# ESMS-Group-Public/FoKL-GPy

Hardware: AMD Instinct MI355X
Metric: candidate-terms/sec (basis build + Gibbs + BIC) (higher is better)
Workload: dtype f64

## Files before the change

### fokl_gpy_amd/_capi.py

```python
import ctypes
import os

import numpy as np

_HERE = os.path.dirname(os.path.abspath(__file__))
LIB_PATH = os.environ.get('FOKL_HIP_LIBRARY', os.path.join(_HERE, 'libfokl_hip.so'))

UNIQUE_ID_BYTES = 128
K_BASIS, K_GRAM, K_RESID, K_PREDICT, K_RESID_MF, K_GRAM_MFMA, K_GRAM_REDUCE = 0, 1, 2, 3, 4, 5, 6
K_INTEGRATE, K_BAND = 7, 8
K_OPTIMIZE = 9
K_OPTIMIZE_SYSTEM = 10
K_POPULATION = 11
K_RESAMPLE = 12
INTEGRATE_MAX_STATES = 4
RESID_TERMS_MAX_FACTORS = 32
RESID_TERMS_MAX_ORDER = 8
RESID_TERMS_LAYOUTS = ((8, 1), (16, 1), (8, 2), (4, 4), (2, 8), (8, 4), (16, 2), (4, 8))
SLOT_ONES, SLOT_Y, SLOT_FIRST_FREE = 0, 1, 2
PREDICT_NONE, PREDICT_VALU_LDS, PREDICT_VALU_GLOBAL, PREDICT_MFMA = 0, 1, 2, 3
POPULATION_COEFFICIENTS = ('none', 'registers', 'table')
POPULATION_MAX_CUTS = 32
RESAMPLE_MAX_COLUMNS = 768
RESAMPLE_ATTEMPT_CAP = 64
RESAMPLE_SEGMENTS = 3
RES_BETA, RES_SIG_NORMAL, RES_SIG_UNIFORM, RES_TAU_NORMAL, RES_TAU_UNIFORM, RES_START = 3, 4, 5, 6, 7, 8
GRAM_KERNELS = ('none', 'valu', 'tiles', 'dma', 'panel', 'tiles4')
RESID_KERNELS = ('none', 'columns', 'matrix_free')
BASIS_KERNELS = ('none', 'reg_table', 'lds_table')

c_int, c_i32, c_i64, c_dbl, c_vp = ctypes.c_int, ctypes.c_int32, ctypes.c_int64, ctypes.c_double, ctypes.c_void_p

SIGNATURES = {
    'fokl_version': (c_int, []),
    'fokl_device_count': (c_int, [c_vp]),
    'fokl_ctx_create': (c_int, [c_int, c_vp]),
    'fokl_ctx_destroy': (None, [c_vp]),
    'fokl_last_error': (ctypes.c_char_p, [c_vp]),
    'fokl_sync': (c_int, [c_vp]),
    'fokl_upload': (c_int, [c_vp, c_vp, c_vp, c_i64, c_int, c_int, c_vp, c_int, c_int]),
    'fokl_stage_inputs': (c_int, [c_vp, c_vp, c_i64, c_int, c_vp, c_vp]),
    'fokl_upload_staged': (c_int, [c_vp, c_vp, c_i64, c_int, c_int, c_vp, c_int, c_int, c_vp, c_vp]),
    'fokl_download_inputs': (c_int, [c_vp, c_vp]),
    'fokl_column_min_max': (c_int, [c_vp, c_i64, c_int, c_vp, c_vp, c_int]),
    'fokl_normalize_columns': (c_int, [c_vp, c_i64, c_int, c_vp, c_vp, c_int]),
    'fokl_reserve_slots': (c_int, [c_vp, c_int]),
    'fokl_slot_capacity': (c_int, [c_vp]),
    'fokl_rows': (c_i64, [c_vp]),
    'fokl_build_terms': (c_int, [c_vp, c_vp, c_int, c_vp]),
    'fokl_build_terms_deriv': (c_int, [c_vp, c_vp, c_int, c_vp, c_int, c_int, c_dbl]),
    'fokl_gram': (c_int, [c_vp, c_vp, c_int, c_vp, c_int, c_vp, c_int, c_int]),
    'fokl_gram_launch': (c_int, [c_vp, c_vp, c_int, c_vp, c_int, c_int]),
    'fokl_gram_fetch': (c_int, [c_vp, c_vp, c_i64]),
    'fokl_gram_ready': (c_int, [c_vp]),
    'fokl_gram_plan': (c_int, [c_vp, c_int, c_vp, c_int, c_int, c_vp, c_vp, c_vp, c_vp, c_vp, c_int]),
    'fokl_bic_resid': (c_int, [c_vp, c_vp, c_int, c_vp, c_vp, c_int]),
    'fokl_bic_resid_launch': (c_int, [c_vp, c_vp, c_int, c_vp]),
    'fokl_bic_resid_fetch': (c_int, [c_vp, c_vp, c_int]),
    'fokl_bic_resid_terms_launch': (c_int, [c_vp, c_vp, c_int, c_vp]),
    'fokl_predict': (c_int, [c_vp, c_vp, c_int, c_vp, c_int, c_int, c_vp, c_vp]),
    'fokl_predict_report': (c_int, [c_vp, c_vp]),
    'fokl_fit_report': (c_int, [c_vp, c_int, c_vp, c_int]),
    'fokl_population_stats': (c_int, [c_vp, c_vp, c_int, c_vp, c_int, c_vp, c_vp, c_int, c_int, c_vp, c_vp]),
    'fokl_population_report': (c_int, [c_vp, c_vp]),
    'fokl_resample_chains': (c_int, [c_vp, c_int, c_vp, c_vp, c_vp, c_dbl, c_dbl, c_dbl, c_dbl, c_dbl, c_int, c_vp, c_vp, c_int,
                                     c_int, c_int, ctypes.c_uint32, c_int, c_int, c_vp, c_vp, c_vp, c_vp, c_vp, c_vp]),
    'fokl_resample_report': (c_int, [c_vp, c_vp]),
    'fokl_read_slot': (c_int, [c_vp, c_int, c_i64, c_i64, c_vp]),
    'fokl_write_slot': (c_int, [c_vp, c_int, c_i64, c_i64, c_vp]),
    'fokl_timing_enable': (c_int, [c_vp, c_int]),
    'fokl_timing_reset': (c_int, [c_vp]),
    'fokl_timing_get': (c_int, [c_vp, c_int, c_vp, c_vp, c_vp, c_vp, c_vp]),
    'fokl_probe': (c_int, [c_vp, c_int, c_vp]),
    'fokl_gibbs_chain': (c_int, [c_vp, c_vp, c_int, c_dbl, c_dbl, c_dbl, c_dbl, c_dbl, c_dbl, c_dbl, c_int,
                                 c_vp, c_vp, c_vp, c_vp, c_vp, c_vp, c_vp]),
    'fokl_noise_tape': (c_int, [c_int, c_int, c_dbl, c_dbl, c_vp, c_vp, c_vp, c_vp, c_vp, c_vp, c_vp, c_vp, c_vp,
                                c_vp]),
    'fokl_gibbs_chain_from_tape': (c_int, [c_vp, c_vp, c_int, c_dbl, c_dbl, c_dbl, c_dbl, c_dbl, c_int, c_vp, c_vp, c_vp,
                                           c_vp, c_vp, c_vp, c_vp, c_vp, c_vp, c_vp]),
    'fokl_pool_create': (c_int, [c_int, c_int, c_int, c_int, c_int, c_vp, c_vp, c_vp, c_vp, c_vp, c_vp, c_int, c_vp]),
    'fokl_pool_stream': (c_vp, [c_vp]),
    'fokl_pool_use_dsyevd': (c_int, [c_vp, c_vp, c_int]),
    'fokl_pool_use_dgemm': (c_int, [c_vp, c_vp]),
    'fokl_device_dgemm': (None, [c_vp] * 13),
    'fokl_device_dgemm_configure': (c_int, [c_int, c_vp, c_int, c_vp]),
    'fokl_device_dgemm_stats': (c_int, [c_vp, c_vp, c_vp]),
    'fokl_pool_spectral_affinity': (c_int, [c_vp, c_vp, c_int]),
    'fokl_pool_release_hold': (c_int, [c_vp, ctypes.c_uint64]),
    'fokl_pool_destroy': (None, [c_vp]),
    'fokl_pool_submit_noise': (c_int, [c_vp, c_int, c_int, c_dbl, c_dbl, c_vp, c_vp, c_vp, c_vp, c_vp, c_vp, c_vp, c_int,
                                       c_vp, c_int, c_int, c_vp, c_vp]),
    'fokl_tape_ready': (c_int, [c_vp, c_int, c_vp, c_int]),
    'fokl_pool_resolve': (c_int, [c_vp, c_int]),
    'fokl_pool_submit_chain': (c_int, [c_vp, c_vp, c_vp, c_int, c_dbl, c_dbl, c_dbl, c_dbl, c_dbl, c_int, c_vp, c_vp,
                                       c_vp, c_vp, c_vp, c_vp, c_vp, c_int, c_int, c_vp, c_vp, c_vp, c_vp, c_vp]),
    'fokl_pool_submit_spectral': (c_int, [c_vp, c_vp, c_int, c_vp, c_int, c_int, c_vp, c_vp, c_vp, c_vp, c_vp,
                                          c_vp]),
    'fokl_pool_submit_spectral_update': (c_int, [c_vp, c_vp, c_int, c_vp, c_int, c_int, c_vp, c_vp, c_int, c_vp, c_vp, c_vp,
                                                 c_vp, c_vp, c_vp, c_vp, c_vp]),
    'fokl_pool_poll': (c_int, [c_vp]),
    'fokl_pool_wait': (c_int, [c_vp]),
    'fokl_pool_busy_seconds': (c_int, [c_vp, c_vp, c_vp, c_vp, c_vp]),
    'fokl_pool_noise_waits': (c_int, [c_vp, c_vp, c_vp]),
    'fokl_pool_chain_segments': (c_int, [c_vp, c_vp, c_vp]),
    'fokl_thread_cpu_seconds': (c_int, [c_vp, c_int]),
    'fokl_pool_stream_stats': (c_int, [c_vp, c_vp, c_vp, c_vp, c_vp, c_vp]),
    'fokl_stream_create': (c_int, [c_vp, c_i32, c_i32, c_dbl, c_int, c_vp, c_int, c_vp]),
    'fokl_stream_prestates_published': (c_i64, [c_vp]),
    'fokl_stream_given_gauss': (c_dbl, [c_vp]),
    'fokl_stream_destroy': (None, [c_vp]),
    'fokl_stream_walk': (c_int, [c_vp, c_int, c_int, c_dbl, c_dbl, c_vp, c_vp, c_vp, c_vp]),
    'fokl_stream_tell': (c_int, [c_vp, c_vp]),
    'fokl_stream_seek': (c_int, [c_vp, c_vp]),
    'fokl_stream_hold': (c_int, [c_vp, c_vp]),
    'fokl_stream_release': (c_int, [c_vp, ctypes.c_uint64]),
    'fokl_stream_advance_floor': (c_int, [c_vp]),
    'fokl_stream_state': (c_int, [c_vp, c_vp, c_vp, c_vp, c_vp]),
    'fokl_stream_expand': (c_int, [c_vp, c_int, c_dbl, c_dbl, c_vp, c_int, c_int, c_vp, c_vp, c_vp, c_vp, c_vp]),
    'fokl_stream_stats': (c_int, [c_vp, c_vp, c_vp, c_vp, c_vp, c_vp]),
    'fokl_stream_set_helpers': (c_int, [c_vp, c_int, c_vp]),
    'fokl_stream_place_bulk': (c_int, [c_vp, c_vp, c_int]),
    'fokl_stream_fast_ln_error': (c_dbl, [c_i64]),
    'fokl_search_create': (c_int, [c_vp, c_vp, c_vp, c_vp]),
    'fokl_search_bind_spectral': (c_int, [c_vp, c_vp, c_int, c_dbl, c_int]),
    'fokl_search_hold_spectral': (c_int, [c_vp, c_int]),
    'fokl_search_set_update': (c_int, [c_vp, c_int, c_int, c_int]),
    'fokl_search_set_decide': (c_int, [c_vp, c_int, c_dbl]),
    'fokl_search_set_deterministic': (c_int, [c_vp, c_int]),
    'fokl_search_destroy': (None, [c_vp]),
    'fokl_search_error': (ctypes.c_char_p, [c_vp]),
    'fokl_search_mispredicted': (c_int, [c_vp]),
    'fokl_search_set_substage': (c_int, [c_vp, c_vp, c_int]),
    'fokl_search_speculate': (c_int, [c_vp, c_vp, c_vp, c_int]),
    'fokl_search_drop_speculation': (c_int, [c_vp]),
    'fokl_search_spectral': (c_int, [c_vp, c_vp, c_int, c_vp, c_int, c_vp]),
    'fokl_search_spectral_from': (c_int, [c_vp, c_vp, c_int, c_vp, c_int, c_vp, c_int, c_vp]),
    'fokl_spectrum_done': (c_int, [c_vp]),
    'fokl_spectrum_wait': (c_int, [c_vp, c_vp, c_vp, c_vp]),
    'fokl_spectrum_release': (None, [c_vp, c_vp]),
    'fokl_spectrum_retain': (c_int, [c_vp, c_vp]),
    'fokl_search_model_begin': (c_int, [c_vp, c_vp, c_int, c_vp, c_int, c_vp, c_vp, c_vp, c_int, c_vp, c_vp]),
    'fokl_search_model_commit': (c_int, [c_vp, c_vp, c_vp, c_dbl, c_int, c_vp]),
    'fokl_run_create': (c_int, [c_vp, c_vp, c_vp]),
    'fokl_run_set_update': (c_int, [c_vp, c_int, c_int, c_int]),
    'fokl_run_search': (c_int, [c_vp, c_vp]),
    'fokl_run_result': (c_int, [c_vp, c_vp, c_vp, c_vp, c_vp, c_vp]),
    'fokl_run_arrays': (c_int, [c_vp, c_vp, c_vp, c_vp, c_vp, c_vp, c_vp]),
    'fokl_run_error': (ctypes.c_char_p, [c_vp]),
    'fokl_run_destroy': (None, [c_vp]),
    'fokl_search_score': (c_int, [c_vp, c_vp, c_dbl, c_dbl, c_int, c_int, c_vp]),
    'fokl_outcome_info': (c_int, [c_vp, c_vp, c_vp]),
    'fokl_outcome_spectrum': (c_int, [c_vp, c_vp, c_vp]),
    'fokl_outcome_chain_ready': (c_int, [c_vp]),
    'fokl_outcome_draws': (c_int, [c_vp, c_vp, c_vp]),
    'fokl_outcome_intercept_scale': (c_int, [c_vp, c_vp, c_vp]),
    'fokl_outcome_new_term_stats': (c_int, [c_vp, c_vp, c_vp, c_int, c_int, c_int, c_vp, c_vp]),
    'fokl_outcome_release': (None, [c_vp, c_vp]),
    'fokl_outcome_drop': (None, [c_vp, c_vp]),
    'fokl_search_verify': (c_int, [c_vp, c_int]),
    'fokl_search_register_forecast': (c_int, [c_vp, c_vp, c_int, c_vp, c_dbl]),
    'fokl_search_clear_forecasts': (None, [c_vp]),
    'fokl_search_likely_first_tests': (c_int, [c_vp, c_vp, c_int, c_dbl, c_vp, c_vp, c_vp]),
    'fokl_search_stats': (c_int, [c_vp, c_vp, c_int]),
    'fokl_search_trace': (c_i64, [c_vp, c_vp, c_i64]),
    'fokl_search_kill_tests': (c_int, [c_vp, c_vp, c_vp]),
    'fokl_finish_tape_blocks': (c_int, [c_int, c_int, c_vp, c_vp, c_vp, c_vp, c_int, c_int, c_int, c_vp]),
    'fokl_gibbs_chain_from_finished_tape': (c_int, [c_vp, c_vp, c_int, c_dbl, c_dbl, c_dbl, c_dbl, c_dbl, c_int, c_vp,
                                                    c_vp, c_vp, c_vp, c_int, c_vp, c_vp, c_vp, c_vp]),
    'fokl_gibbs_chain_segments_host': (c_int, [c_vp, c_vp, c_int, c_dbl, c_dbl, c_dbl, c_dbl, c_dbl, c_int, c_vp, c_vp,
                                               c_vp, c_vp, c_int, c_vp, c_vp, c_vp, c_vp, c_int, c_int, c_vp]),
    'fokl_rng_normals': (c_int, [c_vp, c_vp, c_vp, c_vp, c_i64, c_vp]),
    'fokl_rng_gammas': (c_int, [c_vp, c_vp, c_vp, c_vp, c_dbl, c_dbl, c_i64, c_vp]),
    'fokl_gp_integrate': (c_int, [c_int, c_int, c_i64, c_vp, c_vp, c_vp, c_vp, c_vp, c_vp, c_vp, c_vp, c_vp, c_int, c_int,
                                  c_dbl, c_vp, c_vp]),
    'fokl_gp_integrate_ensemble': (c_int, [c_vp, c_int, c_int, c_int, c_i64, c_vp, c_vp, c_vp, c_vp, c_vp, c_vp, c_vp, c_vp,
                                           c_vp, c_vp, c_int, c_int, c_dbl, c_vp, c_int, c_int, c_vp, c_vp, c_vp]),
    'fokl_model_optimize': (c_int, [c_vp, c_int, c_int, c_vp, c_int, c_vp, c_vp, c_int, c_int, c_vp, c_vp, c_int, c_vp, c_dbl,
                                    c_int, c_dbl, c_vp, c_vp, c_vp, c_vp]),
    'fokl_system_optimize': (c_int, [c_vp, c_int, c_int, c_vp, c_vp, c_vp, c_vp, c_vp, c_vp, c_int, c_vp, c_vp, c_int, c_int,
                                     c_vp, c_vp, c_int, c_vp, c_int, c_int, c_dbl, c_dbl, c_dbl, c_int, c_vp, c_vp, c_vp,
                                     c_int, c_dbl, c_dbl, c_vp, c_vp, c_vp, c_vp, c_vp, c_vp, c_vp]),
    'fokl_embedded_hmc': (c_int, [c_vp, c_int, c_int, c_vp, c_int, c_vp, c_int, c_vp, c_int, c_vp, c_int, c_int, c_int, c_int,
                                  ctypes.c_uint32, c_vp, c_dbl, c_int, c_vp, c_vp, c_vp, c_vp, c_vp, c_vp, c_vp, c_vp, c_vp]),
    'fokl_embedded_rng': (c_int, [ctypes.c_uint32, ctypes.c_uint32, ctypes.c_uint32, c_int, c_int, c_vp]),
    'fokl_dchain_create': (c_int, [c_int, c_int, c_vp]),
    'fokl_dchain_destroy': (None, [c_vp]),
    'fokl_dchain_submit': (c_int, [c_vp, c_int, c_int, c_vp, c_vp, c_dbl, c_dbl, c_dbl, c_dbl, c_dbl, c_vp, c_vp, c_vp,
                                   c_vp, c_vp, c_vp, c_int, c_int, c_int, c_vp, c_vp]),
    'fokl_dchain_prestate_ring': (c_int, [c_vp, c_vp, c_vp]),
    'fokl_dchain_bind_stream': (c_int, [c_vp, c_vp]),
    'fokl_dchain_submit_rows': (c_int, [c_vp, c_int, c_int, c_vp, c_vp, c_dbl, c_dbl, c_dbl, c_dbl, c_dbl, c_dbl, c_dbl, c_vp,
                                        c_vp, c_vp, c_vp, c_vp, c_int, c_vp, c_vp]),
    'fokl_dchain_stream_stats': (c_int, [c_vp, c_vp, c_vp]),
# ... 228 lines not shown
            off.append(off[-1] + pad(count))
        rows = off[4] + pad((ints[1] + d + 1) // 2) + 8
        off.append(rows)
        return tuple(off), ints, rows + 4 * d + 8

    @classmethod
    def doubles_needed(cls, p1, draws):
        return cls._layout(int(p1), int(draws))[2]

    def __init__(self, p1, draws, raw=None):
        self.p1, self.draws = p1, d = int(p1), int(draws)
        off, ints, total = self._layout(p1, d)
        self._off, self._ints = off, ints
        if raw is None:
            raw = np.empty(total, dtype=np.float64)
        elif raw.shape[0] < total:
            raise ValueError("buffer too small for this tape")
        shift = ((-raw.__array_interface__['data'][0]) % 64) // 8
        self._buf = raw[shift:]
        self._addr = self._buf.__array_interface__['data'][0]
        self._buf[off[4]:off[4] + ints[1] // 2] = 0.0
        self.finishing_requested = False
        self.materialised_by_pool = False

    def _int_area(self):
        return self._buf[self._off[4]:].view(np.int32)

    normals = property(lambda self: self._buf[:self.draws * self.p1].reshape(self.draws, self.p1))
    pair_r2 = property(lambda self: self._buf[self._off[1]:self._off[1] + self.draws * (self.p1 // 2 + 1)]
                       .reshape(self.draws, self.p1 // 2 + 1))
    gam_sig = property(lambda self: self._buf[self._off[2]:self._off[2] + self.draws])
    gam_tau = property(lambda self: self._buf[self._off[3]:self._off[3] + self.draws])
    progress = property(lambda self: self._int_area()[:1])
    block_done = property(lambda self: self._int_area()[self._ints[0]:self._ints[0] + -(-self.draws // self.BLOCK)])
    lead = property(lambda self: self._int_area()[self._ints[1]:self._ints[1] + self.draws])

    def pointers(self):
        a, off = self._addr, self._off
        return (a, a + 8 * off[1], a + 8 * off[4] + 4 * self._ints[1], a + 8 * off[2], a + 8 * off[3])

    def progress_pointer(self):
        return self._addr + 8 * self._off[4]

    def rows_pointer(self):
        return self._addr + 8 * self._off[5]

    rows = property(lambda self: self._buf[self._off[5]:self._off[5] + 4 * self.draws].view(np.uint64)
                    .reshape(self.draws, 4))

    def block_done_pointer(self):
        return self._addr + 8 * self._off[4] + 4 * self._ints[0]


def record_noise_tape(tape, astar, atau_star, stream):
    try:
        _check(load().fokl_noise_tape(tape.p1, tape.draws, float(astar), float(atau_star), *stream.args(),
                                      *tape.pointers(), tape.progress_pointer()))
    except BaseException:
        tape.progress[0] = -1
        raise
    return tape


def noise_tape(p1, draws, astar, atau_star, stream):
    return record_noise_tape(NoiseTape(p1, draws), astar, atau_star, stream)


class _StreamCursor(ctypes.Structure):
    _fields_ = [('position', ctypes.c_uint64), ('gauss_source', ctypes.c_uint64), ('has_gauss', ctypes.c_int32)]


class StreamEngine:

    def __init__(self, stream, bulk_threads=2, prestates=None):
        self._lib = load()
        self._h = None
        self.stream = stream
        h = c_vp(0)
        _check(self._lib.fokl_stream_create(_ptr(stream.key), stream.pos, stream.has_gauss, stream.cache,
                                            int(bulk_threads), prestates[0] if prestates else None,
                                            prestates[1] if prestates else 0, ctypes.byref(h)))
        self._h = h

    def close(self, write_back=True):
        if self._h:
            if write_back:
                _check(self._lib.fokl_stream_state(self._h, *self.stream.args()))
            self._lib.fokl_stream_destroy(self._h)
            self._h = None

    def __del__(self):
        self.close(write_back=False)

    def walk(self, tape, astar, atau_star):
        hold = ctypes.c_uint64(0)
        _check(self._lib.fokl_stream_hold(self._h, ctypes.byref(hold)))
        a = tape._addr
        rc = self._lib.fokl_stream_walk(self._h, tape.p1, tape.draws, float(astar), float(atau_star), tape.rows_pointer(),
                                        a + 8 * tape._off[2], a + 8 * tape._off[3], tape.progress_pointer())
        if rc:
            self._lib.fokl_stream_release(self._h, hold)
        _check(rc)
        _check(self._lib.fokl_stream_advance_floor(self._h))
        return hold.value

    def expand(self, tape, astar, atau_star, first=0, last=None):
        ptr = tape.pointers()
        _check(self._lib.fokl_stream_expand(self._h, tape.p1, float(astar), float(atau_star), tape.rows_pointer(),
                                            int(first), tape.draws if last is None else int(last), ptr[0], ptr[1], ptr[2],
                                            ptr[3], ptr[4]))
        return tape

    def release(self, hold):
        _check(self._lib.fokl_stream_release(self._h, ctypes.c_uint64(hold)))

    def tell(self):
        cur = _StreamCursor()
        _check(self._lib.fokl_stream_tell(self._h, ctypes.byref(cur)))
        return cur

    def seek(self, cursor):
        _check(self._lib.fokl_stream_seek(self._h, ctypes.byref(cursor)))

    def numpy_state(self):
        st = LegacyStream(self.stream.as_numpy_state())
        _check(self._lib.fokl_stream_state(self._h, *st.args()))
        return st.as_numpy_state()

    def stats(self):
        b, w, seg, ga, ge = c_dbl(0), c_dbl(0), c_i64(0), c_i64(0), c_i64(0)
        _check(self._lib.fokl_stream_stats(self._h, *[ctypes.byref(x) for x in (b, w, seg, ga, ge)]))
        return dict(bulk_s=b.value, walker_wait_s=w.value, segments=seg.value, gamma_attempts=ga.value,
                    gamma_attempts_exact=ge.value)


def tape_ready(tape):
    return load().fokl_tape_ready(tape.progress_pointer(), tape.draws,
                                  tape.block_done_pointer() if tape.materialised_by_pool else None, tape.BLOCK)


def gibbs_chain_from_tape(lamb, qty, b, btau, dtd, sigsqd0, tausqd0, tape, want_sig_tau=False, follow=False):
    lamb = np.ascontiguousarray(lamb, dtype=np.float64)
    qty = np.ascontiguousarray(qty, dtype=np.float64)
    p1 = lamb.shape[0]
    if p1 != tape.p1:
        raise ValueError("tape was recorded for a different model size")
    w = np.empty((tape.draws, p1), dtype=np.float64)
    sigs = np.empty(tape.draws) if want_sig_tau else None
    taus = np.empty(tape.draws) if want_sig_tau else None
    flag = ctypes.c_int32(0)
    _check(load().fokl_gibbs_chain_from_tape(_ptr(lamb), _ptr(qty), p1, float(b), float(btau), float(dtd),
                                             float(sigsqd0), float(tausqd0), tape.draws, *tape.pointers(), _ptr(w),
                                             _ptr(sigs), _ptr(taus), ctypes.byref(flag),
                                             tape.progress_pointer() if follow else None))
    if want_sig_tau:
        return w, bool(flag.value), sigs, taus
    return w, bool(flag.value)


def finish_tape_blocks(tape, part=0, parts=1, follow=False):
    ptr = tape.pointers()
    _check(load().fokl_finish_tape_blocks(tape.p1, tape.draws, ptr[0], ptr[1], ptr[2],
                                          tape.progress_pointer() if follow else None, int(part), int(parts),
                                          tape.BLOCK, tape.block_done_pointer()))


def gibbs_chain_from_finished_tape(lamb, qty, b, btau, dtd, sigsqd0, tausqd0, tape, follow=False):
    lamb = np.ascontiguousarray(lamb, dtype=np.float64)
    qty = np.ascontiguousarray(qty, dtype=np.float64)
    p1 = lamb.shape[0]
    if p1 != tape.p1:
        raise ValueError("tape was recorded for a different model size")
    w = np.empty((tape.draws, p1), dtype=np.float64)
    flag = ctypes.c_int32(0)
    ptr = tape.pointers()
    _check(load().fokl_gibbs_chain_from_finished_tape(_ptr(lamb), _ptr(qty), p1, float(b), float(btau), float(dtd),
                                                      float(sigsqd0), float(tausqd0), tape.draws, ptr[0], ptr[3],
                                                      ptr[4], tape.block_done_pointer() if follow else None,
                                                      tape.BLOCK, _ptr(w), None, None, ctypes.byref(flag)))
    return w, bool(flag.value)


CHAIN_SEGMENTS, CHAIN_WARM = 8, 64


def gibbs_chain_segments_host(lamb, qty, b, btau, dtd, sigsqd0, tausqd0, tape, follow=False, segments=CHAIN_SEGMENTS,
                              warm=CHAIN_WARM, states=False):
    lamb = np.ascontiguousarray(lamb, dtype=np.float64)
    qty = np.ascontiguousarray(qty, dtype=np.float64)
    p1 = lamb.shape[0]
    if p1 != tape.p1:
        raise ValueError("tape was recorded for a different model size")
    w = np.empty((tape.draws, p1), dtype=np.float64)
    sigs = np.empty(tape.draws, dtype=np.float64) if states else None
    taus = np.empty(tape.draws, dtype=np.float64) if states else None
    flag, bad_cut = ctypes.c_int32(0), ctypes.c_int32(0)
    ptr = tape.pointers()
    _check(load().fokl_gibbs_chain_segments_host(_ptr(lamb), _ptr(qty), p1, float(b), float(btau), float(dtd),
                                                 float(sigsqd0), float(tausqd0), tape.draws, ptr[0], ptr[3], ptr[4],
                                                 tape.block_done_pointer() if follow else None, tape.BLOCK, _ptr(w),
                                                 _ptr(sigs) if states else None, _ptr(taus) if states else None,
                                                 ctypes.byref(flag), int(segments), int(warm), ctypes.byref(bad_cut)))
    if states:
        return w, bool(flag.value), bool(bad_cut.value), sigs, taus
    return w, bool(flag.value), bool(bad_cut.value)



def _scipy_dsyevd_address():
    try:
        from scipy.linalg import cython_lapack
        capsule = cython_lapack.__pyx_capi__['dsyevd']
        api = ctypes.pythonapi
        api.PyCapsule_GetName.restype = ctypes.c_char_p
        api.PyCapsule_GetName.argtypes = [ctypes.py_object]
        api.PyCapsule_GetPointer.restype = ctypes.c_void_p
        api.PyCapsule_GetPointer.argtypes = [ctypes.py_object, ctypes.c_char_p]
        name = api.PyCapsule_GetName(capsule)
        if name is None or name.count(b'int *') != 6 or b'long' in name:
            return None
        return api.PyCapsule_GetPointer(capsule, name)
    except (ImportError, KeyError):
        return None


def _scipy_dgemm_address():
    try:
        from scipy.linalg import cython_blas
        capsule = cython_blas.__pyx_capi__['dgemm']
        api = ctypes.pythonapi
        api.PyCapsule_GetName.restype = ctypes.c_char_p
        api.PyCapsule_GetName.argtypes = [ctypes.py_object]
        api.PyCapsule_GetPointer.restype = ctypes.c_void_p
        api.PyCapsule_GetPointer.argtypes = [ctypes.py_object, ctypes.c_char_p]
        name = api.PyCapsule_GetName(capsule)
        if name is None or name.count(b'int *') != 6 or name.count(b'char *') != 2 or b'long' in name:
            return None
        return api.PyCapsule_GetPointer(capsule, name)
    except (ImportError, KeyError):
        return None


def _scipy_dsyevr_address():
    from scipy.linalg import cython_lapack
    capsule = cython_lapack.__pyx_capi__['dsyevr']
    api = ctypes.pythonapi
    api.PyCapsule_GetName.restype = ctypes.c_char_p
    api.PyCapsule_GetName.argtypes = [ctypes.py_object]
    api.PyCapsule_GetPointer.restype = ctypes.c_void_p
    api.PyCapsule_GetPointer.argtypes = [ctypes.py_object, ctypes.c_char_p]
    name = api.PyCapsule_GetName(capsule)
    if name is None or name.count(b'int *') != 11 or b'long' in name:
        raise FoklNativeError(-2, f"unexpected signature of scipy's dsyevr: {name!r}")
    return api.PyCapsule_GetPointer(capsule, name)


class PoolJob:
    __slots__ = ('_h', 'keep', 'result', 'recycle', 'held', 'unresolved', 'ignore_failure', 'co_reader')

    def __init__(self, handle, keep, result=None, tentative=False):
        self._h, self.keep, self.result = handle, keep, result
        self.recycle = None
        self.held = None
        self.unresolved = bool(tentative)
        self.ignore_failure = False
        self.co_reader = None

    def done(self):
        if self._h is not None and load().fokl_pool_poll(self._h):
            self.wait()
        return self._h is None

    def resolve(self, commit):
        if self.unresolved:
            self.unresolved = False
            _check(load().fokl_pool_resolve(self._h, int(bool(commit))))

    def wait(self):
        if self._h is not None:
            h, self._h = self._h, None
            rc = load().fokl_pool_wait(h)
            if not self.ignore_failure:
                _check(rc)
        return self.result


class SpectralResult:
    __slots__ = ('lamb', 'Qt', 'qty', 'betahat', 'moments', '_buf', '_addr')

    @staticmethod
    def doubles(p1):
        return p1 * (p1 + 3) + 2

    def __init__(self, p1, buf=None):
        buf = self._buf = np.empty(p1 * (p1 + 3) + 2, dtype=np.float64) if buf is None else buf
        self._addr = buf.__array_interface__['data'][0]
        self.lamb, self.qty, self.betahat = buf[:p1], buf[p1:2 * p1], buf[2 * p1:3 * p1]
        self.Qt = buf[3 * p1:3 * p1 + p1 * p1].reshape(p1, p1)
        self.moments = buf[3 * p1 + p1 * p1:]

    def pointers(self, p1):
        a = self._addr
        return (a, a + 24 * p1, a + 8 * p1, a + 16 * p1, a + 8 * p1 * (p1 + 3))


class HostPool:

    def __init__(self, stream, chain_threads=2, finish_threads=2, spectral_threads=3, noise_cpu=-1, bulk_threads=2,
                 prestates=None, device_dgemm=None):
        self._lib = load()
        self.stream = stream
        self._h = None
        h = c_vp(0)
        fn = _scipy_dsyevr_address() if spectral_threads > 0 else None
        self.finish_threads = int(finish_threads)
        _check(self._lib.fokl_pool_create(int(chain_threads), self.finish_threads, int(spectral_threads),
                                          max(1, int(bulk_threads)), int(noise_cpu), c_vp(fn),
                                          *stream.args(), prestates[0] if prestates else None,
                                          prestates[1] if prestates else 0, ctypes.byref(h)))
        self._h = h
        self.dsyevd_from = 0
        dc_from = int(os.environ.get('FOKL_EIGH_DC_FROM', '80'))
        if spectral_threads > 0 and dc_from > 0 and os.environ.get('FOKL_EIGH_SIGNS', 'canonical') != 'lapack':
            fd = _scipy_dsyevd_address()
            if fd:
                _check(self._lib.fokl_pool_use_dsyevd(self._h, c_vp(fd), dc_from))
                self.dsyevd_from = dc_from
        self.has_dgemm = False
        if spectral_threads > 0:
            fg = _scipy_dgemm_address()
            self.device_dgemm_from = 0
            if fg and device_dgemm is not None:
                entry = c_vp(0)
                if self._lib.fokl_device_dgemm_configure(int(device_dgemm[0]), c_vp(fg), int(device_dgemm[1]),
                                                         ctypes.byref(entry)) == 0 and entry.value:
                    fg, self.device_dgemm_from = entry.value, int(device_dgemm[1])
            if fg:
                _check(self._lib.fokl_pool_use_dgemm(self._h, c_vp(fg)))
                self.has_dgemm = True

    def spectral_affinity(self, cpus):
        cpus = np.ascontiguousarray(sorted(cpus), dtype=np.int32)
        _check(self._lib.fokl_pool_spectral_affinity(self._h, _ptr(cpus), cpus.shape[0]))

    def stream_handle(self):
        return self._lib.fokl_pool_stream(self._h)

    def set_walk_helpers(self, count, cpus=None):
        arr = None
        if cpus is not None:
            arr = np.ascontiguousarray(list(cpus)[:count] + [-1] * max(0, count - len(cpus)), dtype=np.int32)
        _check(self._lib.fokl_stream_set_helpers(c_vp(self.stream_handle()), int(count), _ptr(arr) if arr is not None else None))

    def place_bulk_threads(self, cpus):
        arr = np.ascontiguousarray(list(cpus), dtype=np.int32)
        _check(self._lib.fokl_stream_place_bulk(c_vp(self.stream_handle()), _ptr(arr), arr.shape[0]))

    def close(self):
        if self._h:
            self._lib.fokl_pool_destroy(self._h)
            self._h = None

    __del__ = close

    def submit_noise(self, tape, astar, atau_star, tentative=False, finish=False):
        h = c_vp(0)
        finish = bool(finish) and self.finish_threads > 0
        _check(self._lib.fokl_pool_submit_noise(self._h, tape.p1, tape.draws, float(astar), float(atau_star),
                                                tape.rows_pointer(), *tape.pointers(), tape.progress_pointer(),
                                                int(bool(tentative)), tape.block_done_pointer(), tape.BLOCK, int(finish),
                                                None, ctypes.byref(h)))
        tape.finishing_requested = finish
        tape.materialised_by_pool = True
        return PoolJob(h, (tape,), tape, tentative)

    def submit_chain(self, lamb, qty, b, btau, dtd, sigsqd0, tausqd0, tape, w_raw=None):
        p1 = lamb.shape[0]
        if p1 != tape.p1:
            raise ValueError("tape was recorded for a different model size")
        if w_raw is None:
            w = np.empty((tape.draws, p1), dtype=np.float64)
        else:
            w = w_raw[:tape.draws * p1].reshape(tape.draws, p1)
        flag = np.zeros(1, dtype=np.int32)
        h = c_vp(0)
        _check(self._lib.fokl_pool_submit_chain(self._h, _ptr(lamb), _ptr(qty), p1, float(b), float(btau), float(dtd),
                                                float(sigsqd0), float(tausqd0), tape.draws, *tape.pointers(),
                                                tape.progress_pointer(), tape.block_done_pointer(),
                                                tape.BLOCK, int(tape.finishing_requested), _ptr(w), _ptr(flag),
                                                None, None, ctypes.byref(h)))
        return PoolJob(h, (lamb, qty, tape, w, flag), (w, flag))

    def submit_spectral(self, gram, idx, ycol):
        p1 = idx.shape[0]
        res = SpectralResult(p1)
        h = c_vp(0)
        _check(self._lib.fokl_pool_submit_spectral(self._h, _ptr(gram), gram.shape[1], _ptr(idx), p1, int(ycol),
                                                   *res.pointers(p1), ctypes.byref(h)))
        return PoolJob(h, (gram, idx, res), res)

    def submit_spectral_update(self, gram, idx, ycol, parent, parent_pos):
        p1 = idx.shape[0]
        res = SpectralResult(p1)
        updated = np.full(1, -1, dtype=np.int32)
        h = c_vp(0)
        _check(self._lib.fokl_pool_submit_spectral_update(self._h, _ptr(gram), gram.shape[1], _ptr(idx), p1, int(ycol),
                                                          _ptr(parent.lamb), _ptr(parent.Qt), int(parent_pos), None,
                                                          *res.pointers(p1), _ptr(updated), ctypes.byref(h)))
        return PoolJob(h, (gram, idx, res, parent, updated), res), updated

    def busy_seconds(self):
        v = [c_dbl(0) for _ in range(4)]
        _check(self._lib.fokl_pool_busy_seconds(self._h, *[ctypes.byref(x) for x in v]))
        w = [c_dbl(0), c_dbl(0)]
        _check(self._lib.fokl_pool_noise_waits(self._h, ctypes.byref(w[0]), ctypes.byref(w[1])))
        b, ww, seg, ga, ge = c_dbl(0), c_dbl(0), c_i64(0), c_i64(0), c_i64(0)
        _check(self._lib.fokl_pool_stream_stats(self._h, *[ctypes.byref(x) for x in (b, ww, seg, ga, ge)]))
        cs = [c_i64(0), c_i64(0)]
        _check(self._lib.fokl_pool_chain_segments(self._h, ctypes.byref(cs[0]), ctypes.byref(cs[1])))
        return dict(noise=v[0].value, chain=v[1].value, finish=v[2].value, spectral=v[3].value,
                    host_chains_segmented=cs[0].value, host_chain_recuts=cs[1].value,
                    noise_queue_wait=w[0].value, noise_verdict_wait=w[1].value, bulk=b.value, walker_wait=ww.value,
                    stream_segments=seg.value, gamma_attempts=ga.value, gamma_attempts_exact=ge.value)



class _SearchParams(ctypes.Structure):
    _fields_ = [('n', c_i64), ('a', c_dbl), ('b', c_dbl), ('atau', c_dbl), ('btau', c_dbl), ('threshav', c_dbl),
                ('threshstda', c_dbl), ('threshstdb', c_dbl), ('guess_margin', c_dbl), ('draws', c_i32), ('half0', c_i32),
                ('aic', c_i32), ('lookahead', c_i32), ('foresight', c_i32), ('speculation_max', c_i32),
                ('tentative_tapes', c_i32), ('test_rewinds', c_i32), ('device_chain_columns', c_i32),
                ('finish_threads', c_i32), ('flip_guess', c_i32), ('device_rows', c_i32)]


class _OutcomeView(ctypes.Structure):
    _fields_ = [('spectrum', c_vp), ('idx', c_vp), ('ev', c_dbl), ('siglik', c_dbl), ('intercept_scale', c_dbl),
                ('p1', c_i32), ('on_device', c_i32)]


_FORESEE_CB = ctypes.CFUNCTYPE(None, c_vp, ctypes.POINTER(c_i32), c_int)
_IDLE_CB = ctypes.CFUNCTYPE(c_int, c_vp)
_RESIDUAL_CB = ctypes.CFUNCTYPE(c_int, c_vp, ctypes.POINTER(c_i32), c_int, ctypes.POINTER(c_dbl), ctypes.POINTER(c_dbl),
                                ctypes.POINTER(c_dbl))


class _KillTestsArgs(ctypes.Structure):
# ... 301 lines not shown
        self._engine, self._ticket, self.p1, self.draws, self.keep = engine, ticket, p1, draws, keep
        self.recycle = None
        self._stats = None
        self.ignore_failure = False
        self._area = self._flag = None
        self._mark = float(ticket) if ticket is not None else 0.0
        self._misses = 0
        if stats_address:
            self._area = np.ctypeslib.as_array((ctypes.c_double * (7 + p1)).from_address(stats_address))
            self._flag = ctypes.c_double.from_address(stats_address + 8 * (4 + p1))

    def resolve(self, commit):
        pass

    def _ran(self):
        return self._flag is not None and self._flag.value == self._mark

    def done(self):
        if self._ticket is None or self._stats is not None or self._ran():
            return True
        if self._flag is not None:
            self._misses += 1
            if self._misses % 64:
                return False
        return bool(self._engine._lib.fokl_dchain_poll(self._engine._h, self._ticket))

    def wait(self):
        if self._stats is None:
            if self._ticket is None:
                raise RuntimeError("device chain: released before anybody read its statistics")
            if self._ran():
                self._stats = np.array(self._area[:4 + self.p1])
            else:
                buf = np.empty(4 + self.p1, dtype=np.float64)
                _check(self._engine._lib.fokl_dchain_wait(self._engine._h, self._ticket, _ptr(buf)))
                self._stats = buf
        return self._stats[4:], np.array([int(self._stats[0])], dtype=np.int32)

    @property
    def kernel_seconds(self):
        if self._area is not None and self._ran():
            return float(self._area[5 + self.p1])
        return 0.0

    @property
    def rows_averaged(self):
        self.wait()
        return int(self._stats[3])

    @property
    def bad_cut(self):
        self.wait()
        if self._area is None:
            raise RuntimeError("device chain: released, its statistics area belongs to another chain")
        return bool(self._area[6 + self.p1] != 0.0)

    @property
    def last_state(self):
        self.wait()
        return float(self._stats[1]), float(self._stats[2])

    def fetch_w(self, out=None):
        w = np.empty((self.draws, self.p1), dtype=np.float64) if out is None else out
        _check(self._engine._lib.fokl_dchain_fetch_w(self._engine._h, self._ticket, _ptr(w)))
        return w

    def try_release(self):
        if self._ticket is None or not self._engine._h:
            return True
        if self._flag is not None and not self._ran() and self._stats is None:
            return False
        if self._engine._lib.fokl_dchain_try_release(self._engine._h, self._ticket):
            self._ticket, self.keep, self._area, self._flag = None, None, None, None
            return True
        return False

    def release(self):
        if self._ticket is not None and self._engine._h:
            self._engine._lib.fokl_dchain_release(self._engine._h, self._ticket)
        self._ticket = None
        self.keep = self._area = self._flag = None


class DeviceChainEngine:
    max_columns = 768

    def __init__(self, device=0, slots=96):
        self._lib = load()
        self._h = None
        h = c_vp(0)
        _check(self._lib.fokl_dchain_create(int(device), int(slots), ctypes.byref(h)))
        self._h = h
        self.device = int(device)

    def close(self):
        if self._h:
            self._lib.fokl_dchain_destroy(self._h)
            self._h = None

    __del__ = close

    def submit(self, lamb, qty, b, btau, dtd, sigsqd0, tausqd0, tape, stat_first=0, follow=True):
        lamb = np.ascontiguousarray(lamb, dtype=np.float64)
        qty = np.ascontiguousarray(qty, dtype=np.float64)
        p1 = lamb.shape[0]
        if p1 != tape.p1:
            raise ValueError("tape was recorded for a different model size")
        ptr = tape.pointers()
        finished = bool(tape.finishing_requested)
        ticket, area = c_i64(0), c_vp(0)
        _check(self._lib.fokl_dchain_submit(self._h, p1, tape.draws, _ptr(lamb), _ptr(qty), float(b), float(btau),
                                            float(dtd), float(sigsqd0), float(tausqd0), ptr[0], ptr[2], ptr[3], ptr[4],
                                            tape.progress_pointer() if follow else None,
                                            tape.block_done_pointer() if finished or tape.materialised_by_pool else None,
                                            tape.BLOCK, int(finished),
                                            int(stat_first), ctypes.byref(ticket), ctypes.byref(area)))
        return DeviceChainJob(self, ticket.value, p1, tape.draws, (tape,), area.value)

    def prestate_ring(self):
        ring, entries = c_vp(0), c_int(0)
        _check(self._lib.fokl_dchain_prestate_ring(self._h, ctypes.byref(ring), ctypes.byref(entries)))
        return ring.value, entries.value

    def bind(self, stream_handle):
        _check(self._lib.fokl_dchain_bind_stream(self._h, stream_handle))

    def submit_rows(self, lamb, qty, b, btau, dtd, sigsqd0, tausqd0, astar, atau_star, tape, span, stat_first=0):
        lamb = np.ascontiguousarray(lamb, dtype=np.float64)
        qty = np.ascontiguousarray(qty, dtype=np.float64)
        p1 = lamb.shape[0]
        ptr = tape.pointers()
        ticket, area = c_i64(0), c_vp(0)
        _check(self._lib.fokl_dchain_submit_rows(self._h, p1, tape.draws, _ptr(lamb), _ptr(qty), float(b), float(btau),
                                                 float(dtd), float(sigsqd0), float(tausqd0), float(astar), float(atau_star),
                                                 tape.rows_pointer(), ptr[3], ptr[4], tape.progress_pointer(), _ptr(span),
                                                 int(stat_first), ctypes.byref(ticket), ctypes.byref(area)))
        return DeviceChainJob(self, ticket.value, p1, tape.draws, (tape, span), area.value)

    def stream_stats(self):
        seg, rows = c_i64(0), c_i64(0)
        _check(self._lib.fokl_dchain_stream_stats(self._h, ctypes.byref(seg), ctypes.byref(rows)))
        return dict(segments_made=seg.value, rows_jobs=rows.value)

    def flush(self):
        _check(self._lib.fokl_dchain_flush(self._h))

    def stats(self):
        busy, issued, launches, staged = c_dbl(0), c_i64(0), c_i64(0), c_i64(0)
        _check(self._lib.fokl_dchain_stats(self._h, ctypes.byref(busy), ctypes.byref(issued), ctypes.byref(launches),
                                           ctypes.byref(staged)))
        recuts = c_i64(0)
        _check(self._lib.fokl_dchain_recuts(self._h, ctypes.byref(recuts)))
        return dict(dispatch_s=busy.value, issued=issued.value, launches=launches.value, staged=staged.value,
                    recuts=recuts.value)


class DeviceSpectralJob:

    def __init__(self, engine, ticket, result, p1):
        self.engine, self.ticket, self.p1 = engine, int(ticket), int(p1)
        n = self.p1
        area = (ctypes.c_double * (n * n + 3 * n + 7)).from_address(result)
        self._area = np.frombuffer(area, dtype=np.float64)
        self._released = False

    def done(self):
        rc = self.engine._lib.fokl_dspectral_poll(self.engine._h, self.ticket)
        if rc < 0:
            _check(-rc)
        return rc == 1

    def wait(self):
        _check(self.engine._lib.fokl_dspectral_wait(self.engine._h, self.ticket))
        n, a = self.p1, self._area
        return a[:n], a[3 * n:3 * n + n * n].reshape(n, n), a[n:2 * n], a[2 * n:3 * n], a[3 * n + n * n:3 * n + n * n + 2]

    def info(self):
        a = self._area[3 * self.p1 + self.p1 * self.p1 + 2:]
        return dict(sweeps=int(a[0]), rotations=int(a[1]), seconds=float(a[2]), not_converged=bool(a[3]))
# ... 147 lines not shown
                 bic_resid_fetch=bic_resid_fetch)
    keep = [pending, raised]
    for name, fn in table.items():
        cb = _OPS_TYPES[name](guard(fn))
        keep.append(cb)
        setattr(ops, name, ctypes.cast(cb, c_vp).value)
    return ops, tuple(keep)


class NativeRun:

    def __init__(self, backend, kernel_id, **params):
        self._lib = load()
        self._h = None
        self._ops, self._keep = backend_ops(backend, kernel_id)
        if isinstance(self._keep[0], dict):
            self._keep[0]['m'] = int(params['m'])
        self._prm = _RunParams(**{k: int(v) for k, v in params.items()})
        self.m = int(params['m'])
        h = c_vp(0)
        _check(self._lib.fokl_run_create(ctypes.byref(self._ops), ctypes.byref(self._prm), ctypes.byref(h)))
        self._h = h
        self._reraise()

    def _reraise(self):
        raised = self._keep[1] if isinstance(self._keep[0], dict) else None
        if raised:
            exc = raised[0]
            del raised[:]
            raise exc

    def set_update(self, from_columns, depth, lookahead):
        _check(self._lib.fokl_run_set_update(self._h, int(from_columns), int(depth), int(lookahead)))

    def search(self, native_search):
        rc = self._lib.fokl_run_search(self._h, native_search._h)
        self._reraise()
        if rc != 0:
            native_search._checked(rc)
        return self

    def result(self):
        rows, n_evs, subs = c_i32(0), c_i32(0), c_i32(0)
        best, last = c_vp(0), c_vp(0)
        _check(self._lib.fokl_run_result(self._h, ctypes.byref(rows), ctypes.byref(n_evs), ctypes.byref(subs),
                                         ctypes.byref(best), ctypes.byref(last)))
        mtx = np.zeros((max(rows.value, 0), self.m), dtype=np.int32)
        evs = np.zeros(n_evs.value)
        sizes = np.zeros(max(subs.value, 1), dtype=np.int32)
        stats = np.zeros(16)
        total = self._lib.fokl_run_arrays(self._h, _ptr(mtx) if mtx.size else None, _ptr(evs) if evs.size else None,
                                          _ptr(sizes), None, None, _ptr(stats))
        mean_abs, rel_std = np.zeros(max(total, 1)), np.zeros(max(total, 1))
        self._lib.fokl_run_arrays(self._h, None, None, None, _ptr(mean_abs), _ptr(rel_std), None)
        per, at = [], 0
        for size in sizes[:subs.value]:
            per.append(dict(mean_abs=mean_abs[at:at + size].copy(), rel_std=rel_std[at:at + size].copy()))
            at += int(size)
        return (mtx.astype(np.float64), evs, per, best.value, last.value, dict(zip(RUN_STATS, stats[:len(RUN_STATS)])))

    def close(self):
        if self._h is not None and self._h:
            self._lib.fokl_run_destroy(self._h)
            self._h = None

    def __del__(self):
        try:
            self.close()
        except Exception:
            pass


class DeviceContext:

    def __init__(self, device=0):
        self._lib = load()
        h = c_vp(0)
        _check(self._lib.fokl_ctx_create(int(device), ctypes.byref(h)))
        self._h = h
        self.device = device

    def close(self):
        if getattr(self, '_h', None) is not None and self._h:
            self._lib.fokl_ctx_destroy(self._h)
            self._h = None

    def __del__(self):
        try:
            self.close()
        except Exception:
            pass

    def _ck(self, rc):
        _check(rc, self._h)

    def sync(self):
        self._ck(self._lib.fokl_sync(self._h))

    _lazy_owner = None

    def _settle_lazy_inputs(self, keep=None):
        owner, self._lazy_owner = self._lazy_owner, None
        model = owner() if owner is not None else None
        if model is not None and model is not keep:
            model._materialise_inputs()

    def upload(self, x, y, kernel_id, phis_packed, n_basis, width):
        self._settle_lazy_inputs()
        x = np.ascontiguousarray(x, dtype=np.float64)
        y = np.ascontiguousarray(np.reshape(y, -1), dtype=np.float64)
        if x.ndim != 2 or x.shape[0] != y.shape[0]:
            raise ValueError("inputs must be [n, m] and data [n]")
        phis_packed = np.ascontiguousarray(phis_packed, dtype=np.float64)
        self._ck(self._lib.fokl_upload(self._h, _ptr(x), _ptr(y), x.shape[0], x.shape[1], int(kernel_id),
                                       _ptr(phis_packed), int(n_basis), int(width)))
        self.n, self.m = x.shape

    def stage_inputs(self, x, owner=None):
        if x.dtype != np.float64 or x.ndim != 2 or not x.flags.c_contiguous:
            raise ValueError("stage_inputs: float64 C-contiguous [n, m] expected")
        self._settle_lazy_inputs(keep=owner)
        lows, highs = np.empty(x.shape[1]), np.empty(x.shape[1])
        self._ck(self._lib.fokl_stage_inputs(self._h, _ptr(x), x.shape[0], x.shape[1], _ptr(lows), _ptr(highs)))
        self._staged_shape = x.shape
        return lows, highs

    def upload_staged(self, y, kernel_id, phis_packed, n_basis, width, lows, spans, owner=None):
        n, m = self._staged_shape
        y = np.ascontiguousarray(np.reshape(y, -1), dtype=np.float64)
        if y.shape[0] != n:
            raise ValueError("inputs must be [n, m] and data [n]")
        phis_packed = np.ascontiguousarray(phis_packed, dtype=np.float64)
        lows, spans = np.ascontiguousarray(lows, dtype=np.float64), np.ascontiguousarray(spans, dtype=np.float64)
        self._ck(self._lib.fokl_upload_staged(self._h, _ptr(y), n, m, int(kernel_id), _ptr(phis_packed), int(n_basis),
                                              int(width), _ptr(lows), _ptr(spans)))
        self.n, self.m = n, m
        if owner is not None:
            import weakref
            self._lazy_owner = weakref.ref(owner)

    def download_inputs(self):
        out = np.empty((getattr(self, 'n', 0) or 1, getattr(self, 'm', 0) or 1), dtype=np.float64)
        self._ck(self._lib.fokl_download_inputs(self._h, _ptr(out)))
        return out

    def reserve_slots(self, n_slots):
        self._ck(self._lib.fokl_reserve_slots(self._h, int(n_slots)))

    @property
    def slot_capacity(self):
        return self._lib.fokl_slot_capacity(self._h)

    def build_terms(self, terms, slots):
        terms = np.ascontiguousarray(np.atleast_2d(terms), dtype=np.int32)
        slots = np.ascontiguousarray(slots, dtype=np.int32)
        if terms.shape[0] != slots.shape[0]:
            raise ValueError("one slot per term")
        self._ck(self._lib.fokl_build_terms(self._h, _ptr(terms), terms.shape[0], _ptr(slots)))

    def build_terms_deriv(self, terms, slots, wrt_input, order, divisor):
        terms = np.ascontiguousarray(np.atleast_2d(terms), dtype=np.int32)
        slots = np.ascontiguousarray(slots, dtype=np.int32)
        if terms.shape[0] != slots.shape[0]:
            raise ValueError("one slot per term")
        self._ck(self._lib.fokl_build_terms_deriv(self._h, _ptr(terms), terms.shape[0], _ptr(slots), int(wrt_input),
                                                  int(order), float(divisor)))
# ... 317 lines not shown
```

### fokl_gpy_amd/csrc/fokl_hostpool.cpp

```cpp
#include <algorithm>
#include <array>
#include <atomic>
#include <chrono>
#include <cmath>
#include <condition_variable>
#include <cstdint>
#include <cstdio>
#include <cstdlib>
#include <cstring>
#include <deque>
#include <mutex>
#include <string>
#include <thread>
#include <vector>

#include <immintrin.h>
#include <pthread.h>
#include <sched.h>
#include <sys/prctl.h>

#include "../../include/fokl_hip_internal.h"
#include "fokl_spin.h"

extern void fokl_set_global_error(const std::string &msg);

extern "C" __attribute__((visibility("hidden"))) void fokl_finish_tape_rows(int p1, double *normals, const double *pair_r2,
                                                                            const int32_t *lead, int k0, int k1);
extern "C" __attribute__((visibility("hidden"))) int64_t fokl_chain_follow_waited_ns();
extern "C" __attribute__((visibility("hidden"))) int fokl_gibbs_chain_from_raw_blocks(
    const double *lamb, const double *qty, int p1, double b, double btau, double dtd, double sigsqd0, double tausqd0,
    int draws, const double *normals, const double *pair_r2, const int32_t *lead, const double *gam_sig,
    const double *gam_tau, const int32_t *block_done, int block, double *w_out, int32_t *bstar_negative);

static std::atomic<int64_t> g_thread_cpu_ns[8];

extern "C" __attribute__((visibility("hidden"))) void fokl_note_thread_cpu(int kind)
{
    timespec ts;
    if (kind >= 0 && kind < 8 && clock_gettime(CLOCK_THREAD_CPUTIME_ID, &ts) == 0)
        g_thread_cpu_ns[kind].fetch_add((int64_t)ts.tv_sec * 1000000000LL + ts.tv_nsec, std::memory_order_relaxed);
}

extern "C" __attribute__((visibility("hidden"))) int64_t fokl_dchain_dispatcher_cpu_ns();

extern "C" int fokl_thread_cpu_seconds(double *seconds, int count)
{
    if (!seconds || count < 6) {
        fokl_set_global_error("fokl_thread_cpu_seconds: room for six values is needed");
        return FOKL_ERR_ARG;
    }
    for (int k = 0; k < 5; ++k) seconds[k] = 1e-9 * (double)g_thread_cpu_ns[k].load(std::memory_order_relaxed);
    seconds[5] = 1e-9 * (double)fokl_dchain_dispatcher_cpu_ns();
    return 6;
}

namespace {

struct ThreadCpuNote {
    int kind;
    ~ThreadCpuNote() { fokl_note_thread_cpu(kind); }
};

using dsyevr_fn = void (*)(char *jobz, char *range, char *uplo, int *n, double *a, int *lda, double *vl, double *vu,
                           int *il, int *iu, double *abstol, int *m, double *w, double *z, int *ldz, int *isuppz,
                           double *work, int *lwork, int *iwork, int *liwork, int *info);

using dsyevd_fn = void (*)(char *jobz, char *uplo, int *n, double *a, int *lda, double *w, double *work, int *lwork,
                          int *iwork, int *liwork, int *info);

using dgemm_fn = void (*)(char *transa, char *transb, int *m, int *n, int *k, double *alpha, double *a, int *lda, double *b,
                          int *ldb, double *beta, double *c, int *ldc);

enum class Kind { noise, chain, finish, spectral };

struct Queue {
    std::mutex m;
    std::condition_variable cv;
    std::deque<fokl_host_job *> q;
    bool stop = false;
};

}

struct fokl_host_job {
    void (*then)(void *) = nullptr;
    void *then_arg = nullptr;
    Kind kind;
    fokl_host_pool *pool = nullptr;
    std::atomic<int> done{0};
    int status = FOKL_OK;
    std::string error;
    bool tentative = false;
    std::atomic<int> verdict{0};
    int64_t t_submit = 0, t_start = 0, t_recorded = 0;
    std::atomic<int> pending{1};
    std::atomic<int> started{0};
    fokl_host_job *parent = nullptr;
    int p1 = 0, draws = 0;
    double astar = 0, atau_star = 0;
    fokl_tape_row *rows = nullptr;
    uint64_t hold = 0;
    bool held = false;
    uint64_t *span_out = nullptr;
    bool rows_only = false;
    bool finish_normals = false;
    double *normals = nullptr, *pair_r2 = nullptr, *gam_sig = nullptr, *gam_tau = nullptr;
    int32_t *lead = nullptr, *progress = nullptr;
    const double *lamb = nullptr, *qty = nullptr;
    double b = 0, btau = 0, dtd = 0, sigsqd0 = 0, tausqd0 = 0;
    double *w_out = nullptr;
    int32_t *bstar_negative = nullptr;
    const int32_t *raw_block_done = nullptr;
    int32_t *block_done = nullptr;
    int block = 0, part = 0, parts = 0;
    bool self_owned = false;
    const double *gram = nullptr;
    int ld = 0, ycol = 0;
    std::vector<int32_t> idx;
    double *lamb_out = nullptr, *qt_out = nullptr, *qty_out = nullptr, *betahat_out = nullptr, *moments_out = nullptr;
    const double *parent_lamb = nullptr, *parent_qt = nullptr;
    int parent_pos = -1;
    bool parent_failed = false;
    int32_t *updated_out = nullptr;
    std::vector<fokl_host_job *> dependents;
    bool has_run = false;
    int run_status = FOKL_OK;
};

struct fokl_host_pool {
    Queue noise_q, chain_q, spectral_q;
    std::deque<Queue> finish_q;
    std::vector<std::thread> threads;
    std::vector<size_t> spectral_thread_ids;
    dsyevr_fn dsyevr = nullptr;
    dsyevd_fn dsyevd = nullptr;
    int dsyevd_from = 0;
    dgemm_fn dgemm = nullptr;
    std::mutex dep_m;
    fokl_stream *stream = nullptr;
    uint32_t *mt_key = nullptr;
    int32_t *mt_pos = nullptr, *has_gauss = nullptr;
    double *gauss_cache = nullptr;
    std::atomic<int64_t> noise_busy_ns{0}, chain_busy_ns{0}, finish_busy_ns{0}, spectral_busy_ns{0};
    std::atomic<int64_t> chains_segmented{0}, chain_recuts{0};
    bool chain_profile = std::getenv("FOKL_CHAIN_PROFILE") != nullptr;
    std::atomic<int64_t> noise_queue_wait_ns{0}, noise_verdict_wait_ns{0};
    std::mutex done_m;
    std::condition_variable done_cv;
    std::mutex start_m;
    std::condition_variable start_cv;
    std::string trace_path;
    std::vector<std::array<int64_t, 7>> trace;
    int test_delay_us = 0;
    bool lapack_signs = false;
    double singular = 1e-9;
};

namespace {

inline int64_t now_ns()
{
    return std::chrono::duration_cast<std::chrono::nanoseconds>(std::chrono::steady_clock::now().time_since_epoch())
        .count();
}

void finish(fokl_host_job *job, int status, const char *what)
{
    fokl_host_pool *pool = job->pool;
    job->status = status;
    if (status != FOKL_OK) job->error = what;
    {
        std::lock_guard<std::mutex> lock(pool->done_m);
        job->done.store(1, std::memory_order_release);
    }
    pool->done_cv.notify_all();
}

void spectral_tail(fokl_host_pool *pool, fokl_host_job *job, const double *xty);

int spectral(fokl_host_pool *pool, fokl_host_job *job, std::string &err)
{
    const int n = (int)job->idx.size();
    const int32_t *idx = job->idx.data();
    const double *g = job->gram;
    const size_t ld = (size_t)job->ld;
    static thread_local std::vector<double> a, xty, work;
    static thread_local std::vector<int> iwork, isuppz;
    if (a.size() < (size_t)n * n) a.resize((size_t)n * n);
    if (xty.size() < (size_t)n) xty.resize((size_t)n);
    for (int i = 0; i < n; ++i) {
        const double *row = g + (size_t)idx[i] * ld;
        for (int j = 0; j < n; ++j) a[(size_t)j * n + i] = row[idx[j]];
        xty[i] = row[job->ycol];
    }
    char jobz = 'V', range = 'A', uplo = 'L';
    int nn = n, lda = n, ldz = n, il = 1, iu = n, m = 0, info = 0, lwork = -1, liwork = -1, iwork_query = 0;
    double vl = 0.0, vu = 1.0, abstol = 0.0, work_query = 0.0;
    double *z = job->qt_out;
    bool by_dsyevd = false;
    if (pool->dsyevd && pool->dsyevd_from > 0 && n >= pool->dsyevd_from && !pool->lapack_signs) {
        std::memcpy(z, a.data(), sizeof(double) * (size_t)n * n);
        pool->dsyevd(&jobz, &uplo, &nn, z, &lda, job->lamb_out, &work_query, &lwork, &iwork_query, &liwork, &info);
        if (info != 0) {
            err = "dsyevd workspace query failed";
            return FOKL_ERR_NUMERIC;
        }
        lwork = (int)work_query;
        liwork = iwork_query;
        if (work.size() < (size_t)std::max(1, lwork)) work.resize((size_t)std::max(1, lwork));
        if (iwork.size() < (size_t)std::max(1, liwork)) iwork.resize((size_t)std::max(1, liwork));
        pool->dsyevd(&jobz, &uplo, &nn, z, &lda, job->lamb_out, work.data(), &lwork, iwork.data(), &liwork, &info);
        if (info != 0) {
            err = "dsyevd did not converge (info = " + std::to_string(info) + ")";
            return FOKL_ERR_NUMERIC;
        }
        by_dsyevd = true;
    }
    if (by_dsyevd && !(job->lamb_out[0] > pool->singular * job->lamb_out[n - 1])) {
        by_dsyevd = false;
        lwork = liwork = -1;
    }
    if (!by_dsyevd) {
        if (isuppz.size() < (size_t)2 * std::max(1, n)) isuppz.resize((size_t)2 * std::max(1, n));
        pool->dsyevr(&jobz, &range, &uplo, &nn, a.data(), &lda, &vl, &vu, &il, &iu, &abstol, &m, job->lamb_out, z, &ldz,
                     isuppz.data(), &work_query, &lwork, &iwork_query, &liwork, &info);
        if (info != 0) {
            err = "dsyevr workspace query failed";
            return FOKL_ERR_NUMERIC;
        }
        lwork = (int)work_query;
        liwork = iwork_query;
        if (work.size() < (size_t)std::max(1, lwork)) work.resize((size_t)std::max(1, lwork));
        if (iwork.size() < (size_t)std::max(1, liwork)) iwork.resize((size_t)std::max(1, liwork));
        pool->dsyevr(&jobz, &range, &uplo, &nn, a.data(), &lda, &vl, &vu, &il, &iu, &abstol, &m, job->lamb_out, z, &ldz,
                     isuppz.data(), work.data(), &lwork, iwork.data(), &liwork, &info);
        if (info != 0 || m != n) {
            err = "dsyevr did not converge (info = " + std::to_string(info) + ")";
            return FOKL_ERR_NUMERIC;
        }
    }
    spectral_tail(pool, job, xty.data());
    return FOKL_OK;
}

void spectral_tail(fokl_host_pool *pool, fokl_host_job *job, const double *xty)
{
    const int n = (int)job->idx.size();
    const int32_t *idx = job->idx.data();
    const double *g = job->gram;
    const size_t ld = (size_t)job->ld;
    double *z = job->qt_out;
    for (int j = 0; j < n && !pool->lapack_signs; ++j) {
        double *v = z + (size_t)j * n;
        int piv = 0;
        double best = std::fabs(v[0]);
        for (int i = 1; i < n; ++i)
// ... 290 lines not shown
    if (deps.size() > 1) {
        {
            std::lock_guard<std::mutex> lk(pool->spectral_q.m);
            for (auto it = deps.rbegin(); it + 1 != deps.rend(); ++it) pool->spectral_q.q.push_front(*it);
        }
        if (deps.size() > 2)
            pool->spectral_q.cv.notify_all();
        else
            pool->spectral_q.cv.notify_one();
    }
    return deps.front();
}

fokl_host_job *run(fokl_host_pool *pool, fokl_host_job *job)
{
    const auto t0 = std::chrono::steady_clock::now();
    fokl_host_job *next = nullptr;
    int rc = FOKL_OK;
    std::string err;
    std::atomic<int64_t> *busy = nullptr;
    switch (job->kind) {
    case Kind::noise:
        break;
    case Kind::finish:
        rc = expand_tape_blocks(pool, job);
        busy = &pool->finish_busy_ns;
        break;
    case Kind::chain:
        if (pool->chain_profile) job->t_start = now_ns();
        if (job->block_done) {
            int32_t recut = 0;
            rc = fokl_gibbs_chain_segments_host(job->lamb, job->qty, job->p1, job->b, job->btau, job->dtd, job->sigsqd0,
                                                job->tausqd0, job->draws, job->normals, job->gam_sig, job->gam_tau,
                                                job->block_done, job->block, job->w_out, nullptr, nullptr,
                                                job->bstar_negative, FOKL_CHAIN_SEGMENTS, FOKL_CHAIN_WARM, &recut);
            const char *recursion = std::getenv("FOKL_HCHAIN_RECURSION");
            if (job->draws >= 4 * FOKL_CHAIN_WARM && !(recursion && std::strcmp(recursion, "serial") == 0))
                pool->chains_segmented.fetch_add(1, std::memory_order_relaxed);
            if (recut) pool->chain_recuts.fetch_add(1, std::memory_order_relaxed);
            const auto t_chain = std::chrono::steady_clock::now();
            if (rc != FOKL_OK) err = "chain: invalid arguments or the tape producer failed";
            if (rc == FOKL_OK && job->then) job->then(job->then_arg);
            if (pool->chain_profile) {
                const auto us = [](std::chrono::steady_clock::duration d) {
                    return 1e-3 * (double)std::chrono::duration_cast<std::chrono::nanoseconds>(d).count();
                };
                const double waited = 1e-3 * (double)fokl_chain_follow_waited_ns();
                std::fprintf(stderr, "fokl_chain: p1 %d draws %d queued %.1f us, waited for the tape %.1f us, recursion %.1f us, "
                                     "statistics %.1f us, recut %d\n", job->p1, job->draws, 1e-3 * (double)(job->t_start - job->t_submit),
                             waited, us(t_chain - t0) - waited, us(std::chrono::steady_clock::now() - t_chain), (int)recut);
            }
            busy = &pool->chain_busy_ns;
            break;
        }
        rc = fokl_gibbs_chain_from_raw_blocks(job->lamb, job->qty, job->p1, job->b, job->btau, job->dtd, job->sigsqd0,
                                              job->tausqd0, job->draws, job->normals, job->pair_r2, job->lead,
                                              job->gam_sig, job->gam_tau, job->raw_block_done, job->block, job->w_out,
                                              job->bstar_negative);
        if (rc != FOKL_OK) err = "chain: invalid arguments or the tape producer failed";
        if (rc == FOKL_OK && job->then) job->then(job->then_arg);
        busy = &pool->chain_busy_ns;
        break;
    case Kind::spectral:
        rc = job->parent_lamb ? spectral_update(pool, job, err) : spectral(pool, job, err);
        next = release_dependents(pool, job, rc);
        busy = &pool->spectral_busy_ns;
        break;
    }
    if (busy) {
        const auto dt = std::chrono::steady_clock::now() - t0;
        busy->fetch_add(std::chrono::duration_cast<std::chrono::nanoseconds>(dt).count(), std::memory_order_relaxed);
    }
    if (job->self_owned) {
        if (job->parent) settle(job->parent);
        delete job;
        return next;
    }
    finish(job, rc, err.c_str());
    return next;
}

void worker(fokl_host_pool *pool, Queue *queue)
{
    ThreadCpuNote note{queue == &pool->chain_q ? 1 : queue == &pool->spectral_q ? 3 : 2};
    prctl(PR_SET_TIMERSLACK, 2000UL, 0, 0, 0);
    for (;;) {
        fokl_host_job *job;
        {
            std::unique_lock<std::mutex> lock(queue->m);
            queue->cv.wait(lock, [&] { return queue->stop || !queue->q.empty(); });
            if (queue->q.empty()) return;
            job = queue->q.front();
            queue->q.pop_front();
        }
        while (job) job = run(pool, job);
    }
}

struct Speculation {
    fokl_host_job *job;
    fokl_stream_cursor at_start;
};

constexpr size_t kMaxSpeculation = 64;

void trace_noise(fokl_host_pool *pool, fokl_host_job *job, int64_t verdict_seen)
{
    if (!pool->trace_path.empty())
        pool->trace.push_back({job->t_submit, job->t_start, job->t_recorded, verdict_seen, job->p1,
                               job->tentative ? 1 : 0, job->verdict.load(std::memory_order_acquire)});
}

void settle(fokl_host_job *job)
{
    if (job->pending.fetch_sub(1, std::memory_order_acq_rel) != 1) return;
    fokl_host_pool *pool = job->pool;
    if (job->held && !job->span_out) {
        job->held = false;
        fokl_stream_release(pool->stream, job->hold);
    }
    {
        std::lock_guard<std::mutex> lock(pool->done_m);
        job->done.store(1, std::memory_order_release);
    }
    pool->done_cv.notify_all();
}

void mark_started(fokl_host_pool *pool, fokl_host_job *job)
{
    if (job->pending.load(std::memory_order_relaxed) > 1) {
        {
            std::lock_guard<std::mutex> lock(pool->start_m);
            job->started.store(1, std::memory_order_release);
        }
        pool->start_cv.notify_all();
    } else {
        job->started.store(1, std::memory_order_release);
    }
}

void record_tape(fokl_host_pool *pool, fokl_host_job *job)
{
    mark_started(pool, job);
    const auto t0 = std::chrono::steady_clock::now();
    job->t_start = std::chrono::duration_cast<std::chrono::nanoseconds>(t0.time_since_epoch()).count();
    int rc = fokl_stream_hold(pool->stream, &job->hold);
    job->held = rc == FOKL_OK;
    if (job->span_out) job->span_out[0] = job->hold;
    if (rc == FOKL_OK && job->rows_only) {
        int32_t local = 0;
        rc = fokl_stream_walk(pool->stream, job->p1, job->draws, job->astar, job->atau_star, job->rows, job->gam_sig,
                              job->gam_tau, &local);
        if (rc == FOKL_OK) {
            fokl_stream_cursor at;
            fokl_stream_tell(pool->stream, &at);
            if (job->span_out) job->span_out[1] = at.position;
        }
        __atomic_store_n(job->progress, rc == FOKL_OK ? job->draws : -1, __ATOMIC_RELEASE);
    } else if (rc == FOKL_OK && !pool->finish_q.empty()) {
        rc = fokl_stream_walk(pool->stream, job->p1, job->draws, job->astar, job->atau_star, job->rows, job->gam_sig,
                              job->gam_tau, job->progress);
    } else if (rc == FOKL_OK) {
        const int block = job->block > 0 ? job->block : FOKL_TAPE_BLOCK;
        for (int k0 = 0; k0 < job->draws && rc == FOKL_OK; k0 += block) {
            const int k1 = std::min(job->draws, k0 + block);
            rc = fokl_stream_walk(pool->stream, job->p1, k1 - k0, job->astar, job->atau_star, job->rows + k0,
                                  job->gam_sig + k0, job->gam_tau + k0, nullptr);
            if (rc == FOKL_OK)
                rc = fokl_stream_expand(pool->stream, job->p1, job->astar, job->atau_star, job->rows, k0, k1, job->normals,
                                        job->pair_r2, job->lead, job->gam_sig, job->gam_tau);
            if (rc != FOKL_OK) break;
            if (job->block_done) __atomic_store_n(job->block_done + k0 / block, 1, __ATOMIC_RELEASE);
            __atomic_store_n(job->progress, k1, __ATOMIC_RELEASE);
        }
        if (rc != FOKL_OK) {
            if (job->block_done)
                for (int blk = 0; blk < (job->draws + block - 1) / block; ++blk) {
                    int32_t open = 0;
                    __atomic_compare_exchange_n(job->block_done + blk, &open, -1, false, __ATOMIC_ACQ_REL,
                                                __ATOMIC_ACQUIRE);
                }
            __atomic_store_n(job->progress, -1, __ATOMIC_RELEASE);
        }
    }
    if (rc != FOKL_OK) {
        job->status = rc;
        job->error = "noise tape: invalid arguments, gamma shape or the stream's producers failed";
    }
    fokl_stream_advance_floor(pool->stream);
    const auto t1 = std::chrono::steady_clock::now();
    job->t_recorded = std::chrono::duration_cast<std::chrono::nanoseconds>(t1.time_since_epoch()).count();
    pool->noise_busy_ns.fetch_add(std::chrono::duration_cast<std::chrono::nanoseconds>(t1 - t0).count(),
                                  std::memory_order_relaxed);
}

void noise_worker(fokl_host_pool *pool)
{
    ThreadCpuNote note{0};
    prctl(PR_SET_TIMERSLACK, 2000UL, 0, 0, 0);
    Queue *queue = &pool->noise_q;
    std::deque<Speculation> open;
    auto aborted = [&](fokl_host_job *job) {
        __atomic_store_n(job->progress, -1, __ATOMIC_RELEASE);
        if (job->block_done && job->pending.load(std::memory_order_acquire) <= 1) {
            const int block = job->block > 0 ? job->block : FOKL_TAPE_BLOCK;
            for (int blk = 0; blk < (job->draws + block - 1) / block; ++blk) {
                int32_t open = 0;
                __atomic_compare_exchange_n(job->block_done + blk, &open, -1, false, __ATOMIC_ACQ_REL, __ATOMIC_ACQUIRE);
            }
        }
        mark_started(pool, job);
        trace_noise(pool, job, now_ns());
        settle(job);
    };
    auto first_aborted = [&]() -> size_t {
        size_t i = 0;
        while (i < open.size() && open[i].job->verdict.load(std::memory_order_acquire) >= 0) ++i;
        return i;
    };
    auto settle_verdicts = [&] {
        while (!open.empty() && open.front().job->verdict.load(std::memory_order_acquire) > 0) {
            fokl_host_job *job = open.front().job;
            open.pop_front();
            trace_noise(pool, job, now_ns());
            settle(job);
        }
        const size_t cut = first_aborted();
        if (cut < open.size()) {
            fokl_stream_seek(pool->stream, &open[cut].at_start);
            for (size_t k = cut; k < open.size(); ++k) aborted(open[k].job);
            open.erase(open.begin() + (std::ptrdiff_t)cut, open.end());
        }
    };
    for (;;) {
        settle_verdicts();
        if (pool->test_delay_us > 0)
            std::this_thread::sleep_for(std::chrono::microseconds(pool->test_delay_us));
        fokl_host_job *job = nullptr;
        bool stopping = false, must_settle = false;
        {
            std::unique_lock<std::mutex> lock(queue->m);
            if (open.empty()) {
                const auto w0 = std::chrono::steady_clock::now();
                queue->cv.wait(lock, [&] { return queue->stop || !queue->q.empty(); });
                pool->noise_queue_wait_ns.fetch_add(
                    std::chrono::duration_cast<std::chrono::nanoseconds>(std::chrono::steady_clock::now() - w0).count(),
                    std::memory_order_relaxed);
                if (queue->q.empty()) return;
            }
            stopping = queue->stop;
            if (!queue->q.empty()) {
                fokl_host_job *next = queue->q.front();
                if (!open.empty() && first_aborted() < open.size())
                    must_settle = true;
                else if (open.empty() || (next->tentative && open.size() < kMaxSpeculation)) {
                    job = next;
                    queue->q.pop_front();
                }
            }
        }
        if (must_settle) continue;
        if (!job) {
            (void)stopping;
            const auto w0 = std::chrono::steady_clock::now();
            auto settled = [&] {
                return open.front().job->verdict.load(std::memory_order_acquire) > 0 || first_aborted() < open.size();
            };
            auto more = [&] {
                if (open.size() >= kMaxSpeculation) return false;
                std::lock_guard<std::mutex> lock(queue->m);
                return !queue->q.empty() && queue->q.front()->tentative;
            };
            for (int spins = 0; !settled(); ++spins) {
                if (spins < fokl_spin_budget(4000)) {
                    _mm_pause();
                    if ((spins & 63) == 63 && more()) break;
                } else {
                    std::unique_lock<std::mutex> lock(queue->m);
                    if (settled()) break;
                    if (open.size() < kMaxSpeculation && !queue->q.empty() && queue->q.front()->tentative) break;
                    queue->cv.wait_until(lock, std::chrono::system_clock::now() + std::chrono::microseconds(200));
                    if (open.size() < kMaxSpeculation && !queue->q.empty() && queue->q.front()->tentative) break;
                }
            }
            pool->noise_verdict_wait_ns.fetch_add(
                std::chrono::duration_cast<std::chrono::nanoseconds>(std::chrono::steady_clock::now() - w0).count(),
                std::memory_order_relaxed);
            continue;
        }
        if (job->tentative) {
            if (job->verdict.load(std::memory_order_acquire) < 0) {
                aborted(job);
                continue;
            }
            open.push_back({job, {}});
            fokl_stream_tell(pool->stream, &open.back().at_start);
            record_tape(pool, job);
        } else {
            record_tape(pool, job);
            trace_noise(pool, job, job->t_recorded);
            settle(job);
        }
    }
}

void submit(Queue &queue, fokl_host_job *job)
{
    {
        std::lock_guard<std::mutex> lock(queue.m);
        queue.q.push_back(job);
    }
    queue.cv.notify_one();
}

void stop(Queue &queue)
{
    {
        std::lock_guard<std::mutex> lock(queue.m);
        queue.stop = true;
    }
    queue.cv.notify_all();
}

}

extern "C" int fokl_pool_create(int chain_threads, int finish_threads, int spectral_threads, int bulk_threads,
                                int noise_cpu, void *dsyevr, uint32_t *mt_key, int32_t *mt_pos, int32_t *has_gauss,
                                double *gauss_cache, uint32_t *prestate_ring, int prestate_entries, fokl_host_pool **out)
{
    if (!out || chain_threads < 1 || bulk_threads < 1 || bulk_threads > 16 || spectral_threads < 0 || chain_threads > 64 || spectral_threads > 64 ||
        finish_threads < 0 || finish_threads > 64 || !mt_key ||
        !mt_pos || !has_gauss || !gauss_cache || (spectral_threads > 0 && !dsyevr)) {
        fokl_set_global_error("fokl_pool_create: bad thread counts, null RNG state or missing dsyevr");
        return FOKL_ERR_ARG;
    }
    if (*mt_pos < 0 || *mt_pos > 624) {
        fokl_set_global_error("fokl_pool_create: invalid MT19937 position");
        return FOKL_ERR_ARG;
    }
    auto *pool = new fokl_host_pool();
    if (fokl_stream_create(mt_key, *mt_pos, *has_gauss, *gauss_cache, bulk_threads, prestate_ring, prestate_entries,
                           &pool->stream) != FOKL_OK) {
        delete pool;
        return FOKL_ERR_STATE;
    }
    pool->dsyevr = reinterpret_cast<dsyevr_fn>(dsyevr);
    pool->mt_key = mt_key;
    pool->mt_pos = mt_pos;
    pool->has_gauss = has_gauss;
    pool->gauss_cache = gauss_cache;
    if (const char *path = std::getenv("FOKL_POOL_TRACE")) pool->trace_path = path;
    if (const char *us = std::getenv("FOKL_POOL_TEST_DELAY_US")) pool->test_delay_us = std::max(0, std::atoi(us));
    if (const char *signs = std::getenv("FOKL_EIGH_SIGNS")) pool->lapack_signs = std::strcmp(signs, "lapack") == 0;
    if (const char *sing = std::getenv("FOKL_EIGH_SINGULAR")) pool->singular = std::max(0.0, std::atof(sing));
    try {
        pool->threads.emplace_back(noise_worker, pool);
        if (noise_cpu >= 0 && noise_cpu < CPU_SETSIZE) {
            cpu_set_t set;
            CPU_ZERO(&set);
            CPU_SET(noise_cpu, &set);
            pthread_setaffinity_np(pool->threads.back().native_handle(), sizeof(set), &set);
        }
        for (int i = 0; i < chain_threads; ++i) pool->threads.emplace_back(worker, pool, &pool->chain_q);
        pool->finish_q.resize((size_t)finish_threads);
        for (auto &q : pool->finish_q) pool->threads.emplace_back(worker, pool, &q);
        for (int i = 0; i < spectral_threads; ++i) {
            pool->spectral_thread_ids.push_back(pool->threads.size());
            pool->threads.emplace_back(worker, pool, &pool->spectral_q);
        }
    } catch (const std::exception &e) {
        stop(pool->noise_q);
        stop(pool->chain_q);
        stop(pool->spectral_q);
        for (auto &q : pool->finish_q) stop(q);
        for (auto &t : pool->threads) t.join();
        fokl_stream_destroy(pool->stream);
        delete pool;
        fokl_set_global_error(std::string("fokl_pool_create: ") + e.what());
        return FOKL_ERR_STATE;
    }
    *out = pool;
    return FOKL_OK;
}

extern "C" void fokl_pool_destroy(fokl_host_pool *pool)
{
    if (!pool) return;
    stop(pool->noise_q);
    stop(pool->chain_q);
    stop(pool->spectral_q);
    for (auto &q : pool->finish_q) stop(q);
    for (auto &t : pool->threads) t.join();
    fokl_stream_state(pool->stream, pool->mt_key, pool->mt_pos, pool->has_gauss, pool->gauss_cache);
    fokl_stream_destroy(pool->stream);
    if (!pool->trace_path.empty()) {
        if (FILE *f = std::fopen(pool->trace_path.c_str(), "a")) {
            for (const auto &r : pool->trace)
                std::fprintf(f, "noise %lld %lld %lld %lld %lld %lld %lld\n", (long long)r[0], (long long)r[1],
                             (long long)r[2], (long long)r[3], (long long)r[4], (long long)r[5], (long long)r[6]);
            std::fclose(f);
        }
    }
    delete pool;
}

static void submit_finish_jobs(fokl_host_pool *pool, fokl_host_job *parent, bool finish_normals)
{
    const int parts = (int)pool->finish_q.size();
    for (int part = 0; part < parts; ++part) {
        auto *fin = new fokl_host_job();
        fin->pool = pool;
        fin->kind = Kind::finish;
        fin->self_owned = true;
        fin->parent = parent;
        fin->p1 = parent->p1;
        fin->draws = parent->draws;
        fin->astar = parent->astar;
        fin->atau_star = parent->atau_star;
        fin->rows = parent->rows;
        fin->normals = parent->normals;
        fin->pair_r2 = parent->pair_r2;
        fin->lead = parent->lead;
        fin->gam_sig = parent->gam_sig;
        fin->gam_tau = parent->gam_tau;
        fin->progress = parent->progress;
        fin->block_done = parent->block_done;
        fin->block = parent->block;
        fin->finish_normals = finish_normals;
        fin->part = part;
        fin->parts = parts;
        submit(pool->finish_q[(size_t)part], fin);
    }
}

extern "C" int fokl_pool_submit_noise(fokl_host_pool *pool, int p1, int draws, double astar, double atau_star,
                                      fokl_tape_row *rows, double *normals, double *pair_r2, int32_t *lead,
                                      double *gam_sig, double *gam_tau, int32_t *progress, int tentative,
                                      int32_t *block_done, int block, int finish, uint64_t *span_out,
                                      fokl_host_job **out)
{
    const bool rows_only = finish == 2;
    if (!pool || !out || p1 <= 0 || draws < 0 || !rows || !gam_sig || !gam_tau || !progress ||
        (!rows_only && (!normals || !pair_r2 || !lead || !block_done || block < 1)) || (rows_only && !span_out)) {
        fokl_set_global_error("fokl_pool_submit_noise: null pointer, empty model or bad block size");
        return FOKL_ERR_ARG;
    }
    auto *job = new fokl_host_job();
    job->pool = pool;
    job->kind = Kind::noise;
    job->p1 = p1;
    job->draws = draws;
    job->astar = astar;
    job->atau_star = atau_star;
    job->rows = rows;
    job->normals = normals;
    job->pair_r2 = pair_r2;
    job->lead = lead;
    job->gam_sig = gam_sig;
    job->gam_tau = gam_tau;
    job->progress = progress;
    job->block_done = block_done;
    job->block = block;
    job->tentative = tentative != 0;
    job->span_out = span_out;
    job->rows_only = rows_only;
    if (!pool->trace_path.empty()) job->t_submit = now_ns();
    *out = job;
    if (!rows_only && !pool->finish_q.empty()) {
        job->pending.store(1 + (int)pool->finish_q.size(), std::memory_order_relaxed);
        submit_finish_jobs(pool, job, finish == 1);
    }
    submit(pool->noise_q, job);
    return FOKL_OK;
}

extern "C" int fokl_pool_submit_chain(fokl_host_pool *pool, const double *lamb, const double *qty, int p1, double b,
                                      double btau, double dtd, double sigsqd0, double tausqd0, int draws,
                                      const double *normals, const double *pair_r2, const int32_t *lead,
                                      const double *gam_sig, const double *gam_tau, const int32_t *progress,
                                      int32_t *block_done, int block, int finishing_requested, double *w_out,
                                      int32_t *bstar_negative, void (*then)(void *), void *then_arg, fokl_host_job **out)
{
    if (!pool || !out || !lamb || !qty || p1 <= 0 || draws < 0 || !normals || !pair_r2 || !lead || !gam_sig ||
        !gam_tau || !progress || !w_out || !bstar_negative || !block_done || block < 1) {
        fokl_set_global_error("fokl_pool_submit_chain: null pointer or empty model");
        return FOKL_ERR_ARG;
    }
    auto *job = new fokl_host_job();
    job->pool = pool;
    job->kind = Kind::chain;
    job->lamb = lamb;
    job->qty = qty;
    job->p1 = p1;
    job->b = b;
    job->btau = btau;
    job->dtd = dtd;
    job->sigsqd0 = sigsqd0;
    job->tausqd0 = tausqd0;
    job->draws = draws;
    job->normals = const_cast<double *>(normals);
    job->pair_r2 = const_cast<double *>(pair_r2);
    job->lead = const_cast<int32_t *>(lead);
    job->gam_sig = const_cast<double *>(gam_sig);
    job->gam_tau = const_cast<double *>(gam_tau);
    job->progress = const_cast<int32_t *>(progress);
    job->w_out = w_out;
    job->bstar_negative = bstar_negative;
    job->block = block;
    job->then = then;
    job->then_arg = then_arg;
    if (finishing_requested)
        job->block_done = block_done;
    else
        job->raw_block_done = block_done;
    *out = job;
    if (pool->chain_profile) job->t_submit = now_ns();
    submit(pool->chain_q, job);
    return FOKL_OK;
}

static int new_spectral_job(const char *who, fokl_host_pool *pool, const double *gram, int ld, const int32_t *idx, int p1,
                            int ycol, double *lamb_out, double *qt_out, double *qty_out, double *betahat_out,
                            double *moments_out, fokl_host_job **job_out)
{
    const std::string name(who);
    if (!pool || !job_out || !gram || !idx || p1 <= 0 || ld <= 0 || ycol < 0 || ycol >= ld || !lamb_out || !qt_out ||
        !qty_out || !betahat_out) {
        fokl_set_global_error(name + ": null pointer, empty model or y column out of range");
        return FOKL_ERR_ARG;
    }
    if (!pool->dsyevr) {
        fokl_set_global_error(name + ": the pool was created without spectral threads");
        return FOKL_ERR_STATE;
    }
    for (int i = 0; i < p1; ++i)
        if (idx[i] < 0 || idx[i] >= ld) {
            fokl_set_global_error(name + ": column index out of range");
            return FOKL_ERR_ARG;
        }
    auto *job = new fokl_host_job();
    job->pool = pool;
    job->kind = Kind::spectral;
    job->gram = gram;
    job->ld = ld;
    job->ycol = ycol;
    job->idx.assign(idx, idx + p1);
    job->lamb_out = lamb_out;
    job->qt_out = qt_out;
    job->qty_out = qty_out;
    job->betahat_out = betahat_out;
    job->moments_out = moments_out;
    *job_out = job;
    return FOKL_OK;
}

extern "C" int fokl_pool_submit_spectral(fokl_host_pool *pool, const double *gram, int ld, const int32_t *idx, int p1,
                                         int ycol, double *lamb_out, double *qt_out, double *qty_out,
                                         double *betahat_out, double *moments_out, fokl_host_job **out)
{
    const int rc = new_spectral_job("fokl_pool_submit_spectral", pool, gram, ld, idx, p1, ycol, lamb_out, qt_out, qty_out,
                                    betahat_out, moments_out, out);
    if (rc == FOKL_OK) submit(pool->spectral_q, *out);
    return rc;
}

extern "C" int fokl_pool_submit_spectral_update(fokl_host_pool *pool, const double *gram, int ld, const int32_t *idx, int p1,
                                                int ycol, const double *parent_lamb, const double *parent_qt,
                                                int parent_pos, fokl_host_job *parent_job, double *lamb_out,
                                                double *qt_out, double *qty_out, double *betahat_out, double *moments_out,
                                                int32_t *updated, fokl_host_job **out)
{
    if (!parent_lamb || !parent_qt || parent_pos < 0 || parent_pos > p1 ||
        (parent_job && (parent_job->kind != Kind::spectral || parent_job->pool != pool))) {
        fokl_set_global_error("fokl_pool_submit_spectral_update: no parent, position out of range or a job of another kind");
        return FOKL_ERR_ARG;
    }
    const int rc = new_spectral_job("fokl_pool_submit_spectral_update", pool, gram, ld, idx, p1, ycol, lamb_out, qt_out,
                                    qty_out, betahat_out, moments_out, out);
    if (rc != FOKL_OK) return rc;
    fokl_host_job *job = *out;
    job->parent_lamb = parent_lamb;
    job->parent_qt = parent_qt;
    job->parent_pos = parent_pos;
    job->updated_out = updated;
    if (parent_job) {
        std::lock_guard<std::mutex> lk(pool->dep_m);
        if (!parent_job->has_run) {
            parent_job->dependents.push_back(job);
            return FOKL_OK;
        }
        job->parent_failed = parent_job->run_status != FOKL_OK;
    }
    submit(pool->spectral_q, job);
    return FOKL_OK;
}

extern "C" int fokl_pool_use_dgemm(fokl_host_pool *pool, void *fn)
{
    if (!pool) {
        fokl_set_global_error("fokl_pool_use_dgemm: null pool");
        return FOKL_ERR_ARG;
    }
    pool->dgemm = reinterpret_cast<dgemm_fn>(fn);
    return FOKL_OK;
}

extern "C" int fokl_tape_ready(const int32_t *progress, int draws, const int32_t *block_done, int block)
{
    if (progress) {
        const int32_t p = __atomic_load_n(progress, __ATOMIC_ACQUIRE);
        if (p < 0) return -1;
        if (p < draws) return 0;
    }
    if (block_done && block > 0) {
        const int nblocks = (draws + block - 1) / block;
        for (int blk = nblocks - 1; blk >= 0; --blk) {
            const int32_t f = __atomic_load_n(block_done + blk, __ATOMIC_ACQUIRE);
            if (f < 0) return -1;
            if (f == 0) return 0;
        }
    }
    return 1;
}

extern "C" int fokl_pool_resolve(fokl_host_job *job, int commit)
{
    if (!job || job->kind != Kind::noise || !job->tentative) {
        fokl_set_global_error("fokl_pool_resolve: not a tentative noise job");
        return FOKL_ERR_ARG;
    }
    int expected = 0;
    if (!job->verdict.compare_exchange_strong(expected, commit ? 1 : -1)) {
        fokl_set_global_error("fokl_pool_resolve: the job has been resolved already");
        return FOKL_ERR_STATE;
    }
// ... 115 lines not shown
```

### fokl_gpy_amd/csrc/fokl_stream.cpp

```cpp
#include <algorithm>
#include <atomic>
#include <chrono>
#include <cmath>
#include <condition_variable>
#include <cstdint>
#include <cstdio>
#include <cstdlib>
#include <cstring>
#include <memory>
#include <mutex>
#include <set>
#include <string>
#include <thread>
#include <vector>

#include <immintrin.h>
#include <sched.h>
#include <deque>

#include "../../include/fokl_hip_internal.h"
#include "fokl_spin.h"

extern void fokl_set_global_error(const std::string &msg);
extern "C" __attribute__((visibility("hidden"))) void fokl_note_thread_cpu(int kind);

namespace {

constexpr int MT_N = 624, MT_SHIFT = 227;
constexpr int kSegBlocks = FOKL_SEGMENT_BLOCKS;
constexpr int kSegWords = kSegBlocks * MT_N;
constexpr int kSegDoubles = kSegWords / 2;
static_assert(kSegDoubles == FOKL_SEGMENT_DOUBLES, "include/fokl_hip_internal.h and this file disagree on the segment size");
constexpr int kSegSlots = kSegDoubles / 2;
constexpr int kSegMaskWords = kSegSlots / 64;
constexpr int kSegTail = 32;
constexpr int kTable = 8192;
constexpr int kAhead = 24;
constexpr int kAheadMax = 192;
constexpr uint64_t kLeadBit = FOKL_ROW_LEAD;
constexpr uint64_t kCachedHalf = FOKL_SOURCE_X1_HALF;
constexpr uint64_t kGivenGauss = FOKL_SOURCE_GIVEN;
constexpr uint64_t kFinalValue = FOKL_GAMMA_FINAL_VALUE;

static_assert(kSegSlots % 64 == 0, "mask words must not straddle segments");

#define FOKL_WIDE_TARGET __attribute__((target("avx512f,avx512dq,avx512vl,avx512bw,bmi,bmi2,popcnt,lzcnt")))

inline bool cpu_is_wide()
{
    static const bool wide = [] {
        const char *isa = std::getenv("FOKL_SAMPLER_ISA");
        if (isa && std::strcmp(isa, "base") == 0) return false;
        return __builtin_cpu_supports("avx512f") && __builtin_cpu_supports("avx512dq") &&
               __builtin_cpu_supports("avx512vl") && __builtin_cpu_supports("avx512bw") &&
               __builtin_cpu_supports("bmi2") && __builtin_cpu_supports("popcnt");
    }();
    return wide;
}

struct alignas(64) Segment {
    uint32_t buf[MT_N + kSegWords + kSegTail];
    alignas(64) uint64_t mask[2][kSegMaskWords];
    alignas(64) uint64_t g0[2][kSegMaskWords + 1];
    alignas(64) uint64_t g1[3][2][kSegMaskWords + 1];
    uint16_t cum[2][kSegMaskWords + 2];
    int32_t safe[2];
    int64_t index;
    std::atomic<int> ready;

    uint32_t *words() { return buf + MT_N; }
    const uint32_t *words() const { return buf + MT_N; }
};


inline uint32_t twist(uint32_t a, uint32_t b)
{
    const uint32_t y = (a & 0x80000000u) | (b & 0x7fffffffu);
    return (y >> 1) ^ ((0u - (y & 1u)) & 0x9908b0dfu);
}

void recurrence_portable(uint32_t *buf, int from, int to)
{
    for (int g = from; g < to; ++g) buf[g] = buf[g - MT_SHIFT] ^ twist(buf[g - MT_N], buf[g - MT_N + 1]);
}

FOKL_WIDE_TARGET void recurrence_wide(uint32_t *buf, int from, int to)
{
    const __m512i upper = _mm512_set1_epi32((int)0x80000000u), mag = _mm512_set1_epi32((int)0x9908b0dfu);
    const __m512i one = _mm512_set1_epi32(1);
    int g = from;
    if ((from & 15) == 0 && (reinterpret_cast<uintptr_t>(buf) & 63) == 0) {
        __m512i a = _mm512_load_si512(buf + g - MT_N);
        __m512i c_lo = _mm512_load_si512(buf + g - 240);
        for (; g + 16 <= to; g += 16) {
            const __m512i a_next = _mm512_load_si512(buf + g - MT_N + 16);
            const __m512i c_hi = _mm512_load_si512(buf + g - 224);
            const __m512i b = _mm512_alignr_epi32(a_next, a, 1);
            const __m512i c = _mm512_alignr_epi32(c_hi, c_lo, 13);
            const __m512i y = _mm512_ternarylogic_epi32(upper, a, b, 0xca);
            const __mmask16 odd = _mm512_test_epi32_mask(y, one);
            __m512i r = _mm512_xor_si512(c, _mm512_srli_epi32(y, 1));
            r = _mm512_mask_xor_epi32(r, odd, r, mag);
            _mm512_store_si512(buf + g, r);
            a = a_next;
            c_lo = c_hi;
        }
    }
// ... 157 lines not shown
            const __m512i c3 = _mm512_and_si512(s1, s2);
            alignas(64) uint64_t value[4][8], own[8];
            _mm512_store_si512(own, m);
            _mm512_store_si512(value[0], A1);
            _mm512_store_si512(value[1], _mm512_or_si512(_mm512_xor_si512(s1, s2), E5));
            _mm512_store_si512(value[2], _mm512_or_si512(_mm512_ternarylogic_epi64(c1, c2, c3, 0x96), E5));
            _mm512_store_si512(value[3], _mm512_or_si512(_mm512_ternarylogic_epi64(c1, c2, c3, 0xe8), E5));
            for (int k = 0; k < 8; ++k) {
                seg->cum[a][w0 + k] = (uint16_t)c;
                const int at = (int)(c >> 6), sh = (int)(c & 63);
                for (int pl = 0; pl < 4; ++pl) {
                    const uint64_t bits = _pext_u64(value[pl][k], own[k]);
                    planes[pl][at] |= bits << sh;
                    if (sh) planes[pl][at + 1] |= bits >> (64 - sh);
                }
                c += (uint32_t)__builtin_popcountll(own[k]);
            }
        }
        seg->cum[a][kSegMaskWords] = seg->cum[a][kSegMaskWords + 1] = (uint16_t)c;
        seg->safe[a] = (int32_t)seg->cum[a][kSegMaskWords - 1] +
                       __builtin_popcountll(M[kSegMaskWords - 1] & ((1ull << 40) - 1));
    }
}

std::mutex g_spare_m;
std::vector<Segment *> g_spares;
constexpr size_t kSpareMax = 1024;

Segment *take_segment()
{
    {
        std::lock_guard<std::mutex> lock(g_spare_m);
        if (!g_spares.empty()) {
            Segment *s = g_spares.back();
            g_spares.pop_back();
            return s;
        }
    }
    void *mem = nullptr;
    if (posix_memalign(&mem, 64, sizeof(Segment)) != 0) return nullptr;
    return new (mem) Segment;
}

void give_segment(Segment *s)
{
    if (!s) return;
    {
        std::lock_guard<std::mutex> lock(g_spare_m);
        if (g_spares.size() < kSpareMax) {
            g_spares.push_back(s);
            return;
        }
    }
    s->~Segment();
    std::free(s);
}

}

namespace {
struct WalkCrew;
}

struct fokl_stream {
    WalkCrew *crew = nullptr;
    uint32_t key0[MT_N];
    int pos0 = 0;
    int o = 0;
    std::mutex token_m;
    std::mutex room_m;
    std::condition_variable room_cv;
    std::atomic<int> sleepers{0};
    uint32_t carry[MT_N];
    int64_t next_raw = 0;
    int64_t oldest_alive = 0;
    std::atomic<int64_t> limit{kAhead};
    std::atomic<int> ahead{kAhead};
    std::atomic<int64_t> low_water{0};
    uint32_t *pre_ring = nullptr;
    int pre_entries = 0;
    std::atomic<int64_t> pre_published{0};
    bool stop = false;
    std::atomic<bool> stop_flag{false};
    std::vector<std::thread> threads;
    std::atomic<Segment *> table[kTable];
    std::atomic<int64_t> bulk_busy_ns{0}, segments_made{0};
    std::atomic<int64_t> token_ns{0}, token_recurrence_ns{0}, token_wait_ns{0};
    std::mutex hold_m;
    std::multiset<uint64_t> holds;
    uint64_t walker_floor = 0;
    uint64_t D = 0;
    int has_gauss = 0;
    uint64_t gauss_src = 0;
    double gauss0 = 0.0;
    std::atomic<int64_t> walker_wait_ns{0};
    std::atomic<int64_t> exact_draws{0}, gamma_draws{0};
    std::atomic<int64_t> rollbacks{0};
    std::atomic<int64_t> position_iterations{0};
    bool wide = false;
    std::string error;
};

namespace {

inline int64_t now_ns()
{
    return std::chrono::duration_cast<std::chrono::nanoseconds>(std::chrono::steady_clock::now().time_since_epoch())
        .count();
}

void update_low_water(fokl_stream *e)
{
    uint64_t d = e->walker_floor;
    if (!e->holds.empty()) d = std::min(d, *e->holds.begin());
    e->low_water.store((int64_t)(d / kSegDoubles), std::memory_order_release);
}

void generate_raw(fokl_stream *e, uint32_t *buf, int64_t index)
{
    int from = MT_N;
    if (index == 0) {
        std::memset(buf, 0, MT_N * sizeof(uint32_t));
        std::memcpy(buf + MT_N, e->key0, MT_N * sizeof(uint32_t));
        from = 2 * MT_N;
    } else {
        std::memcpy(buf, e->carry, MT_N * sizeof(uint32_t));
    }
    const int to = MT_N + kSegWords + kSegTail;
    if (e->wide)
        recurrence_wide(buf, from, to);
    else
        recurrence_portable(buf, from, to);
    std::memcpy(e->carry, buf + kSegWords, MT_N * sizeof(uint32_t));
    if (e->pre_ring) {
        constexpr int kRuns = kSegBlocks / FOKL_PRESTATE_BLOCKS;
        for (int run = 0; run < kRuns; ++run) {
            const int64_t entry_index = index * kRuns + run;
            uint32_t *entry = e->pre_ring + (size_t)(entry_index % e->pre_entries) * FOKL_PRESTATE_WORDS;
            const bool given = index == 0 && run == 0;
            std::memcpy(entry, given ? e->key0 : buf + (size_t)MT_N * FOKL_PRESTATE_BLOCKS * run, MT_N * sizeof(uint32_t));
            entry[MT_N] = (uint32_t)((uint64_t)entry_index & 0xffffffffu);
            entry[MT_N + 1] = (uint32_t)((uint64_t)entry_index >> 32);
            entry[MT_N + 2] = given ? 1u : 0u;
            entry[MT_N + 3] = (uint32_t)e->o;
        }
        e->pre_published.store(index + 1, std::memory_order_release);
    }
}

static const bool g_bulk_profile = std::getenv("FOKL_WALK_PROFILE") != nullptr;

void bulk_worker(fokl_stream *e)
{
    struct Note {
        ~Note() { fokl_note_thread_cpu(4); }
    } note;

    void *scratch_mem = nullptr;
    if (posix_memalign(&scratch_mem, 64, sizeof(uint32_t) * (size_t)(MT_N + kSegWords + kSegTail + 64)) != 0) {
        std::lock_guard<std::mutex> lock(e->token_m);
        e->error = "fokl_stream: out of memory";
        e->stop = true;
        e->stop_flag.store(true, std::memory_order_release);
        e->room_cv.notify_all();
        return;
    }
    struct Free {
        void *p;
        ~Free() { std::free(p); }
    } scratch_owner{scratch_mem};
    uint32_t *scratch = static_cast<uint32_t *>(scratch_mem);
    for (;;) {
        Segment *seg = take_segment();
        if (!seg) {
            std::lock_guard<std::mutex> lock(e->token_m);
            e->error = "fokl_stream: out of memory";
            e->stop = true;
            e->stop_flag.store(true, std::memory_order_release);
            e->room_cv.notify_all();
            return;
        }
        int64_t index = 0;
        std::vector<Segment *> retired;
        {
            const int64_t t_want = g_bulk_profile ? now_ns() : 0;
            std::unique_lock<std::mutex> lock(e->token_m);
            int64_t t_got = g_bulk_profile ? now_ns() : 0;
            if (g_bulk_profile) e->token_wait_ns.fetch_add(t_got - t_want, std::memory_order_relaxed);
            for (;;) {
                if (e->stop) {
                    give_segment(seg);
                    return;
                }
                const int64_t low = e->low_water.load(std::memory_order_acquire);
                if (e->next_raw < e->limit.load(std::memory_order_acquire) && e->next_raw - low < kTable - 2) break;
                const int64_t next = e->next_raw;
                lock.unlock();
                auto room_now = [&] {
                    return e->stop_flag.load(std::memory_order_seq_cst) ||
                           (next < e->limit.load(std::memory_order_seq_cst) &&
                            next - e->low_water.load(std::memory_order_seq_cst) < kTable - 2);
                };
                bool ready = false;
                for (int spins = 0, lim = fokl_spin_budget(400); spins < lim && !ready; ++spins) {
                    ready = room_now();
                    if (!ready) _mm_pause();
                }
                if (!ready) {
                    std::unique_lock<std::mutex> room(e->room_m);
                    e->sleepers.fetch_add(1, std::memory_order_seq_cst);
                    e->room_cv.wait(room, room_now);
                    e->sleepers.fetch_sub(1, std::memory_order_seq_cst);
                }
                lock.lock();
                if (g_bulk_profile) t_got = now_ns();
            }
            const int64_t low = e->low_water.load(std::memory_order_acquire);
            while (e->oldest_alive < low && e->oldest_alive < e->next_raw) {
                retired.push_back(e->table[e->oldest_alive % kTable].exchange(nullptr, std::memory_order_acq_rel));
                ++e->oldest_alive;
            }
            index = e->next_raw;
            seg->index = index;
            seg->ready.store(0, std::memory_order_relaxed);
            const int64_t t0 = now_ns();
            generate_raw(e, scratch, index);
            e->bulk_busy_ns.fetch_add(now_ns() - t0, std::memory_order_relaxed);
            ++e->next_raw;
            if (g_bulk_profile) {
                e->token_recurrence_ns.fetch_add(now_ns() - t0, std::memory_order_relaxed);
                e->token_ns.fetch_add(now_ns() - t_got, std::memory_order_relaxed);
            }
        }
        for (Segment *s : retired) give_segment(s);
        const int64_t t0 = now_ns();
        std::memcpy(seg->buf, scratch, MT_N * sizeof(uint32_t));
        if (e->wide)
            finish_segment_wide(seg, e->o, scratch + MT_N);
        else
            finish_segment_portable(seg, e->o, scratch + MT_N);
        seg->ready.store(1, std::memory_order_release);
        e->table[index % kTable].store(seg, std::memory_order_release);
        e->segments_made.fetch_add(1, std::memory_order_relaxed);
        e->bulk_busy_ns.fetch_add(now_ns() - t0, std::memory_order_relaxed);
    }
}

static const bool g_ahead_adapts = !(std::getenv("FOKL_STREAM_AHEAD") && std::strcmp(std::getenv("FOKL_STREAM_AHEAD"), "fixed") == 0);

Segment *segment_of(fokl_stream *e, uint64_t D, bool walker)
{
    const int64_t index = (int64_t)(D / kSegDoubles);
    Segment *seg = e->table[index % kTable].load(std::memory_order_acquire);
    if (seg && seg->index == index) return seg;
    const int ahead = e->ahead.load(std::memory_order_relaxed);
    if (walker && index + ahead > e->limit.load(std::memory_order_relaxed)) {
        e->limit.store(index + ahead, std::memory_order_seq_cst);
        if (e->sleepers.load(std::memory_order_seq_cst) > 0) {
            { std::lock_guard<std::mutex> lock(e->room_m); }
            e->room_cv.notify_all();
        }
    }
    const int64_t t0 = now_ns();
    for (int spins = 0;; ++spins) {
        seg = e->table[index % kTable].load(std::memory_order_acquire);
        if (seg && seg->index == index) break;
        if (spins < fokl_spin_budget(4000))
            _mm_pause();
        else
            std::this_thread::sleep_for(std::chrono::microseconds(5));
        if ((spins & 1023) == 1023 && e->stop_flag.load(std::memory_order_acquire)) return nullptr;
    }
    if (walker) {
        const int64_t waited = e->walker_wait_ns.fetch_add(now_ns() - t0, std::memory_order_relaxed) + (now_ns() - t0);
        const int64_t want = kAhead + 8 * (waited / 500000);
        if (want > ahead && ahead < kAheadMax && g_ahead_adapts) e->ahead.store((int)std::min<int64_t>(want, kAheadMax), std::memory_order_relaxed);
    }
    return seg;
}

struct Reader {
    fokl_stream *e;
    bool walker;
    int o;
    Segment *seg = nullptr;
    uint64_t lo = 1, hi = 0;
    bool failed = false;

    Reader(fokl_stream *engine, bool is_walker) : e(engine), walker(is_walker), o(engine->o) {}

    __attribute__((always_inline)) inline bool locate(uint64_t D)
    {
        if (D - lo < (uint64_t)kSegDoubles && seg) return true;
        return relocate(D);
    }

    __attribute__((noinline)) bool relocate(uint64_t D)
    {
        Segment *s = segment_of(e, D, walker);
        if (!s) {
            failed = true;
            return false;
        }
        seg = s;
        lo = (D / kSegDoubles) * kSegDoubles;
        hi = lo + kSegDoubles;
        if (walker) {
            const int64_t want = (int64_t)(D / kSegDoubles) + 1 + e->ahead.load(std::memory_order_relaxed);
            if (want > e->limit.load(std::memory_order_relaxed)) {
                e->limit.store(want, std::memory_order_seq_cst);
                if (e->sleepers.load(std::memory_order_seq_cst) > 0) {
                    { std::lock_guard<std::mutex> lock(e->room_m); }
                    e->room_cv.notify_all();
                }
            }
        }
        return true;
    }

    __attribute__((always_inline)) inline void prefetch_words(uint64_t D) const
    {
        if (D - lo >= (uint64_t)kSegDoubles) return;
        const char *p = reinterpret_cast<const char *>(seg->words() + o + 2 * (D - lo));
        __builtin_prefetch(p);
        __builtin_prefetch(p + 24);
    }

// ... 608 lines not shown
    const uint64_t slot = 64ull * wc + (uint64_t)_tzcnt_u64(_pdep_u64(1ull << (idx - cum[wc]), seg->mask[a][wc]));
    const uint64_t A = lo + 2 * slot + (uint64_t)a;
    if (hs) {
        const uint64_t *X = seg->mask[a ^ 1];
        uint64_t t = slot + 1 + (uint64_t)a;
        uint64_t mm = X[t >> 6] >> (t & 63);
        if (!mm) {
            t = (t | 63) + 1;
            mm = X[t >> 6];
        }
        t += (uint64_t)_tzcnt_u64(mm);
        const uint64_t Q = lo + 2 * t + (uint64_t)(a ^ 1);
        src[0] = A | kCachedHalf;
        up[0] = A + 2;
        src[1] = Q;
        up[1] = Q + 2;
        after = {Q + 3, Q, 1};
    } else {
        src[0] = A;
        up[0] = A + 2;
        src[1] = A | kCachedHalf;
        up[1] = A + 3;
        after = {A + 4, A, 0};
    }
}

static const bool g_prefetch_second = !(std::getenv("FOKL_WALK_PREFETCH") && std::strcmp(std::getenv("FOKL_WALK_PREFETCH"), "first") == 0);

FOKL_WIDE_TARGET static inline void block_positions(const BlockIn &in, BlockOut &out, int o)
{
    uint32_t wc = in.wc0;
    uint64_t D = in.D0, gsrc = in.gsrc0;
    const bool stream_rows = g_row_stream && (reinterpret_cast<uintptr_t>(in.rows) & 31) == 0;
    for (int i = 0; i < in.count; ++i) {
        const int lead = in.h[i];
        iteration_sites(in.seg, in.lo, in.a, wc, in.e[i], in.hs[i], out.source + 2 * i, out.upos + 2 * i, out.after[i]);
        const __m256i rowv = _mm256_set_epi64x((long long)out.source[2 * i + 1], (long long)out.source[2 * i],
                                               (long long)(lead ? gsrc : 0), (long long)(D | (lead ? kLeadBit : 0)));
        if (stream_rows)
            _mm256_stream_si256(reinterpret_cast<__m256i *>(in.rows + i), rowv);
        else
            _mm256_storeu_si256(reinterpret_cast<__m256i *>(in.rows + i), rowv);
        D = out.after[i].D;
        gsrc = out.after[i].gauss_src;
        const char *site = reinterpret_cast<const char *>(in.seg->words() + o + 2 * ((out.source[2 * i] & ~kCachedHalf) - in.lo));
        __builtin_prefetch(site);
        __builtin_prefetch(site + 24);
        if (g_prefetch_second) {
            const char *site2 = reinterpret_cast<const char *>(in.seg->words() + o + 2 * ((out.source[2 * i + 1] & ~kCachedHalf) - in.lo));
            __builtin_prefetch(site2 + 24);
        }
    }
}

constexpr int kCrewRing = 16;
static const int g_crew_depth = [] {
    const char *v = std::getenv("FOKL_CREW_DEPTH");
    const int n = v ? std::atoi(v) : 8;
    return n >= 2 && n <= kCrewRing ? n : 8;
}();
constexpr int kCrewMax = 4;

struct alignas(64) CrewSlot {
    BlockIn in;
    int redo = -1;
    IterationStart redo_from{};
    int64_t exact = 0;
    alignas(64) std::atomic<uint64_t> ready{0};
    alignas(64) std::atomic<uint64_t> done{0};
};

struct WalkCrew {
    fokl_stream *e = nullptr;
    int helpers = 0;
    CrewSlot slots[kCrewRing];
    uint64_t issued = 0;
    alignas(64) std::atomic<uint64_t> claimed{0};
    std::unique_ptr<BlockOut> walker_out;
    alignas(64) std::atomic<bool> stop{false};
    std::atomic<int> sleepers{0};
    std::mutex m;
    std::condition_variable cv;
    std::vector<std::thread> threads;
    std::vector<int> cpus;
};

FOKL_WIDE_TARGET static void crew_process(WalkCrew *crew, uint64_t n, BlockOut &out, Walk &checker)
{
    CrewSlot &slot = crew->slots[n % kCrewRing];
    const BlockIn &in = slot.in;
    const int o = crew->e->o;
    checker.r.failed = false;
    const int64_t t0 = g_walk_profile ? now_ns() : 0;
    block_positions(in, out, o);
    const int64_t t1 = g_walk_profile ? now_ns() : 0;
    const __m512d bvec = _mm512_setr_pd(in.b_sig, in.b_tau, in.b_sig, in.b_tau, in.b_sig, in.b_tau, in.b_sig, in.b_tau);
    const __m512d cvec = _mm512_setr_pd(in.c_sig, in.c_tau, in.c_sig, in.c_tau, in.c_sig, in.c_tau, in.c_sig, in.c_tau);
    int64_t exact = 0;
    const int redo = check_tests(checker, o, out.source, out.upos, in.count, bvec, cvec, in.b_sig, in.c_sig, in.b_tau, in.c_tau,
                                 exact);
    if (g_walk_profile) {
        g_walk_ns[1].fetch_add(t1 - t0, std::memory_order_relaxed);
        g_walk_ns[2].fetch_add(now_ns() - t1, std::memory_order_relaxed);
    }
    slot.redo = redo;
    slot.exact = exact;
    if (redo > 0)
        slot.redo_from = out.after[redo - 1];
    else if (redo == 0)
        slot.redo_from = {in.D0, in.gsrc0, (int)in.h[0]};
    _mm_sfence();
    slot.done.store(n, std::memory_order_release);
}

static inline uint64_t crew_claim(WalkCrew *crew)
{
    uint64_t n = crew->claimed.load(std::memory_order_acquire);
    while (crew->slots[(n + 1) % kCrewRing].ready.load(std::memory_order_acquire) == n + 1)
        if (crew->claimed.compare_exchange_weak(n, n + 1, std::memory_order_acq_rel)) return n + 1;
    return 0;
}

FOKL_WIDE_TARGET void crew_helper(WalkCrew *crew, int which)
{
    struct Note {
        ~Note() { fokl_note_thread_cpu(0); }
    } note;
    if (which < (int)crew->cpus.size() && crew->cpus[(size_t)which] >= 0) {
        cpu_set_t set;
        CPU_ZERO(&set);
        CPU_SET(crew->cpus[(size_t)which], &set);
        (void)sched_setaffinity(0, sizeof(set), &set);
    }
    Walk checker(crew->e, Walk::ReaderOnly{});
    std::unique_ptr<BlockOut> out(new BlockOut());
    for (;;) {
        uint64_t n = 0;
        for (int spins = 0; (n = crew_claim(crew)) == 0; ++spins) {
            if (crew->stop.load(std::memory_order_acquire)) return;
            if (spins < fokl_spin_budget(20000)) {
                _mm_pause();
            } else {
                std::unique_lock<std::mutex> lock(crew->m);
                crew->sleepers.fetch_add(1, std::memory_order_seq_cst);
                crew->cv.wait(lock, [&] {
                    if (crew->stop.load(std::memory_order_seq_cst)) return true;
                    const uint64_t c = crew->claimed.load(std::memory_order_seq_cst);
                    return crew->slots[(c + 1) % kCrewRing].ready.load(std::memory_order_seq_cst) == c + 1;
                });
                crew->sleepers.fetch_sub(1, std::memory_order_seq_cst);
                spins = 0;
            }
        }
        crew_process(crew, n, *out, checker);
    }
}

void crew_stop(fokl_stream *e)
{
    WalkCrew *crew = e->crew;
    if (!crew) return;
    {
        std::lock_guard<std::mutex> lock(crew->m);
        crew->stop.store(true, std::memory_order_seq_cst);
    }
    crew->cv.notify_all();
    for (auto &t : crew->threads) t.join();
    delete crew;
    e->crew = nullptr;
}

FOKL_WIDE_TARGET static inline void prefetch_crossing(fokl_stream *e, Walk &w, int p1)
{
    if (!w.r.seg || w.D - w.r.lo >= (uint64_t)kSegDoubles) return;
    const Segment *seg = w.r.seg;
    const uint64_t q = (w.D - w.r.lo) >> 1;
    const size_t word = (size_t)(q >> 6);
    __builtin_prefetch(&seg->mask[0][word]);
    __builtin_prefetch(&seg->mask[1][word]);
    if (word + 8 < (size_t)kSegMaskWords) {
        __builtin_prefetch(&seg->mask[0][word + 8]);
        __builtin_prefetch(&seg->mask[1][word + 8]);
    }
    const uint64_t site = (w.D - w.r.lo) + (uint64_t)(1.27 * (p1 + 1));
    const char *words = reinterpret_cast<const char *>(seg->words() + e->o);
    const Segment *next = e->table[(seg->index + 1) % kTable].load(std::memory_order_acquire);
    if (next && next->index != seg->index + 1) next = nullptr;
    for (int line = -2; line <= 3; ++line) {
        const int64_t d = (int64_t)site + 8 * line;
        if (d < 0) continue;
        if (d < kSegDoubles)
            __builtin_prefetch(words + 8 * d);
        else if (next)
            __builtin_prefetch(reinterpret_cast<const char *>(next->words() + e->o) + 8 * (d - kSegDoubles));
    }
    if (next && site + 512 >= (uint64_t)kSegDoubles) {
        for (int a = 0; a < 2; ++a) {
            __builtin_prefetch(&next->mask[a][0]);
            __builtin_prefetch(&next->cum[a][0]);
            __builtin_prefetch(&next->g0[a][0]);
            __builtin_prefetch(&next->g1[0][a][0]);
            __builtin_prefetch(&next->g1[1][a][0]);
            __builtin_prefetch(&next->g1[2][a][0]);
        }
        __builtin_prefetch(&next->safe[0]);
    }
}

static const bool g_crew_inline = !(std::getenv("FOKL_CREW_INLINE") && std::strcmp(std::getenv("FOKL_CREW_INLINE"), "0") == 0);

FOKL_WIDE_TARGET int walk_tape_crew(fokl_stream *e, int p1, int draws, double astar, double atau_star, fokl_tape_row *rows,
                                    int32_t *progress)
{
    WalkCrew *crew = e->crew;
    const int64_t t_enter = g_walk_profile ? now_ns() : 0;
    int64_t idle_ns = 0;
    Walk w(e);
    const double b_sig = astar - 1.0 / 3.0, c_sig = 1.0 / std::sqrt(9 * b_sig);
    const double b_tau = atau_star - 1.0 / 3.0, c_tau = 1.0 / std::sqrt(9 * b_tau);
    int64_t exact = 0, rolled_back = 0, by_position = 0;
    int k = 0, k_issued = 0, published = 0;
    auto publish = [&](int upto) {
        const int whole = upto == draws ? draws : upto - upto % FOKL_TAPE_BLOCK;
        if (progress && whole > published) __atomic_store_n(progress, whole, __ATOMIC_RELEASE);
        published = std::max(published, whole);
    };
    uint64_t first_open = crew->issued + 1;
    std::deque<uint64_t> inline_after;
    Walk lender(e, Walk::ReaderOnly{});
    auto wait_done = [&](uint64_t n) -> CrewSlot & {
        CrewSlot &slot = crew->slots[n % kCrewRing];
        int64_t idle_from = 0;
        for (int spins = 0; slot.done.load(std::memory_order_acquire) != n; ++spins) {
            if (const uint64_t mine = crew_claim(crew)) {
                if (idle_from) idle_ns += now_ns() - idle_from;
                idle_from = 0;
                crew_process(crew, mine, *crew->walker_out, lender);
                spins = 0;
            } else if (spins < 50000) {
                if (g_walk_profile && !idle_from) idle_from = now_ns();
                _mm_pause();
            } else {
                std::this_thread::yield();
            }
        }
        if (idle_from) idle_ns += now_ns() - idle_from;
        return slot;
    };
    auto judge_oldest = [&]() -> bool {
// ... 231 lines not shown
}

inline uint64_t walker_reach(const fokl_stream *e)
{
    return e->has_gauss && e->gauss_src != kGivenGauss ? std::min(e->D, e->gauss_src) : e->D;
}

}

extern "C" int fokl_stream_create(const uint32_t *mt_key, int32_t mt_pos, int32_t has_gauss, double gauss_cache,
                                  int bulk_threads, uint32_t *prestate_ring, int prestate_entries, fokl_stream **out)
{
    if (!out || !mt_key || mt_pos < 0 || mt_pos > MT_N || bulk_threads < 1 || bulk_threads > 16 ||
        (prestate_ring && prestate_entries < 4 * kAheadMax * (kSegBlocks / FOKL_PRESTATE_BLOCKS))) {
        fokl_set_global_error("fokl_stream_create: null pointer, invalid MT19937 position or thread count");
        return FOKL_ERR_ARG;
    }
    auto *e = new fokl_stream();
    std::memcpy(e->key0, mt_key, sizeof(e->key0));
    e->pos0 = mt_pos;
    e->o = mt_pos & 1;
    e->D = (uint64_t)(mt_pos >> 1);
    e->walker_floor = e->D;
    e->has_gauss = has_gauss ? 1 : 0;
    e->gauss_src = kGivenGauss;
    e->gauss0 = gauss_cache;
    e->pre_ring = prestate_ring;
    e->pre_entries = prestate_ring ? prestate_entries : 0;
    e->wide = cpu_is_wide();
    for (auto &t : e->table) t.store(nullptr, std::memory_order_relaxed);
    try {
        for (int i = 0; i < bulk_threads; ++i) e->threads.emplace_back(bulk_worker, e);
    } catch (const std::exception &ex) {
        {
            std::lock_guard<std::mutex> lock(e->token_m);
            e->stop = true;
        }
        {
            std::lock_guard<std::mutex> room(e->room_m);
            e->stop_flag.store(true, std::memory_order_release);
        }
        e->room_cv.notify_all();
        for (auto &t : e->threads) t.join();
        delete e;
        fokl_set_global_error(std::string("fokl_stream_create: ") + ex.what());
        return FOKL_ERR_STATE;
    }
    *out = e;
    return FOKL_OK;
}

extern "C" void fokl_stream_destroy(fokl_stream *e)
{
    if (!e) return;
    if (g_walk_profile && g_walk_iterations.load() > 0) {
        const double n = (double)g_walk_iterations.exchange(0);
        std::fprintf(stderr, "fokl_stream: rank walk, %.0f iterations: chase %.2f positions %.2f tests %.2f ns per iteration; "
                             "position walk %.0f iterations, %.1f ns each\n", n, g_walk_ns[0].exchange(0) / n,
                     g_walk_ns[1].exchange(0) / n, g_walk_ns[2].exchange(0) / n, (double)g_walk_by_position.load(),
                     g_walk_ns[3].exchange(0) / std::max(1.0, (double)g_walk_by_position.load()));
        g_walk_by_position.store(0);
        if (g_crew_tapes.load() > 0)
            std::fprintf(stderr, "fokl_stream: walk crew: %lld tapes, the walking thread inside them %.3f ms, of which waiting for a "
                                 "verdict with no block to take %.3f ms\n", (long long)g_crew_tapes.exchange(0),
                         g_crew_wall_ns.exchange(0) / 1e6, g_crew_idle_ns.exchange(0) / 1e6);
    }
    if (g_walk_profile && e->segments_made.load() > 0) {
        const double n = (double)e->segments_made.load();
        std::fprintf(stderr, "fokl_stream: %.0f segments; per segment: token held %.2f us (recurrence + pre-states %.2f), waited for "
                             "the token %.2f us, all of the bulk phase %.2f us; walker waited %.2f ms, ahead %d\n", n,
                     e->token_ns.load() / 1e3 / n, e->token_recurrence_ns.load() / 1e3 / n, e->token_wait_ns.load() / 1e3 / n,
                     e->bulk_busy_ns.load() / 1e3 / n, e->walker_wait_ns.load() / 1e6, e->ahead.load());
    }
    {
        std::lock_guard<std::mutex> lock(e->token_m);
        e->stop = true;
    }
    {
        std::lock_guard<std::mutex> room(e->room_m);
        e->stop_flag.store(true, std::memory_order_release);
    }
    e->room_cv.notify_all();
    crew_stop(e);
    for (auto &t : e->threads) t.join();
    for (auto &t : e->table) give_segment(t.exchange(nullptr));
    delete e;
}

extern "C" int fokl_stream_place_bulk(fokl_stream *e, const int32_t *cpus, int count)
{
    if (!e || !cpus || count < 1) {
        fokl_set_global_error("fokl_stream_place_bulk: null pointer or no CPUs");
        return FOKL_ERR_ARG;
    }
    int failed = 0;
    for (size_t i = 0; i < e->threads.size(); ++i) {
        cpu_set_t set;
        CPU_ZERO(&set);
        const int cpu = (int)cpus[i % (size_t)count];
        if (cpu < 0 || cpu >= CPU_SETSIZE) continue;
        CPU_SET(cpu, &set);
        failed += pthread_setaffinity_np(e->threads[i].native_handle(), sizeof(set), &set) != 0;
    }
    if (failed) {
        fokl_set_global_error("fokl_stream_place_bulk: pthread_setaffinity_np failed");
        return FOKL_ERR_STATE;
    }
    return FOKL_OK;
}

extern "C" int fokl_stream_set_helpers(fokl_stream *e, int count, const int32_t *cpus)
{
    if (!e || count < 0) {
        fokl_set_global_error("fokl_stream_set_helpers: null stream or negative count");
        return FOKL_ERR_ARG;
    }
    crew_stop(e);
    if (count == 0 || !e->wide) return FOKL_OK;
    auto *crew = new WalkCrew();
    crew->e = e;
    crew->helpers = std::min(count, kCrewMax);
    crew->walker_out.reset(new BlockOut());
    for (int i = 0; i < crew->helpers; ++i) crew->cpus.push_back(cpus ? (int)cpus[i] : -1);
    e->crew = crew;
    try {
        for (int i = 0; i < crew->helpers; ++i) crew->threads.emplace_back(crew_helper, crew, i);
    } catch (const std::exception &ex) {
        crew_stop(e);
        fokl_set_global_error(std::string("fokl_stream_set_helpers: ") + ex.what());
        return FOKL_ERR_STATE;
    }
    return FOKL_OK;
}

extern "C" int fokl_stream_walk(fokl_stream *e, int p1, int draws, double astar, double atau_star, fokl_tape_row *rows,
                                double *gam_sig, double *gam_tau, int32_t *progress)
{
    if (!e || p1 <= 0 || draws < 0 || !rows || !gam_sig || !gam_tau) {
        fokl_set_global_error("fokl_stream_walk: null pointer or empty model");
        if (progress) __atomic_store_n(progress, -1, __ATOMIC_RELEASE);
        return FOKL_ERR_ARG;
    }
    if (!(astar >= 0.0) || !(atau_star >= 0.0)) {
        fokl_set_global_error("fokl_stream_walk: gamma shape parameter is negative or NaN");
        if (progress) __atomic_store_n(progress, -1, __ATOMIC_RELEASE);
        return FOKL_ERR_NUMERIC;
    }
    return e->wide ? walk_tape_wide(e, p1, draws, astar, atau_star, rows, gam_sig, gam_tau, progress)
                   : walk_tape_base(e, p1, draws, astar, atau_star, rows, gam_sig, gam_tau, progress);
}

extern "C" int64_t fokl_stream_prestates_published(const fokl_stream *e)
{
    return e ? e->pre_published.load(std::memory_order_acquire) : 0;
}

extern "C" double fokl_stream_given_gauss(const fokl_stream *e) { return e ? e->gauss0 : 0.0; }

extern "C" int fokl_stream_tell(const fokl_stream *e, fokl_stream_cursor *out)
{
    if (!e || !out) {
        fokl_set_global_error("fokl_stream_tell: null pointer");
        return FOKL_ERR_ARG;
    }
    out->position = e->D;
    out->has_gauss = e->has_gauss;
    out->gauss_source = e->gauss_src;
    return FOKL_OK;
}
// ... 241 lines not shown
```

### fokl_gpy_amd/engine.py

```python
import collections
import itertools
import threading
import math
import os
import time

import numpy as np
from scipy.linalg import eigh as _eigh

from . import _capi

SLOT_ONES, SLOT_Y, SLOT_FIRST_FREE = _capi.SLOT_ONES, _capi.SLOT_Y, _capi.SLOT_FIRST_FREE
from .host_pipeline import (
    HostPipeline, ShardedSpectralJob, GibbsOutcome, EagerOutcome, NativeOutcome, NativeSpectrum, Misprediction, ModelSize,
    chain_engine_for, spectral_engine_for,
    close_chain_engines, drop_spare_buffers, _mark, _flush_marks, _cpu_budget, _thread_plan, _thread_spares,
    _place_host_threads, _SPARES)



def distinct_arrangements(indvec):
    cur = sorted(float(v) for v in indvec)
    n = len(cur)
    rows = [tuple(cur)]
# ... 789 lines not shown
                and os.environ.get('FOKL_STATS', 'native') == 'native'
                and not os.environ.get('FOKL_POOL_TRACE')):
            self._nrun = _capi.NativeRun(
                self.backend, getattr(self.backend, 'kernel_id', getattr(self.backend, 'kernel', 1)),
                m=self.m, n_phis=self.n_phis, way3=int(self.way3), tolerance=self.tolerance, gimmie=int(bool(self.gimmie)),
                draws=self.draws, half0=int(math.ceil(self.draws / 2)), lookahead=self.lookahead,
                lookahead_native=self._lookahead_native, foresight=self.foresight,
                speculate_across=int(self._speculate_across), forecast_early=int(self._forecast_early),
                forecast_polls=0 if os.environ.get('FOKL_SYNC') == 'blocking' else self._forecast_polls,
                matrix_free=int(self._matrix_free), update_from=0, update_depth=0, update_lookahead=0,
                head_start=int(os.environ.get('FOKL_HEAD_START', '1') != '0'), slot_capacity=self.pool.capacity)
        self.stats['t_head_start'] = time.perf_counter() - t_begin_run
        if (self._nrun is None and pipelined and hasattr(self.backend, 'gram_launch')
                and not (self.allreduce or self.candidate_sharded)
                and os.environ.get('FOKL_HEAD_START', '1') != '0'):
            base = self.backend.gram([SLOT_ONES, SLOT_Y], [SLOT_ONES, SLOT_Y], False)
            self._head = (base, self._build_ahead(next(self._patterns())[1], [SLOT_ONES]))
        if pipelined:
            try:
                replicated = self.allreduce or self.candidate_sharded
                self._replicated_native = replicated and self._native_planned()
                if self.allow_device_chains and (not replicated or self._replicated_native):
                    self.chain_engine = chain_engine_for(getattr(getattr(self.backend, 'ctx', None), 'device', None))
                    if self.chain_engine is not None:
                        self.device_chain_columns = min(self.device_chain_columns,
                                                        getattr(self.chain_engine, 'max_columns', 768))
                    self._dchain_stats0 = self.chain_engine.stats() if self.chain_engine is not None else {}
                wide = self.m * (self.m - 1) * (self.m - 2 if self.way3 else 1) >= 1000
                self.host = HostPipeline(self.stream, self.draws,
                                         self.comm if self.candidate_sharded and not self._replicated_native else None,
                                         chain_engine=self.chain_engine, wide_models=wide,
                                         device=getattr(getattr(self.backend, 'ctx', None), 'device', None))
            except (ImportError, KeyError, AttributeError, _capi.FoklNativeError) as exc:
                import warnings
                warnings.warn(f"host thread pipeline unavailable ({exc}); running the search in line", RuntimeWarning)
                self.host = None
        self.stats['t_pool_create'] = time.perf_counter() - t_begin_run
        if self.host is not None and self._native_wanted():
            try:
                half0 = int(math.ceil(self.draws / 2))
                self.native = _capi.NativeSearch(
                    self.host.pool, self.chain_engine, n=self.n, a=self.a, b=self.b, atau=self.atau, btau=self.btau,
                    threshav=self.threshav, threshstda=self.threshstda, threshstdb=self.threshstdb,
                    guess_margin=self.guess_margin, draws=self.draws, half0=half0, aic=int(self.aic),
                    lookahead=self._lookahead_native, foresight=self.foresight, speculation_max=self._speculation_native,
                    tentative_tapes=int(self.tentative_tapes), test_rewinds=int(self._test_rewinds),
                    device_chain_columns=self.device_chain_columns, finish_threads=self.host.pool.finish_threads,
                    flip_guess=self._flip_guess, device_rows=int(self.host.device_rows))
                self.spectral_engine = None
                if not self.allreduce and not self.candidate_sharded:
                    self.spectral_engine = spectral_engine_for(getattr(getattr(self.backend, 'ctx', None), 'device', None))
                if self.spectral_engine is not None:
                    everything = os.environ.get('FOKL_EIGH') == 'device'
                    self.native.bind_spectral(self.spectral_engine,
                                              slack=0.0 if everything else float(os.environ.get('FOKL_DSPECTRAL_SLACK', '-1')),
                                              lookahead=int(os.environ.get('FOKL_DSPECTRAL_LOOKAHEAD', '-1')))
                update_from = int(os.environ.get('FOKL_EIGH_UPDATE', '8'))
                direct_wanted = os.environ.get('FOKL_KILL_DECIDE', 'direct') == 'direct' and \
                    getattr(self, 'allow_direct_decisions', True)
                if update_from > 0 and getattr(self.host.pool, 'has_dgemm', False) \
                        and (direct_wanted or not (self.allreduce or self.candidate_sharded)) \
                        and os.environ.get('FOKL_EIGH_SIGNS', 'canonical') != 'lapack':
                    derived_ahead = 0 if 'FOKL_LOOKAHEAD' in os.environ else _bounded_lookahead(
                        'FOKL_LOOKAHEAD_DERIVED', os.environ.get('FOKL_LOOKAHEAD_DERIVED', '0'))
                    depth_default = '24' if os.environ.get('FOKL_KILL_DECIDE', 'direct') == 'direct' and \
                        getattr(self, 'allow_direct_decisions', True) else '6'
                    self._update_args = (update_from, int(os.environ.get('FOKL_EIGH_UPDATE_DEPTH', depth_default)),
                                         derived_ahead)
                    self.native.set_update(*self._update_args)
                    self.stats['eigh_update_from'] = update_from
                decide = os.environ.get('FOKL_KILL_DECIDE', 'direct')
                if decide not in ('direct', 'g2'):
                    raise ValueError("FOKL_KILL_DECIDE must be direct or g2")
                if not getattr(self, 'allow_direct_decisions', True):
                    decide = 'g2'
                self.native.set_decide(1 if decide == 'direct' else 0, float(os.environ.get('FOKL_KILL_DECIDE_TOL', '0')))
                self.stats['kill_decide'] = decide
                if self.allreduce or self.candidate_sharded:
                    self.native.set_deterministic(True)
            except BaseException:
                if self.native is not None:
                    self.native.close()
                    self.native = None
                self.host.close()
                self.host = None
                if self._head is not None:
                    self._ahead_block(self._head[1])
                    self.pool.give(self._head[1]['slots'])
                    self._head = None
                raise
        self.stats['search_driver'] = 'native' if self.native is not None else 'python'
        if self.native is None and self.host is not None and os.environ.get('FOKL_SEARCH', 'native') != 'python':
            import warnings
            warnings.warn("the native search driver is not available for this search (FOKL_KILL_BIC / FOKL_SEARCH_DIST / a "
                          "stand-in chain engine): it runs on the Python statement of the loop, several times slower -- "
                          "fit_stats['search_driver'] says which", RuntimeWarning)
        _mark('pool_up')
        dgemm0 = _capi.device_dgemm_stats() if self.host is not None else (0, 0, 0)
        self.stats['t_pool_up'] = time.perf_counter() - t_begin_run
        self.stats['finish_log'] = os.environ.get('FOKL_FINISH_LOG', 'fast')
        self.stats['chain_mode'] = 'device' if self.chain_engine is not None else 'host'
        self.stats['eigh_mode'] = (os.environ.get('FOKL_EIGH', 'host') if getattr(self, 'spectral_engine', None) is not None
                                   and self.native is not None else 'host')
        t_up = time.perf_counter()
        try:
            return self._run()
        finally:
            _mark('run_end')
            t_down = time.perf_counter()
            self.stats['t_search_body'] = t_down - t_up
            if self.native is not None:
                for key, value in self.native.stats().items():
                    self.stats[key] = self.stats.get(key, 0) + value
                self.trace = self.native.trace()
                self._outcomes, self._retiring = [], []
                self.native.close()
                self.native = None
                self.stats['t_teardown_search'] = time.perf_counter() - t_down
            if self.host is not None:
                for job in self._device_jobs:
                    job.release()
                self._device_jobs = []
                self._zombies.clear()
                self._unverified.clear()
                if self.chain_engine is not None:
                    now = self.chain_engine.stats()
                    self.stats.update({'dchain_' + k: v - self._dchain_stats0.get(k, 0) for k, v in now.items()})
                t_close = time.perf_counter()
                busy = self.host.close()
                self.stats['t_teardown_pool'] = time.perf_counter() - t_close
                dgemm1 = _capi.device_dgemm_stats()
                self.stats.update(eigen_update_products=dgemm1[0] - dgemm0[0], eigen_update_products_on_device=dgemm1[1] - dgemm0[1],
                                  eigen_update_products_fell_back=dgemm1[2] - dgemm0[2])
                self.stats.update(pool_bulk_s=busy.get('bulk', 0.0), walker_wait_s=busy.get('walker_wait', 0.0),
                                  stream_segments=busy.get('stream_segments', 0),
                                  gamma_attempts_exact=busy.get('gamma_attempts_exact', 0),
                                  pool_noise_s=busy['noise'], pool_chain_s=busy['chain'],
                                  pool_finish_s=busy['finish'], pool_spectral_s=busy['spectral'],
                                  noise_queue_wait_s=busy['noise_queue_wait'],
                                  noise_verdict_wait_s=busy['noise_verdict_wait'],
                                  host_chains_segmented=busy.get('host_chains_segmented', 0),
                                  host_chain_recuts=busy.get('host_chain_recuts', 0),
                                  spectral_remote=self.host.remote_results, exchanges=self.host.exchanges,
                                  spectral_submitted=self.stats.get('spectral_submitted', 0) + self.host.spectral_submitted)
                self.host = None
                self.stats['t_teardown'] = time.perf_counter() - t_down
                _mark('pool_down')
                _flush_marks()

    def _native_wanted(self):
        if not self._native_planned():
            return False
        if self.chain_engine is not None and not isinstance(self.chain_engine, _capi.DeviceChainEngine):
            return False
        return True

    def _native_planned(self):
        from . import host_pipeline
        if os.environ.get('FOKL_SEARCH', 'native') == 'python':
            return False
        if (self.allreduce or self.candidate_sharded) and os.environ.get('FOKL_SEARCH_DIST', 'native') == 'python':
            return False
        if self.kill_bic not in ('auto', 'gram'):
            return False
        return host_pipeline._chain_engine_factory is None

    def _patterns(self):
        m = self.m
        sett = 1 if m == 1 else (3 if self.way3 else 2)
        ind = 1
        while True:
            indvec = deal_indvec(ind, m, sett)
            while True:
                yield ind, list(indvec)
                if not advance_indvec(indvec, m, self.way3):
                    break
            ind += 1
            if ind > self.n_phis:
                return

    def _candidate_split(self):
        return self._replicated_native and self.candidate_sharded and not self.allreduce

    def _share_of(self, slots):
        world, rank = self.comm.world, self.comm.rank
        share = -(-len(slots) // world)
        mine = list(slots[rank * share:(rank + 1) * share])
        mine += [slots[-1]] * (share - len(mine))
        return mine, share

    def _gather_rows(self, local, total, share):
        t0 = time.perf_counter()
        parts = self.comm.allgather(np.ascontiguousarray(local).reshape(-1)).reshape(self.comm.world, share, -1)
        self.stats['candidate_gathers'] = self.stats.get('candidate_gathers', 0) + 1
        self.stats['t_candidate_gather'] = self.stats.get('t_candidate_gather', 0.0) + time.perf_counter() - t0
        return np.concatenate([parts[r, :max(0, min(share, total - r * share))] for r in range(self.comm.world)], axis=0)

    def _gram_of_new_columns(self, new_slots, col_slots):
        if not self._candidate_split():
            return self.backend.gram(new_slots, col_slots, self.allreduce)
        mine, share = self._share_of(new_slots)
        return self._gather_rows(self.backend.gram(mine, col_slots, False), len(new_slots), share)

    def _arrangements(self, indvec):
        key = tuple(float(v) for v in indvec)
        hit = self._arrangement_memo.get(key)
        if hit is None:
            hit = self._arrangement_memo[key] = distinct_arrangements(indvec)
            hit.setflags(write=False)
        return hit

    def _build_ahead(self, indvec, active_slots):
# ... 323 lines not shown
```

### fokl_gpy_amd/host_pipeline.py

```python
import os
import threading
import time

import numpy as np

from . import _capi

_TRACE_PATH = os.environ.get('FOKL_POOL_TRACE')
_trace_log = []


def _mark(tag, info=''):
    if _TRACE_PATH:
        _trace_log.append((time.monotonic_ns(), tag, info))


def _flush_marks():
    if _TRACE_PATH and _trace_log:
        with open(_TRACE_PATH, 'a') as f:
            for t, tag, info in _trace_log:
                f.write(f"driver {t} {tag} {info}\n")
        del _trace_log[:]


# ... 145 lines not shown
    if budget is None:
        budget = _cpu_budget()
    default = (3 if wide_models else 4) if budget >= 12 else (2 if budget >= 5 else 1)
    return max(1, int(os.environ.get('FOKL_BULK_THREADS', str(default))))


def _thread_plan(wide_models=False):
    budget = _cpu_budget()
    exact_log = os.environ.get('FOKL_FINISH_LOG', 'fast') == 'exact'
    if budget >= 12 and wide_models:
        plan = (2, 3 if exact_log else 1, 11)
    elif budget >= 12:
        plan = (2, 3 if exact_log else 2, 8)
    elif budget >= 8:
        plan = (1, 2 if exact_log else 1, 5)
    elif budget >= 5:
        plan = (1, 2 if exact_log else 1, 3)
    elif budget >= 4:
        plan = (1, 1, 2)
    elif budget >= 3:
        plan = (1, 0, 2)
    else:
        plan = (1, 0, 1)
    names = ('FOKL_CHAIN_THREADS', 'FOKL_FINISH_THREADS', 'FOKL_SPECTRAL_THREADS')
    chain, finish, spectral = (int(os.environ.get(name, str(default))) for name, default in zip(names, plan))
    return max(1, chain), max(0, finish), max(1, spectral)


class Misprediction(RuntimeError):
    """A kill-test decision that was taken from a guess (the intercept's posterior mean ~ its least-squares value) before
    the chain that decides it had run turned out wrong when the chain arrived.  Every guess is verified; the caller
    (FoKL._search) restores the random stream and repeats the search without guessing."""


class ModelSize(int):
    __slots__ = ()


_CHAIN_ENGINES = {}
_chain_engine_factory = None


def chain_engine_for(device):
    mode = os.environ.get('FOKL_CHAIN', 'auto')
    if mode not in ('auto', 'device', 'host'):
        raise ValueError("FOKL_CHAIN must be auto, device or host")
    if mode == 'host':
        return None
    if _chain_engine_factory is not None:
        return _chain_engine_factory()
    if device is None:
        if mode == 'device':
            raise RuntimeError("FOKL_CHAIN=device: the backend has no HIP device")
        return None
    engine = _CHAIN_ENGINES.get(device)
    if engine is None:
        try:
            engine = _capi.DeviceChainEngine(device, int(os.environ.get('FOKL_DCHAIN_SLOTS', '128')))
        except _capi.FoklNativeError:
            if mode == 'device':
                raise
            return None
        _CHAIN_ENGINES[device] = engine
    return engine


_SPECTRAL_ENGINES = {}


def spectral_engine_for(device):
    mode = os.environ.get('FOKL_EIGH', 'host')
    if mode not in ('device', 'hybrid', 'host'):
        raise ValueError("FOKL_EIGH must be host, hybrid or device")
    if mode == 'host' or os.environ.get('FOKL_EIGH_SIGNS', 'canonical') == 'lapack':
        return None
    if device is None:
        raise RuntimeError("FOKL_EIGH=device: the backend has no HIP device")
    engine = _SPECTRAL_ENGINES.get(device)
    if engine is None:
        engine = _SPECTRAL_ENGINES[device] = _capi.DeviceSpectralEngine(device)
    return engine


def close_chain_engines():
    for engine in list(_CHAIN_ENGINES.values()) + list(_SPECTRAL_ENGINES.values()):
        engine.close()
    _CHAIN_ENGINES.clear()
    _SPECTRAL_ENGINES.clear()


import atexit
atexit.register(close_chain_engines)


class _SpareAccount:
    doubles = 0
    limit = int(float(os.environ.get('FOKL_HOST_POOL_MB', '2048')) * 131072)


_SPARES = _SpareAccount()
_SPARE_LISTS = threading.local()


def _thread_spares():
    spares = getattr(_SPARE_LISTS, 'by_class', None)
    if spares is None:
        spares = _SPARE_LISTS.by_class = {}
    return spares


def drop_spare_buffers():
    spares = _thread_spares()
    _SPARES.doubles = max(0, _SPARES.doubles - sum(raw.shape[0] for stack in spares.values() for raw in stack))
    spares.clear()


class HostPipeline:

    def __init__(self, stream, draws, comm=None, chain_engine=None, wide_models=False, device=None):
        self.stream, self.draws = stream, int(draws)
        self.dchain = chain_engine
        self._pinned = chain_engine is not None and getattr(chain_engine, 'wants_pinned_tapes', True)
        forced = os.environ.get('FOKL_CANDIDATE_SHARD_FORCE', '0') == '1'
        self.comm = comm if comm is not None and (comm.world > 1 or forced) else None
        self._seq = 0
        self._windows = {}
        self.remote_results = self.exchanges = self.spectral_submitted = 0
        self._saved_affinity, noise_cpu = None, -1
        if os.environ.get('FOKL_PIN_L3', '1') != '0':
            self._saved_affinity, noise_cpu = _place_host_threads()
        chain, finish, spectral = _thread_plan(wide_models)
        self.device_rows = False
        prestates = None
        if isinstance(chain_engine, _capi.DeviceChainEngine) and os.environ.get('FOKL_DCHAIN_ROWS', '1') != '0':
            try:
                prestates = chain_engine.prestate_ring()
            except _capi.FoklNativeError:
                prestates = None
        try:
            dgemm_from = int(os.environ.get('FOKL_EIGH_DGEMM_FROM', '0'))
            bulk = _bulk_threads(wide_models=wide_models)
            self.pool = _capi.HostPool(stream, chain, finish, spectral, noise_cpu, bulk_threads=bulk,
                                       prestates=prestates,
                                       device_dgemm=(device, dgemm_from) if device is not None and dgemm_from > 0 else None)
            if prestates is not None:
                chain_engine.bind(self.pool.stream_handle())
                self.device_rows = True
            helpers = int(os.environ.get('FOKL_WALK_HELPERS', str(0 if wide_models else _walk_helpers_default())))
            if helpers > 0:
                cpus = None
                if self._saved_affinity is not None and os.environ.get('FOKL_WALK_CPUS', 'other') != 'same':
                    picked = _other_cores(self._saved_affinity, os.sched_getaffinity(0), spectral + helpers)
                    if picked is not None:
                        cpus = picked[-helpers:]
                try:
                    self.pool.set_walk_helpers(helpers, cpus)
                except _capi.FoklNativeError:
                    pass
            if (self._saved_affinity is not None and _cpu_budget() >= 12 and os.environ.get('FOKL_BULK_CPUS', 'other') != 'same'):
                picked = _other_cores(self._saved_affinity, os.sched_getaffinity(0), spectral + max(0, helpers) + bulk)
                if picked is not None:
                    try:
                        self.pool.place_bulk_threads(picked[-bulk:])
                    except _capi.FoklNativeError:
                        pass
            if self._saved_affinity is not None and os.environ.get('FOKL_SPECTRAL_DOMAIN', '1') != '0':
                other = None
                if os.environ.get('FOKL_SPECTRAL_DOMAIN', '1') != 'domain' and spectral > 0:
                    other = _spectral_cpus(self._saved_affinity, os.sched_getaffinity(0), spectral)
                if other is None:
                    other = _second_domain(self._saved_affinity, os.sched_getaffinity(0))
                if other:
                    try:
                        self.pool.spectral_affinity(other)
                    except _capi.FoklNativeError:
                        pass
        except BaseException:
            self._restore_affinity()
            raise
        self._live = []
        self._reap_at = 24
        self._spare = _thread_spares()

    CLASS_DOUBLES = 65536

    def _take(self, doubles):
        cls = -(-doubles // self.CLASS_DOUBLES)
        spare = self._spare.get(cls)
        if spare:
            _SPARES.doubles -= cls * self.CLASS_DOUBLES
            return spare.pop()
        if self._pinned:
            try:
                return _capi.pinned_empty(cls * self.CLASS_DOUBLES)
            except _capi.FoklNativeError:
                self._pinned = False
        return np.empty(cls * self.CLASS_DOUBLES, dtype=np.float64)

    def give(self, raw):
        if _SPARES.doubles + raw.shape[0] <= _SPARES.limit:
            _SPARES.doubles += raw.shape[0]
            self._spare.setdefault(raw.shape[0] // self.CLASS_DOUBLES, []).append(raw)

    def _reap(self):
        live = []
        for job in self._live:
            if job.done():
                if job.recycle:
                    for entry in job.recycle:
                        self._retire_buffer(entry)
                    job.recycle = job.keep = None
            else:
                live.append(job)
        self._live = live

    def _retire_buffer(self, entry):
        if isinstance(entry, tuple):
            raw, reader = entry
            if reader.done():
                self.give(raw)
            else:
                reader.recycle.append(raw)
        else:
            self.give(entry)

    def _hand_tape(self, noise_job, owner):
        raw, noise_job.held = noise_job.held, None
        if raw is None:
            return
        reader = noise_job.co_reader
        entry = raw if reader is None or reader is owner else (raw, reader)
        if owner.recycle is None:
            if owner._h is None:
                self._retire_buffer(entry)
                return
            owner.recycle = []
        owner.recycle.append(entry)

    def _track(self, job):
        if len(self._live) >= self._reap_at:
            self._reap()
            self._reap_at = max(24, len(self._live) + 12)
        self._live.append(job)
        return job

    def request(self, p1, astar, atau_star, tentative=False, finish=True):
        raw = self._take(_capi.NoiseTape.doubles_needed(p1, self.draws))
        job = self.pool.submit_noise(_capi.NoiseTape(p1, self.draws, raw), astar, atau_star, tentative, finish=finish)
        job.held = raw
        return self._track(job)

    def abandon(self, noise_job):
        self._hand_tape(noise_job, noise_job)

    def discard(self, noise_job):
        noise_job.resolve(False)
        self._hand_tape(noise_job, noise_job)

    def spectral(self, gram, idx):
        idx = np.ascontiguousarray(idx, dtype=np.int32)
        self.spectral_submitted += 1
        if self.comm is None:
            return self._track(self.pool.submit_spectral(gram, idx, gram.shape[0] - 1))
        seq, self._seq = self._seq, self._seq + 1
        local = None
        if seq % self.comm.world == self.comm.rank:
            local = self._track(self.pool.submit_spectral(gram, idx, gram.shape[0] - 1))
        job = ShardedSpectralJob(self, seq, idx.shape[0], local)
        self._windows.setdefault(seq // self.comm.world, []).append(job)
        return job

    def _exchange(self, window):
        jobs = self._windows.pop(window)
        length = max(_capi.SpectralResult.doubles(job.p1) for job in jobs)
        send = np.zeros(length)
        failure = None
        for job in jobs:
            if job.local is not None:
                try:
                    res = job.local.wait()
                    send[:res._buf.shape[0]] = res._buf
                    job.result = res
                except _capi.FoklNativeError as exc:
                    failure = exc
                    send[:] = np.nan
        gathered = self.comm.allgather(send)
        self.exchanges += 1
        for job in jobs:
            owner = job.seq % self.comm.world
            if np.isnan(gathered[owner, 0]):
                raise RuntimeError(f"candidate-sharded search: rank {owner} could not diagonalise model {job.seq} "
                                   f"({job.p1} columns)") from failure
            if job.result is None:
                need = _capi.SpectralResult.doubles(job.p1)
                job.result = _capi.SpectralResult(job.p1, np.array(gathered[owner, :need]))
                self.remote_results += 1

    def chain(self, spec, b, btau, dtd, sigsqd0, tausqd0, noise_job):
        tape = noise_job.result
        w_raw = self._take(tape.draws * tape.p1)
        job = self.pool.submit_chain(spec.lamb, spec.qty, b, btau, dtd, sigsqd0, tausqd0, tape, w_raw)
        job.recycle = []
        self._hand_tape(noise_job, job)
        return self._track(job), w_raw

    def chain_device(self, spec, b, btau, dtd, sigsqd0, tausqd0, noise_job, stat_first):
        try:
            job = self.dchain.submit(spec.lamb, spec.qty, b, btau, dtd, sigsqd0, tausqd0, noise_job.result, stat_first)
        except _capi.FoklNativeError as exc:
            if exc.code == -3:
                return None
            raise
        job.recycle = []
        self._hand_tape(noise_job, job)
        return self._track(job)

    def chain_ahead(self, spec, b, btau, dtd, sigsqd0, tausqd0, noise_job):
        tape = noise_job.result
        w_raw = self._take(tape.draws * tape.p1)
        job = self.pool.submit_chain(spec.lamb, spec.qty, b, btau, dtd, sigsqd0, tausqd0, tape, w_raw)
        job.recycle = []
        job.ignore_failure = True
        return self._track(job), w_raw

    def adopt(self, chain_job, noise_job):
        chain_job.ignore_failure = False
        self._hand_tape(noise_job, chain_job)

    def disown(self, chain_job, w_raw, noise_job):
        if chain_job.done():
            self.give(w_raw)
        else:
            chain_job.recycle.append(w_raw)
            noise_job.co_reader = chain_job

    def close(self):
        for job in self._live:
            if job.unresolved:
                job.resolve(False)
        for job in self._live:
            if not (isinstance(job, _capi.DeviceChainJob) and job.done()):
                job.wait()
        _mark('jobs_drained')
        self._reap()
        self._live = []
        busy = self.pool.busy_seconds()
        if self.device_rows:
            self.dchain.bind(None)
            self.device_rows = False
        self.pool.close()
        self._restore_affinity()
        return busy

    def _restore_affinity(self):
        if self._saved_affinity is not None:
            try:
                os.sched_setaffinity(0, self._saved_affinity)
            except OSError:
                pass
            self._saved_affinity = None


class ShardedSpectralJob:
    __slots__ = ('owner', 'seq', 'p1', 'local', 'result')

    def __init__(self, owner, seq, p1, local):
        self.owner, self.seq, self.p1, self.local, self.result = owner, seq, p1, local, None

    def wait(self):
        if self.result is None:
            self.owner._exchange(self.seq // self.owner.comm.world)
        return self.result


class GibbsOutcome:
    __slots__ = ('lamb', 'qty', 'Qt', 'betahat', 'ev', 'idx', 'intercept_scale', 'siglik', '_jobs', '_owner', '_w',
                 '_betas', '_w_raw', '_chain_job', 'on_device', 'checks', '_release_wanted', '_dtd')

    def __init__(self, owner, spec, ev, idx, noise_job, chain_job, w_raw):
        self.lamb, self.qty, self.Qt, self.betahat = spec.lamb, spec.qty, spec.Qt, spec.betahat
        self.ev, self.idx = ev, idx
        self._jobs, self._owner = (noise_job, chain_job), owner
        self._w = self._betas = self.intercept_scale = None
        self.siglik = 0.0
        self._w_raw, self._chain_job = w_raw, chain_job
        self.on_device = isinstance(chain_job, _capi.DeviceChainJob)
        self.checks = []
        self._release_wanted = False
        self._dtd = None

    def release(self):
        if self.on_device:
            if self.checks:
                self._release_wanted = True
                return
            self._w = self._jobs = None
            self._owner._release_device_job(self._chain_job)
            return
        raw, self._w_raw = self._w_raw, None
        host = self._owner.host
        if raw is None or host is None:
            return
        self._w = self._jobs = None
        if self._chain_job.done():
            host.give(raw)
        else:
            self._chain_job.recycle.append(raw)

    def intercept_scale_on_host(self, first_row):
        o = self._owner
        noise_job, chain_job = self._jobs
        noise_job.wait()
        tape = noise_job.result
        chain = _capi.gibbs_chain_from_finished_tape if tape.finishing_requested else _capi.gibbs_chain_from_tape
        w, negative = chain(self.lamb, self.qty, o.b, o.btau, self._dtd, o.sigsqd0, o.tausqd0, tape, follow=True)
        if negative:
            raise RuntimeError("bstar < 0 inside the Gibbs chain (only possible with b <= 0): the noise tape "
                               "cannot reproduce the reference's skipped draw (FR:1538-1539)")
        return abs(float(np.mean(w[first_row:] @ self.Qt[:, 0])))

    def chain_ready(self):
        return self._w is not None or self.intercept_scale is not None or self._chain_job.done()

    def mean_intercept_draw(self, first_row):
        if self.on_device:
            o = self._owner
            t0 = time.perf_counter()
            mean_w, negative = self._chain_job.wait()
            o.stats['t_chain'] += time.perf_counter() - t0
            o.stats['dchain_kernel_s'] += getattr(self._chain_job, 'kernel_seconds', 0.0)
            o.stats['dchain_timed'] += 1
            if negative[0]:
                raise RuntimeError("bstar < 0 inside the Gibbs chain (only possible with b <= 0): the noise tape "
                                   "cannot reproduce the reference's skipped draw (FR:1538-1539)")
# ... 167 lines not shown
```

### include/fokl_hip_internal.h

```cpp
#ifndef FOKL_HIP_INTERNAL_H
#define FOKL_HIP_INTERNAL_H

#include <stddef.h>

#include "fokl_hip.h"

#ifdef __cplusplus
extern "C" {
#endif


#define FOKL_SEGMENT_BLOCKS 256
#define FOKL_SEGMENT_DOUBLES 79872
#define FOKL_ROW_LEAD (1ull << 63)
#define FOKL_SOURCE_X1_HALF (1ull << 63)
#define FOKL_SOURCE_GIVEN ((1ull << 62) - 1)
#define FOKL_GAMMA_FINAL_VALUE (~0ull)
#define FOKL_PRESTATE_WORDS 640
#define FOKL_PRESTATE_BLOCKS 32
typedef struct fokl_stream fokl_stream;
typedef struct fokl_tape_row {
    uint64_t start;
    uint64_t lead_source;
    uint64_t gamma[2];
} fokl_tape_row;
typedef struct fokl_stream_cursor {
    uint64_t position;
    uint64_t gauss_source;
    int32_t has_gauss;
} fokl_stream_cursor;
int fokl_stream_create(const uint32_t *mt_key, int32_t mt_pos, int32_t has_gauss, double gauss_cache, int bulk_threads,
                       uint32_t *prestate_ring, int prestate_entries, fokl_stream **out);
int64_t fokl_stream_prestates_published(const fokl_stream *stream);
double fokl_stream_given_gauss(const fokl_stream *stream);
void fokl_stream_destroy(fokl_stream *stream);
int fokl_stream_walk(fokl_stream *stream, int p1, int draws, double astar, double atau_star, fokl_tape_row *rows,
                     double *gam_sig, double *gam_tau, int32_t *progress);
int fokl_stream_tell(const fokl_stream *stream, fokl_stream_cursor *out);
int fokl_stream_seek(fokl_stream *stream, const fokl_stream_cursor *at);
int fokl_stream_hold(fokl_stream *stream, uint64_t *position_out);
int fokl_stream_release(fokl_stream *stream, uint64_t position);
int fokl_stream_advance_floor(fokl_stream *stream);
int fokl_stream_state(fokl_stream *stream, uint32_t *key_out, int32_t *pos_out, int32_t *has_gauss_out,
                      double *gauss_out);
int fokl_stream_expand(fokl_stream *stream, int p1, double astar, double atau_star, const fokl_tape_row *rows, int k0,
                       int k1, double *normals_out, double *pair_r2_out, int32_t *lead_out, double *gam_sig_out,
                       double *gam_tau_out);
int fokl_stream_set_helpers(fokl_stream *stream, int count, const int32_t *cpus);
int fokl_stream_place_bulk(fokl_stream *stream, const int32_t *cpus, int count);
int fokl_stream_stats(const fokl_stream *stream, double *bulk_busy_s, double *walker_wait_s, int64_t *segments,
                      int64_t *gamma_attempts, int64_t *gamma_attempts_exact);
double fokl_stream_fast_ln_error(int64_t n);


typedef struct fokl_host_pool fokl_host_pool;
typedef struct fokl_host_job fokl_host_job;

int fokl_pool_create(int chain_threads, int finish_threads, int spectral_threads, int bulk_threads, int noise_cpu,
                     void *dsyevr, uint32_t *mt_key, int32_t *mt_pos, int32_t *has_gauss, double *gauss_cache,
                     uint32_t *prestate_ring, int prestate_entries, fokl_host_pool **out);
int fokl_pool_use_dsyevd(fokl_host_pool *pool, void *fn, int from_columns);
int fokl_pool_use_dgemm(fokl_host_pool *pool, void *fn);
void fokl_device_dgemm(char *transa, char *transb, int *m, int *n, int *k, double *alpha, double *a, int *lda, double *b,
                       int *ldb, double *beta, double *c, int *ldc);
int fokl_device_dgemm_configure(int device, void *host_dgemm, int from, void **entry);
int fokl_device_dgemm_stats(int64_t *calls, int64_t *on_device, int64_t *failed);

int fokl_pool_spectral_affinity(fokl_host_pool *pool, const int32_t *cpus, int count);
fokl_stream *fokl_pool_stream(fokl_host_pool *pool);
void fokl_pool_destroy(fokl_host_pool *pool);
int fokl_tape_ready(const int32_t *progress, int draws, const int32_t *block_done, int block);

int fokl_pool_submit_noise(fokl_host_pool *pool, int p1, int draws, double astar, double atau_star, fokl_tape_row *rows,
                           double *normals, double *pair_r2, int32_t *lead, double *gam_sig, double *gam_tau,
                           int32_t *progress, int tentative, int32_t *block_done, int block, int finish,
                           uint64_t *span_out, fokl_host_job **out);
int fokl_pool_release_hold(fokl_host_pool *pool, uint64_t position);
int fokl_pool_resolve(fokl_host_job *job, int commit);
int fokl_pool_submit_chain(fokl_host_pool *pool, const double *lamb, const double *qty, int p1, double b, double btau,
                           double dtd, double sigsqd0, double tausqd0, int draws, const double *normals,
                           const double *pair_r2, const int32_t *lead, const double *gam_sig, const double *gam_tau,
                           const int32_t *progress, int32_t *block_done, int block, int finishing_requested,
                           double *w_out, int32_t *bstar_negative, void (*then)(void *), void *then_arg, fokl_host_job **out);
int fokl_pool_submit_spectral(fokl_host_pool *pool, const double *gram, int ld, const int32_t *idx, int p1, int ycol,
                              double *lamb_out, double *qt_out, double *qty_out, double *betahat_out,
                              double *moments_out, fokl_host_job **out);
int fokl_pool_submit_spectral_update(fokl_host_pool *pool, const double *gram, int ld, const int32_t *idx, int p1, int ycol,
                                     const double *parent_lamb, const double *parent_qt, int parent_pos,
                                     fokl_host_job *parent_job, double *lamb_out, double *qt_out, double *qty_out,
                                     double *betahat_out, double *moments_out, int32_t *updated, fokl_host_job **out);
int fokl_pool_poll(const fokl_host_job *job);
int fokl_pool_wait(fokl_host_job *job);
int fokl_pool_busy_seconds(const fokl_host_pool *pool, double *noise, double *chain, double *finish,
                           double *spectral);
int fokl_pool_stream_stats(const fokl_host_pool *pool, double *bulk_busy_s, double *walker_wait_s, int64_t *segments,
                           int64_t *gamma_attempts, int64_t *gamma_attempts_exact);
int fokl_pool_noise_waits(const fokl_host_pool *pool, double *queue_wait, double *verdict_wait);
int fokl_thread_cpu_seconds(double *seconds, int count);


#define FOKL_CHAIN_SEGMENTS 8
#define FOKL_CHAIN_WARM 64

int fokl_gibbs_chain_segments_host(const double *lamb, const double *qty, int p1, double b, double btau, double dtd,
                                   double sigsqd0, double tausqd0, int draws, const double *normals,
                                   const double *gam_sig, const double *gam_tau, const int32_t *block_done, int block,
                                   double *w_out, double *sigs_out, double *taus_out, int32_t *bstar_negative,
                                   int segments, int warm, int32_t *bad_cut);
int fokl_pool_chain_segments(const fokl_host_pool *pool, int64_t *segmented, int64_t *recuts);


typedef struct fokl_dchain fokl_dchain;
typedef struct fokl_search fokl_search;
typedef struct fokl_spectrum fokl_spectrum;
typedef struct fokl_tape fokl_tape;
typedef struct fokl_outcome fokl_outcome;
typedef struct fokl_search_params {
    int64_t n;
    double a, b, atau, btau;
    double threshav, threshstda, threshstdb;
    double guess_margin;
    int32_t draws;
    int32_t half0;
    int32_t aic;
    int32_t lookahead, foresight;
    int32_t speculation_max;
    int32_t tentative_tapes, test_rewinds;
    int32_t device_chain_columns;
    int32_t finish_threads;
    int32_t flip_guess;
    int32_t device_rows;
} fokl_search_params;
int fokl_search_create(fokl_host_pool *pool, fokl_dchain *dchain, const fokl_search_params *params, fokl_search **out);
typedef struct fokl_dspectral fokl_dspectral;
int fokl_search_bind_spectral(fokl_search *search, fokl_dspectral *engine, int max_columns, double slack, int lookahead);
int fokl_search_hold_spectral(fokl_search *search, int hold);
int fokl_search_set_update(fokl_search *search, int from_columns, int depth, int lookahead);
int fokl_search_set_decide(fokl_search *search, int mode, double tolerance);
int fokl_search_set_deterministic(fokl_search *search, int on);
void fokl_search_destroy(fokl_search *search);
const char *fokl_search_error(const fokl_search *search);
int fokl_search_mispredicted(const fokl_search *search);
int fokl_search_set_substage(fokl_search *search, const int64_t *term_ids, int columns);
int fokl_search_speculate(fokl_search *search, const int32_t *sizes, const int32_t *is_model, int count);
int fokl_search_drop_speculation(fokl_search *search);
int fokl_search_spectral(fokl_search *search, const double *gram, int ld, const int32_t *idx, int p1, fokl_spectrum **out);
int fokl_search_spectral_from(fokl_search *search, const double *gram, int ld, const int32_t *idx, int p1,
                              fokl_spectrum *parent, int parent_pos, fokl_spectrum **out);
int fokl_spectrum_done(fokl_spectrum *spectrum);
int fokl_spectrum_wait(fokl_search *search, fokl_spectrum *spectrum, const double **buffer, int *p1);
int fokl_spectrum_retain(fokl_search *search, fokl_spectrum *spectrum);
void fokl_spectrum_release(fokl_search *search, fokl_spectrum *spectrum);
int fokl_search_model_begin(fokl_search *search, const double *gram, int ld, const int32_t *idx, int p1,
// ... 216 lines not shown
```

Before: 583,300.

## Keep host thread pool alive across fits with park/resume instead of recreate

Adds end_fit/begin_fit on the host pool and a reset for the RNG stream engine, so a finished fit parks its worker threads, affinity setup and LAPACK bindings and the next fit with a matching plan reuses them. The goal is to avoid creating and joining threads and reapplying CPU placement on every fit. Per-thread CPU accounting moves from destructor notes to pthread CPU clocks, and an outstanding-job counter lets the pool drain before parking. It also caches scipy LAPACK function addresses. The risk is stale state between fits and more complex lifecycle handling when devices close.

```diff
diff --git a/fokl_gpy_amd/_capi.py b/fokl_gpy_amd/_capi.py
--- a/fokl_gpy_amd/_capi.py
+++ b/fokl_gpy_amd/_capi.py
@@ -88,6 +88,8 @@
     'fokl_pool_spectral_affinity': (c_int, [c_vp, c_vp, c_int]),
     'fokl_pool_release_hold': (c_int, [c_vp, ctypes.c_uint64]),
     'fokl_pool_destroy': (None, [c_vp]),
+    'fokl_pool_end_fit': (c_int, [c_vp]),
+    'fokl_pool_begin_fit': (c_int, [c_vp, c_vp, c_vp, c_vp, c_vp, c_vp, c_int]),
     'fokl_pool_submit_noise': (c_int, [c_vp, c_int, c_int, c_dbl, c_dbl, c_vp, c_vp, c_vp, c_vp, c_vp, c_vp, c_vp, c_int,
                                        c_vp, c_int, c_int, c_vp, c_vp]),
     'fokl_tape_ready': (c_int, [c_vp, c_int, c_vp, c_int]),
@@ -109,6 +111,7 @@
     'fokl_stream_prestates_published': (c_i64, [c_vp]),
     'fokl_stream_given_gauss': (c_dbl, [c_vp]),
     'fokl_stream_destroy': (None, [c_vp]),
+    'fokl_stream_reset': (c_int, [c_vp, c_vp, c_i32, c_i32, c_dbl, c_vp, c_int]),
     'fokl_stream_walk': (c_int, [c_vp, c_int, c_int, c_dbl, c_dbl, c_vp, c_vp, c_vp, c_vp]),
     'fokl_stream_tell': (c_int, [c_vp, c_vp]),
     'fokl_stream_seek': (c_int, [c_vp, c_vp]),
@@ -503,6 +506,11 @@
                                             prestates[1] if prestates else 0, ctypes.byref(h)))
         self._h = h
 
+    def reset(self, stream, prestates=None):
+        _check(self._lib.fokl_stream_reset(self._h, _ptr(stream.key), stream.pos, stream.has_gauss, stream.cache,
+                                           prestates[0] if prestates else None, prestates[1] if prestates else 0))
+        self.stream = stream
+
     def close(self, write_back=True):
         if self._h:
             if write_back:
@@ -628,6 +636,16 @@
 
 
 
+_SCIPY_ADDRESSES = {}
+
+
+def _scipy_address(name):
+    if name not in _SCIPY_ADDRESSES:
+        _SCIPY_ADDRESSES[name] = {'dsyevr': _scipy_dsyevr_address, 'dsyevd': _scipy_dsyevd_address,
+                                  'dgemm': _scipy_dgemm_address}[name]()
+    return _SCIPY_ADDRESSES[name]
+
+
 def _scipy_dsyevd_address():
     try:
         from scipy.linalg import cython_lapack
@@ -733,23 +751,32 @@
         self.stream = stream
         self._h = None
         h = c_vp(0)
-        fn = _scipy_dsyevr_address() if spectral_threads > 0 else None
+        fn = _scipy_address('dsyevr') if spectral_threads > 0 else None
         self.finish_threads = int(finish_threads)
+        self.spectral_threads = int(spectral_threads)
+        self.parked = False
         _check(self._lib.fokl_pool_create(int(chain_threads), self.finish_threads, int(spectral_threads),
                                           max(1, int(bulk_threads)), int(noise_cpu), c_vp(fn),
                                           *stream.args(), prestates[0] if prestates else None,
                                           prestates[1] if prestates else 0, ctypes.byref(h)))
         self._h = h
+        self._bind_lapack(device_dgemm)
+
+    def _bind_lapack(self, device_dgemm):
+        spectral_threads = self.spectral_threads
         self.dsyevd_from = 0
         dc_from = int(os.environ.get('FOKL_EIGH_DC_FROM', '80'))
+        fd = None
         if spectral_threads > 0 and dc_from > 0 and os.environ.get('FOKL_EIGH_SIGNS', 'canonical') != 'lapack':
-            fd = _scipy_dsyevd_address()
-            if fd:
-                _check(self._lib.fokl_pool_use_dsyevd(self._h, c_vp(fd), dc_from))
-                self.dsyevd_from = dc_from
+            fd = _scipy_address('dsyevd')
+        if fd:
+            _check(self._lib.fokl_pool_use_dsyevd(self._h, c_vp(fd), dc_from))
+            self.dsyevd_from = dc_from
+        elif spectral_threads > 0:
+            _check(self._lib.fokl_pool_use_dsyevd(self._h, None, 0))
         self.has_dgemm = False
         if spectral_threads > 0:
-            fg = _scipy_dgemm_address()
+            fg = _scipy_address('dgemm')
             self.device_dgemm_from = 0
             if fg and device_dgemm is not None:
                 entry = c_vp(0)
@@ -783,6 +810,19 @@
             self._h = None
 
     __del__ = close
+
+    def end_fit(self):
+        _check(self._lib.fokl_pool_end_fit(self._h))
+        self.parked, self.stream = True, None
+
+    def begin_fit(self, stream, prestates=None, device_dgemm=None):
+        _check(self._lib.fokl_pool_begin_fit(self._h, *stream.args(), prestates[0] if prestates else None,
+                                             prestates[1] if prestates else 0))
+        self.parked, self.stream = False, stream
+        self._bind_lapack(device_dgemm)
+
+    def abandon(self):
+        self._h = None
 
     def submit_noise(self, tape, astar, atau_star, tentative=False, finish=False):
         h = c_vp(0)
@@ -1250,6 +1290,14 @@
         self.keep = self._area = self._flag = None
 
 
+before_device_close = []
+
+
+def _device_closes(device):
+    for hook in list(before_device_close):
+        hook(device)
+
+
 class DeviceChainEngine:
     max_columns = 768
 
@@ -1263,6 +1311,7 @@
 
     def close(self):
         if self._h:
+            _device_closes(self.device)
             self._lib.fokl_dchain_destroy(self._h)
             self._h = None
 
@@ -1576,6 +1625,7 @@
 
     def close(self):
         if getattr(self, '_h', None) is not None and self._h:
+            _device_closes(self.device)
             self._lib.fokl_ctx_destroy(self._h)
             self._h = None
 
diff --git a/fokl_gpy_amd/csrc/fokl_hostpool.cpp b/fokl_gpy_amd/csrc/fokl_hostpool.cpp
--- a/fokl_gpy_amd/csrc/fokl_hostpool.cpp
+++ b/fokl_gpy_amd/csrc/fokl_hostpool.cpp
@@ -34,14 +34,26 @@
 
 static std::atomic<int64_t> g_thread_cpu_ns[8];
 
-extern "C" __attribute__((visibility("hidden"))) void fokl_note_thread_cpu(int kind)
-{
-    timespec ts;
-    if (kind >= 0 && kind < 8 && clock_gettime(CLOCK_THREAD_CPUTIME_ID, &ts) == 0)
-        g_thread_cpu_ns[kind].fetch_add((int64_t)ts.tv_sec * 1000000000LL + ts.tv_nsec, std::memory_order_relaxed);
-}
-
 extern "C" __attribute__((visibility("hidden"))) int64_t fokl_dchain_dispatcher_cpu_ns();
+
+extern "C" __attribute__((visibility("hidden"))) void fokl_stream_note_cpu(fokl_stream *stream);
+extern "C" __attribute__((visibility("hidden"))) void fokl_stream_park(fokl_stream *stream);
+
+__attribute__((visibility("hidden"))) void fokl_note_threads_cpu(std::vector<std::thread> &threads, std::vector<int64_t> &noted,
+                                                                 int kind)
+{
+    noted.resize(threads.size(), 0);
+    for (size_t i = 0; i < threads.size(); ++i) {
+        clockid_t clock;
+        timespec ts;
+        if (kind < 0 || kind >= 8 || !threads[i].joinable() || pthread_getcpuclockid(threads[i].native_handle(), &clock) != 0 ||
+            clock_gettime(clock, &ts) != 0)
+            continue;
+        const int64_t ns = (int64_t)ts.tv_sec * 1000000000LL + ts.tv_nsec;
+        g_thread_cpu_ns[kind].fetch_add(ns - noted[i], std::memory_order_relaxed);
+        noted[i] = ns;
+    }
+}
 
 extern "C" int fokl_thread_cpu_seconds(double *seconds, int count)
 {
@@ -55,11 +67,6 @@
 }
 
 namespace {
-
-struct ThreadCpuNote {
-    int kind;
-    ~ThreadCpuNote() { fokl_note_thread_cpu(kind); }
-};
 
 using dsyevr_fn = void (*)(char *jobz, char *range, char *uplo, int *n, double *a, int *lda, double *vl, double *vu,
                            int *il, int *iu, double *abstol, int *m, double *w, double *z, int *ldz, int *isuppz,
@@ -131,6 +138,8 @@
     Queue noise_q, chain_q, spectral_q;
     std::deque<Queue> finish_q;
     std::vector<std::thread> threads;
+    std::vector<int> thread_kinds;
+    std::vector<int64_t> thread_noted_ns;
     std::vector<size_t> spectral_thread_ids;
     dsyevr_fn dsyevr = nullptr;
     dsyevd_fn dsyevd = nullptr;
@@ -138,6 +147,9 @@
     dgemm_fn dgemm = nullptr;
     std::mutex dep_m;
     fokl_stream *stream = nullptr;
+    std::atomic<int64_t> outstanding{0};
+    std::atomic<int64_t> fit_begin_ns{0};
+    bool parked = false;
     uint32_t *mt_key = nullptr;
     int32_t *mt_pos = nullptr, *has_gauss = nullptr;
     double *gauss_cache = nullptr;
@@ -151,7 +163,7 @@
     std::condition_variable start_cv;
     std::string trace_path;
     std::vector<std::array<int64_t, 7>> trace;
-    int test_delay_us = 0;
+    std::atomic<int> test_delay_us{0};
     bool lapack_signs = false;
     double singular = 1e-9;
 };
@@ -172,6 +184,7 @@
     {
         std::lock_guard<std::mutex> lock(pool->done_m);
         job->done.store(1, std::memory_order_release);
+        pool->outstanding.fetch_sub(1, std::memory_order_acq_rel);
     }
     pool->done_cv.notify_all();
 }
@@ -628,7 +641,6 @@
 
 void worker(fokl_host_pool *pool, Queue *queue)
 {
-    ThreadCpuNote note{queue == &pool->chain_q ? 1 : queue == &pool->spectral_q ? 3 : 2};
     prctl(PR_SET_TIMERSLACK, 2000UL, 0, 0, 0);
     for (;;) {
         fokl_host_job *job;
@@ -668,6 +680,7 @@
     {
         std::lock_guard<std::mutex> lock(pool->done_m);
         job->done.store(1, std::memory_order_release);
+        pool->outstanding.fetch_sub(1, std::memory_order_acq_rel);
     }
     pool->done_cv.notify_all();
 }
@@ -742,7 +755,6 @@
 
 void noise_worker(fokl_host_pool *pool)
 {
-    ThreadCpuNote note{0};
     prctl(PR_SET_TIMERSLACK, 2000UL, 0, 0, 0);
     Queue *queue = &pool->noise_q;
     std::deque<Speculation> open;
@@ -780,18 +792,17 @@
     };
     for (;;) {
         settle_verdicts();
-        if (pool->test_delay_us > 0)
-            std::this_thread::sleep_for(std::chrono::microseconds(pool->test_delay_us));
+        if (const int delay_us = pool->test_delay_us.load(std::memory_order_relaxed))
+            std::this_thread::sleep_for(std::chrono::microseconds(delay_us));
         fokl_host_job *job = nullptr;
         bool stopping = false, must_settle = false;
         {
             std::unique_lock<std::mutex> lock(queue->m);
             if (open.empty()) {
-                const auto w0 = std::chrono::steady_clock::now();
+                const int64_t w0 = now_ns();
                 queue->cv.wait(lock, [&] { return queue->stop || !queue->q.empty(); });
-                pool->noise_queue_wait_ns.fetch_add(
-                    std::chrono::duration_cast<std::chrono::nanoseconds>(std::chrono::steady_clock::now() - w0).count(),
-                    std::memory_order_relaxed);
+                pool->noise_queue_wait_ns.fetch_add(now_ns() - std::max(w0, pool->fit_begin_ns.load(std::memory_order_acquire)),
+                                                    std::memory_order_relaxed);
                 if (queue->q.empty()) return;
             }
             stopping = queue->stop;
@@ -868,6 +879,46 @@
     queue.cv.notify_all();
 }
 
+void read_fit_environment(fokl_host_pool *pool)
+{
+    const char *path = std::getenv("FOKL_POOL_TRACE");
+    pool->trace_path = path ? path : "";
+    const char *us = std::getenv("FOKL_POOL_TEST_DELAY_US");
+    pool->test_delay_us.store(us ? std::max(0, std::atoi(us)) : 0, std::memory_order_relaxed);
+    const char *signs = std::getenv("FOKL_EIGH_SIGNS");
+    pool->lapack_signs = signs && std::strcmp(signs, "lapack") == 0;
+    const char *sing = std::getenv("FOKL_EIGH_SINGULAR");
+    pool->singular = sing ? std::max(0.0, std::atof(sing)) : 1e-9;
+}
+
+void note_pool_cpu(fokl_host_pool *pool)
+{
+    pool->thread_noted_ns.resize(pool->threads.size(), 0);
+    for (size_t i = 0; i < pool->threads.size(); ++i) {
+        clockid_t clock;
+        timespec ts;
+        if (!pool->threads[i].joinable() || pthread_getcpuclockid(pool->threads[i].native_handle(), &clock) != 0 ||
+            clock_gettime(clock, &ts) != 0)
+            continue;
+        const int64_t ns = (int64_t)ts.tv_sec * 1000000000LL + ts.tv_nsec;
+        g_thread_cpu_ns[pool->thread_kinds[i]].fetch_add(ns - pool->thread_noted_ns[i], std::memory_order_relaxed);
+        pool->thread_noted_ns[i] = ns;
+    }
+    fokl_stream_note_cpu(pool->stream);
+}
+
+void flush_trace(fokl_host_pool *pool)
+{
+    if (pool->trace_path.empty()) return;
+    if (FILE *f = std::fopen(pool->trace_path.c_str(), "a")) {
+        for (const auto &r : pool->trace)
+            std::fprintf(f, "noise %lld %lld %lld %lld %lld %lld %lld\n", (long long)r[0], (long long)r[1],
+                         (long long)r[2], (long long)r[3], (long long)r[4], (long long)r[5], (long long)r[6]);
+        std::fclose(f);
+    }
+    pool->trace.clear();
+}
+
 }
 
 extern "C" int fokl_pool_create(int chain_threads, int finish_threads, int spectral_threads, int bulk_threads,
@@ -895,11 +946,12 @@
     pool->mt_pos = mt_pos;
     pool->has_gauss = has_gauss;
     pool->gauss_cache = gauss_cache;
-    if (const char *path = std::getenv("FOKL_POOL_TRACE")) pool->trace_path = path;
-    if (const char *us = std::getenv("FOKL_POOL_TEST_DELAY_US")) pool->test_delay_us = std::max(0, std::atoi(us));
-    if (const char *signs = std::getenv("FOKL_EIGH_SIGNS")) pool->lapack_signs = std::strcmp(signs, "lapack") == 0;
-    if (const char *sing = std::getenv("FOKL_EIGH_SINGULAR")) pool->singular = std::max(0.0, std::atof(sing));
+    read_fit_environment(pool);
     try {
+        pool->thread_kinds.assign((size_t)(1 + chain_threads + finish_threads + spectral_threads), 0);
+        std::fill_n(pool->thread_kinds.begin() + 1, chain_threads, 1);
+        std::fill_n(pool->thread_kinds.begin() + 1 + chain_threads, finish_threads, 2);
+        std::fill_n(pool->thread_kinds.begin() + 1 + chain_threads + finish_threads, spectral_threads, 3);
         pool->threads.emplace_back(noise_worker, pool);
         if (noise_cpu >= 0 && noise_cpu < CPU_SETSIZE) {
             cpu_set_t set;
@@ -936,18 +988,64 @@
     stop(pool->chain_q);
     stop(pool->spectral_q);
     for (auto &q : pool->finish_q) stop(q);
+    {
+        std::unique_lock<std::mutex> lock(pool->done_m);
+        pool->done_cv.wait(lock, [&] { return pool->outstanding.load(std::memory_order_acquire) <= 0; });
+    }
+    note_pool_cpu(pool);
     for (auto &t : pool->threads) t.join();
-    fokl_stream_state(pool->stream, pool->mt_key, pool->mt_pos, pool->has_gauss, pool->gauss_cache);
+    if (!pool->parked) fokl_stream_state(pool->stream, pool->mt_key, pool->mt_pos, pool->has_gauss, pool->gauss_cache);
     fokl_stream_destroy(pool->stream);
-    if (!pool->trace_path.empty()) {
-        if (FILE *f = std::fopen(pool->trace_path.c_str(), "a")) {
-            for (const auto &r : pool->trace)
-                std::fprintf(f, "noise %lld %lld %lld %lld %lld %lld %lld\n", (long long)r[0], (long long)r[1],
-                             (long long)r[2], (long long)r[3], (long long)r[4], (long long)r[5], (long long)r[6]);
-            std::fclose(f);
-        }
-    }
+    flush_trace(pool);
     delete pool;
+}
+
+extern "C" int fokl_pool_end_fit(fokl_host_pool *pool)
+{
+    if (!pool) {
+        fokl_set_global_error("fokl_pool_end_fit: null pool");
+        return FOKL_ERR_ARG;
+    }
+    if (pool->parked) return FOKL_OK;
+    {
+        std::unique_lock<std::mutex> lock(pool->done_m);
+        pool->done_cv.wait(lock, [&] { return pool->outstanding.load(std::memory_order_acquire) <= 0; });
+    }
+    const int rc = fokl_stream_state(pool->stream, pool->mt_key, pool->mt_pos, pool->has_gauss, pool->gauss_cache);
+    fokl_stream_park(pool->stream);
+    pool->mt_key = nullptr;
+    pool->mt_pos = pool->has_gauss = nullptr;
+    pool->gauss_cache = nullptr;
+    flush_trace(pool);
+    note_pool_cpu(pool);
+    pool->parked = true;
+    return rc;
+}
+
+extern "C" int fokl_pool_begin_fit(fokl_host_pool *pool, uint32_t *mt_key, int32_t *mt_pos, int32_t *has_gauss,
+                                   double *gauss_cache, uint32_t *prestate_ring, int prestate_entries)
+{
+    if (!pool || !mt_key || !mt_pos || !has_gauss || !gauss_cache || *mt_pos < 0 || *mt_pos > 624) {
+        fokl_set_global_error("fokl_pool_begin_fit: null pool, null RNG state or invalid MT19937 position");
+        return FOKL_ERR_ARG;
+    }
+    if (!pool->parked) {
+        fokl_set_global_error("fokl_pool_begin_fit: the pool is bound to a fit (fokl_pool_end_fit first)");
+        return FOKL_ERR_STATE;
+    }
+    const int rc = fokl_stream_reset(pool->stream, mt_key, *mt_pos, *has_gauss, *gauss_cache, prestate_ring, prestate_entries);
+    if (rc != FOKL_OK) return rc;
+    pool->mt_key = mt_key;
+    pool->mt_pos = mt_pos;
+    pool->has_gauss = has_gauss;
+    pool->gauss_cache = gauss_cache;
+    for (auto *c : {&pool->noise_busy_ns, &pool->chain_busy_ns, &pool->finish_busy_ns, &pool->spectral_busy_ns,
+                    &pool->chains_segmented, &pool->chain_recuts, &pool->noise_queue_wait_ns, &pool->noise_verdict_wait_ns})
+        c->store(0, std::memory_order_relaxed);
+    read_fit_environment(pool);
+    pool->fit_begin_ns.store(now_ns(), std::memory_order_release);
+    pool->parked = false;
+    return FOKL_OK;
 }
 
 static void submit_finish_jobs(fokl_host_pool *pool, fokl_host_job *parent, bool finish_normals)
@@ -1012,6 +1110,7 @@
     job->rows_only = rows_only;
     if (!pool->trace_path.empty()) job->t_submit = now_ns();
     *out = job;
+    pool->outstanding.fetch_add(1, std::memory_order_relaxed);
     if (!rows_only && !pool->finish_q.empty()) {
         job->pending.store(1 + (int)pool->finish_q.size(), std::memory_order_relaxed);
         submit_finish_jobs(pool, job, finish == 1);
@@ -1061,6 +1160,7 @@
         job->raw_block_done = block_done;
     *out = job;
     if (pool->chain_profile) job->t_submit = now_ns();
+    pool->outstanding.fetch_add(1, std::memory_order_relaxed);
     submit(pool->chain_q, job);
     return FOKL_OK;
 }
@@ -1097,6 +1197,7 @@
     job->betahat_out = betahat_out;
     job->moments_out = moments_out;
     *job_out = job;
+    pool->outstanding.fetch_add(1, std::memory_order_relaxed);
     return FOKL_OK;
 }
 
diff --git a/fokl_gpy_amd/csrc/fokl_stream.cpp b/fokl_gpy_amd/csrc/fokl_stream.cpp
--- a/fokl_gpy_amd/csrc/fokl_stream.cpp
+++ b/fokl_gpy_amd/csrc/fokl_stream.cpp
@@ -22,7 +22,8 @@
 #include "fokl_spin.h"
 
 extern void fokl_set_global_error(const std::string &msg);
-extern "C" __attribute__((visibility("hidden"))) void fokl_note_thread_cpu(int kind);
+__attribute__((visibility("hidden"))) void fokl_note_threads_cpu(std::vector<std::thread> &threads, std::vector<int64_t> &noted,
+                                                                 int kind);
 
 namespace {
 
@@ -346,7 +347,11 @@
     std::atomic<int64_t> pre_published{0};
     bool stop = false;
     std::atomic<bool> stop_flag{false};
+    std::atomic<bool> paused{false};
+    std::atomic<uint64_t> epoch{0};
+    std::atomic<int> producing{0};
     std::vector<std::thread> threads;
+    std::vector<int64_t> threads_noted_ns;
     std::atomic<Segment *> table[kTable];
     std::atomic<int64_t> bulk_busy_ns{0}, segments_made{0};
     std::atomic<int64_t> token_ns{0}, token_recurrence_ns{0}, token_wait_ns{0};
@@ -416,10 +421,6 @@
 
 void bulk_worker(fokl_stream *e)
 {
-    struct Note {
-        ~Note() { fokl_note_thread_cpu(4); }
-    } note;
-
     void *scratch_mem = nullptr;
     if (posix_memalign(&scratch_mem, 64, sizeof(uint32_t) * (size_t)(MT_N + kSegWords + kSegTail + 64)) != 0) {
         std::lock_guard<std::mutex> lock(e->token_m);
@@ -457,12 +458,15 @@
                     return;
                 }
                 const int64_t low = e->low_water.load(std::memory_order_acquire);
-                if (e->next_raw < e->limit.load(std::memory_order_acquire) && e->next_raw - low < kTable - 2) break;
+                if (!e->paused.load(std::memory_order_relaxed) && e->next_raw < e->limit.load(std::memory_order_acquire) &&
+                    e->next_raw - low < kTable - 2)
+                    break;
                 const int64_t next = e->next_raw;
+                const uint64_t epoch = e->epoch.load(std::memory_order_relaxed);
                 lock.unlock();
                 auto room_now = [&] {
-                    return e->stop_flag.load(std::memory_order_seq_cst) ||
-                           (next < e->limit.load(std::memory_order_seq_cst) &&
+                    return e->stop_flag.load(std::memory_order_seq_cst) || e->epoch.load(std::memory_order_seq_cst) != epoch ||
+                           (!e->paused.load(std::memory_order_seq_cst) && next < e->limit.load(std::memory_order_seq_cst) &&
                             next - e->low_water.load(std::memory_order_seq_cst) < kTable - 2);
                 };
                 bool ready = false;
@@ -485,6 +489,7 @@
                 ++e->oldest_alive;
             }
             index = e->next_raw;
+            e->producing.fetch_add(1, std::memory_order_relaxed);
             seg->index = index;
             seg->ready.store(0, std::memory_order_relaxed);
             const int64_t t0 = now_ns();
@@ -507,6 +512,7 @@
         e->table[index % kTable].store(seg, std::memory_order_release);
         e->segments_made.fetch_add(1, std::memory_order_relaxed);
         e->bulk_busy_ns.fetch_add(now_ns() - t0, std::memory_order_relaxed);
+        e->producing.fetch_sub(1, std::memory_order_release);
     }
 }
 
@@ -1281,6 +1287,7 @@
     std::mutex m;
     std::condition_variable cv;
     std::vector<std::thread> threads;
+    std::vector<int64_t> threads_noted_ns;
     std::vector<int> cpus;
 };
 
@@ -1322,9 +1329,6 @@
 
 FOKL_WIDE_TARGET void crew_helper(WalkCrew *crew, int which)
 {
-    struct Note {
-        ~Note() { fokl_note_thread_cpu(0); }
-    } note;
     if (which < (int)crew->cpus.size() && crew->cpus[(size_t)which] >= 0) {
         cpu_set_t set;
         CPU_ZERO(&set);
@@ -1332,6 +1336,7 @@
         (void)sched_setaffinity(0, sizeof(set), &set);
     }
     Walk checker(crew->e, Walk::ReaderOnly{});
+    uint64_t epoch = crew->e->epoch.load(std::memory_order_acquire);
     std::unique_ptr<BlockOut> out(new BlockOut());
     for (;;) {
         uint64_t n = 0;
@@ -1351,6 +1356,11 @@
                 spins = 0;
             }
         }
+        const uint64_t now = crew->e->epoch.load(std::memory_order_acquire);
+        if (now != epoch) {
+            checker.r = Reader(crew->e, false);
+            epoch = now;
+        }
         crew_process(crew, n, *out, checker);
     }
 }
@@ -1364,6 +1374,7 @@
         crew->stop.store(true, std::memory_order_seq_cst);
     }
     crew->cv.notify_all();
+    fokl_note_threads_cpu(crew->threads, crew->threads_noted_ns, 0);
     for (auto &t : crew->threads) t.join();
     delete crew;
     e->crew = nullptr;
@@ -1761,9 +1772,79 @@
     }
     e->room_cv.notify_all();
     crew_stop(e);
+    fokl_note_threads_cpu(e->threads, e->threads_noted_ns, 4);
     for (auto &t : e->threads) t.join();
     for (auto &t : e->table) give_segment(t.exchange(nullptr));
     delete e;
+}
+
+extern "C" __attribute__((visibility("hidden"))) void fokl_stream_note_cpu(fokl_stream *e)
+{
+    if (!e) return;
+    fokl_note_threads_cpu(e->threads, e->threads_noted_ns, 4);
+    if (e->crew) fokl_note_threads_cpu(e->crew->threads, e->crew->threads_noted_ns, 0);
+}
+
+extern "C" __attribute__((visibility("hidden"))) void fokl_stream_park(fokl_stream *e)
+{
+    if (!e) return;
+    {
+        std::lock_guard<std::mutex> lock(e->token_m);
+        e->paused.store(true, std::memory_order_seq_cst);
+    }
+    for (int spins = 0; e->producing.load(std::memory_order_acquire) > 0; ++spins) {
+        if (spins < 2000)
+            _mm_pause();
+        else
+            std::this_thread::sleep_for(std::chrono::microseconds(5));
+    }
+}
+
+extern "C" int fokl_stream_reset(fokl_stream *e, const uint32_t *mt_key, int32_t mt_pos, int32_t has_gauss, double gauss_cache,
+                                 uint32_t *prestate_ring, int prestate_entries)
+{
+    if (!e || !mt_key || mt_pos < 0 || mt_pos > MT_N ||
+        (prestate_ring && prestate_entries < 4 * kAheadMax * (kSegBlocks / FOKL_PRESTATE_BLOCKS))) {
+        fokl_set_global_error("fokl_stream_reset: null pointer, invalid MT19937 position or a pre-state ring too small");
+        return FOKL_ERR_ARG;
+    }
+    if (e->stop_flag.load(std::memory_order_acquire)) {
+        fokl_set_global_error("fokl_stream_reset: the stream's producers stopped (" + e->error + ")");
+        return FOKL_ERR_STATE;
+    }
+    fokl_stream_park(e);
+    {
+        std::lock_guard<std::mutex> lock(e->token_m);
+        for (auto &t : e->table) give_segment(t.exchange(nullptr, std::memory_order_acq_rel));
+        std::memcpy(e->key0, mt_key, sizeof(e->key0));
+        e->pos0 = mt_pos;
+        e->o = mt_pos & 1;
+        e->next_raw = 0;
+        e->oldest_alive = 0;
+        e->limit.store(kAhead, std::memory_order_seq_cst);
+        e->ahead.store(kAhead, std::memory_order_relaxed);
+        e->low_water.store(0, std::memory_order_seq_cst);
+        e->pre_ring = prestate_ring;
+        e->pre_entries = prestate_ring ? prestate_entries : 0;
+        e->pre_published.store(0, std::memory_order_release);
+        {
+            std::lock_guard<std::mutex> hold(e->hold_m);
+            e->holds.clear();
+            e->D = (uint64_t)(mt_pos >> 1);
+            e->walker_floor = e->D;
+        }
+        e->has_gauss = has_gauss ? 1 : 0;
+        e->gauss_src = kGivenGauss;
+        e->gauss0 = gauss_cache;
+        for (auto *c : {&e->bulk_busy_ns, &e->segments_made, &e->token_ns, &e->token_recurrence_ns, &e->token_wait_ns,
+                        &e->walker_wait_ns, &e->exact_draws, &e->gamma_draws, &e->rollbacks, &e->position_iterations})
+            c->store(0, std::memory_order_relaxed);
+        e->epoch.fetch_add(1, std::memory_order_seq_cst);
+        e->paused.store(false, std::memory_order_seq_cst);
+    }
+    { std::lock_guard<std::mutex> room(e->room_m); }
+    e->room_cv.notify_all();
+    return FOKL_OK;
 }
 
 extern "C" int fokl_stream_place_bulk(fokl_stream *e, const int32_t *cpus, int count)
diff --git a/fokl_gpy_amd/engine.py b/fokl_gpy_amd/engine.py
--- a/fokl_gpy_amd/engine.py
+++ b/fokl_gpy_amd/engine.py
@@ -895,7 +895,7 @@
                 if self.native is not None:
                     self.native.close()
                     self.native = None
-                self.host.close()
+                self.host.close(keep=False)
                 self.host = None
                 if self._head is not None:
                     self._ahead_block(self._head[1])
@@ -915,9 +915,13 @@
         self.stats['chain_mode'] = 'device' if self.chain_engine is not None else 'host'
         self.stats['eigh_mode'] = (os.environ.get('FOKL_EIGH', 'host') if getattr(self, 'spectral_engine', None) is not None
                                    and self.native is not None else 'host')
+        self.stats['pool_reused'] = int(self.host is not None and self.host.reused)
         t_up = time.perf_counter()
+        ended_well = False
         try:
-            return self._run()
+            result = self._run()
+            ended_well = True
+            return result
         finally:
             _mark('run_end')
             t_down = time.perf_counter()
@@ -940,7 +944,7 @@
                     now = self.chain_engine.stats()
                     self.stats.update({'dchain_' + k: v - self._dchain_stats0.get(k, 0) for k, v in now.items()})
                 t_close = time.perf_counter()
-                busy = self.host.close()
+                busy = self.host.close(keep=ended_well and not (self.allreduce or self.candidate_sharded))
                 self.stats['t_teardown_pool'] = time.perf_counter() - t_close
                 dgemm1 = _capi.device_dgemm_stats()
                 self.stats.update(eigen_update_products=dgemm1[0] - dgemm0[0], eigen_update_products_on_device=dgemm1[1] - dgemm0[1],
diff --git a/fokl_gpy_amd/host_pipeline.py b/fokl_gpy_amd/host_pipeline.py
--- a/fokl_gpy_amd/host_pipeline.py
+++ b/fokl_gpy_amd/host_pipeline.py
@@ -251,7 +251,50 @@
     return engine
 
 
+_KEPT_POOLS = {}
+_KEPT_LOCK = threading.Lock()
+_EVERY_DEVICE = object()
+
+
+def _take_kept_pool(device, key):
+    with _KEPT_LOCK:
+        kept = _KEPT_POOLS.pop(device, None)
+    if kept is None:
+        return None
+    pid, kept_key, pool = kept
+    if pid != os.getpid():
+        pool.abandon()
+        return None
+    if kept_key != key:
+        pool.close()
+        return None
+    return pool
+
+
+def _park_pool(device, key, pool):
+    with _KEPT_LOCK:
+        if device not in _KEPT_POOLS:
+            _KEPT_POOLS[device] = (os.getpid(), key, pool)
+            return
+    pool.close()
+
+
+def drop_kept_pools(device=_EVERY_DEVICE):
+    with _KEPT_LOCK:
+        devices = list(_KEPT_POOLS) if device is _EVERY_DEVICE else [d for d in _KEPT_POOLS if d == device]
+        kept = [_KEPT_POOLS.pop(d) for d in devices]
+    for pid, _, pool in kept:
+        if pid == os.getpid():
+            pool.close()
+        else:
+            pool.abandon()
+
+
+_capi.before_device_close.append(drop_kept_pools)
+
+
 def close_chain_engines():
+    drop_kept_pools()
     for engine in list(_CHAIN_ENGINES.values()) + list(_SPECTRAL_ENGINES.values()):
         engine.close()
     _CHAIN_ENGINES.clear()
@@ -298,58 +341,103 @@
         self._saved_affinity, noise_cpu = None, -1
         if os.environ.get('FOKL_PIN_L3', '1') != '0':
             self._saved_affinity, noise_cpu = _place_host_threads()
-        chain, finish, spectral = _thread_plan(wide_models)
-        self.device_rows = False
-        prestates = None
-        if isinstance(chain_engine, _capi.DeviceChainEngine) and os.environ.get('FOKL_DCHAIN_ROWS', '1') != '0':
-            try:
-                prestates = chain_engine.prestate_ring()
-            except _capi.FoklNativeError:
-                prestates = None
+        self.device_rows = self.reused = False
+        self._device, self._key, self.pool = device, None, None
         try:
-            dgemm_from = int(os.environ.get('FOKL_EIGH_DGEMM_FROM', '0'))
-            bulk = _bulk_threads(wide_models=wide_models)
-            self.pool = _capi.HostPool(stream, chain, finish, spectral, noise_cpu, bulk_threads=bulk,
-                                       prestates=prestates,
-                                       device_dgemm=(device, dgemm_from) if device is not None and dgemm_from > 0 else None)
-            if prestates is not None:
+            plan = self._plan(chain_engine, wide_models, device, noise_cpu)
+            self._keep = (os.environ.get('FOKL_POOL_KEEP', '1') != '0' and self.comm is None and comm is None and not _TRACE_PATH
+                          and not os.environ.get('FOKL_POOL_TRACE')
+                          and (chain_engine is None or isinstance(chain_engine, _capi.DeviceChainEngine)))
+            self._key = tuple(sorted(plan.items()))
+            self.pool = _take_kept_pool(device, self._key) if self._keep else None
+            if self.pool is not None:
+                try:
+                    self.pool.begin_fit(stream, prestates=plan['prestates'], device_dgemm=plan['device_dgemm'])
+                    self.reused = True
+                except _capi.FoklNativeError:
+                    self.pool.close()
+                    self.pool = None
+            if self.pool is None:
+                if not self._keep:
+                    drop_kept_pools(device)
+                self.pool = self._create_pool(stream, plan)
+            if plan['prestates'] is not None:
                 chain_engine.bind(self.pool.stream_handle())
                 self.device_rows = True
-            helpers = int(os.environ.get('FOKL_WALK_HELPERS', str(0 if wide_models else _walk_helpers_default())))
-            if helpers > 0:
-                cpus = None
-                if self._saved_affinity is not None and os.environ.get('FOKL_WALK_CPUS', 'other') != 'same':
-                    picked = _other_cores(self._saved_affinity, os.sched_getaffinity(0), spectral + helpers)
-                    if picked is not None:
-                        cpus = picked[-helpers:]
-                try:
-                    self.pool.set_walk_helpers(helpers, cpus)
-                except _capi.FoklNativeError:
-                    pass
-            if (self._saved_affinity is not None and _cpu_budget() >= 12 and os.environ.get('FOKL_BULK_CPUS', 'other') != 'same'):
-                picked = _other_cores(self._saved_affinity, os.sched_getaffinity(0), spectral + max(0, helpers) + bulk)
-                if picked is not None:
-                    try:
-                        self.pool.place_bulk_threads(picked[-bulk:])
-                    except _capi.FoklNativeError:
-                        pass
-            if self._saved_affinity is not None and os.environ.get('FOKL_SPECTRAL_DOMAIN', '1') != '0':
-                other = None
-                if os.environ.get('FOKL_SPECTRAL_DOMAIN', '1') != 'domain' and spectral > 0:
-                    other = _spectral_cpus(self._saved_affinity, os.sched_getaffinity(0), spectral)
-                if other is None:
-                    other = _second_domain(self._saved_affinity, os.sched_getaffinity(0))
-                if other:
-                    try:
-                        self.pool.spectral_affinity(other)
-                    except _capi.FoklNativeError:
-                        pass
         except BaseException:
+            if self.pool is not None:
+                self.pool.close()
             self._restore_affinity()
             raise
         self._live = []
         self._reap_at = 24
         self._spare = _thread_spares()
+
+    def _plan(self, chain_engine, wide_models, device, noise_cpu):
+        try:
+            allowed = frozenset(self._saved_affinity if self._saved_affinity is not None else os.sched_getaffinity(0))
+            home = frozenset(os.sched_getaffinity(0))
+        except (AttributeError, OSError):
+            allowed = home = frozenset()
+        chain, finish, spectral = _thread_plan(wide_models)
+        prestates = None
+        if isinstance(chain_engine, _capi.DeviceChainEngine) and os.environ.get('FOKL_DCHAIN_ROWS', '1') != '0':
+            try:
+                prestates = tuple(chain_engine.prestate_ring())
+            except _capi.FoklNativeError:
+                prestates = None
+        dgemm_from = int(os.environ.get('FOKL_EIGH_DGEMM_FROM', '0'))
+        bulk = _bulk_threads(wide_models=wide_models)
+        helpers = int(os.environ.get('FOKL_WALK_HELPERS', str(0 if wide_models else _walk_helpers_default())))
+        helper_cpus = None
+        if helpers > 0 and self._saved_affinity is not None and os.environ.get('FOKL_WALK_CPUS', 'other') != 'same':
+            picked = _other_cores(self._saved_affinity, home, spectral + helpers)
+            if picked is not None:
+                helper_cpus = tuple(picked[-helpers:])
+        bulk_cpus = None
+        if (self._saved_affinity is not None and _cpu_budget() >= 12 and os.environ.get('FOKL_BULK_CPUS', 'other') != 'same'):
+            picked = _other_cores(self._saved_affinity, home, spectral + max(0, helpers) + bulk)
+            if picked is not None:
+                bulk_cpus = tuple(picked[-bulk:])
+        spectral_cpus = None
+        if self._saved_affinity is not None and os.environ.get('FOKL_SPECTRAL_DOMAIN', '1') != '0':
+            other = None
+            if os.environ.get('FOKL_SPECTRAL_DOMAIN', '1') != 'domain' and spectral > 0:
+                other = _spectral_cpus(self._saved_affinity, home, spectral)
+            if other is None:
+                other = _second_domain(self._saved_affinity, home)
+            if other:
+                spectral_cpus = tuple(sorted(other))
+        return dict(allowed=tuple(sorted(allowed)), home=tuple(sorted(home)), noise_cpu=noise_cpu,
+                    chain=chain, finish=finish, spectral=spectral, bulk=bulk, helpers=helpers, helper_cpus=helper_cpus,
+                    bulk_cpus=bulk_cpus, spectral_cpus=spectral_cpus, prestates=prestates,
+                    engine=id(chain_engine) if chain_engine is not None else None,
+                    device_dgemm=(device, dgemm_from) if device is not None and dgemm_from > 0 else None)
+
+    @staticmethod
+    def _create_pool(stream, plan):
+        pool = _capi.HostPool(stream, plan['chain'], plan['finish'], plan['spectral'], plan['noise_cpu'],
+                              bulk_threads=plan['bulk'], prestates=plan['prestates'], device_dgemm=plan['device_dgemm'])
+        try:
+            if plan['helpers'] > 0:
+                try:
+                    pool.set_walk_helpers(plan['helpers'], plan['helper_cpus'])
+                except _capi.FoklNativeError:
+                    pass
+            if plan['bulk_cpus'] is not None:
+                try:
+                    pool.place_bulk_threads(plan['bulk_cpus'])
+                except _capi.FoklNativeError:
+                    pass
+            if plan['spectral_cpus']:
+                try:
+                    pool.spectral_affinity(plan['spectral_cpus'])
+                except _capi.FoklNativeError:
+                    pass
+        except BaseException:
+            pool.close()
+            raise
+        return pool
 
     CLASS_DOUBLES = 65536
 
@@ -503,7 +591,7 @@
             chain_job.recycle.append(w_raw)
             noise_job.co_reader = chain_job
 
-    def close(self):
+    def close(self, keep=True):
         for job in self._live:
             if job.unresolved:
                 job.resolve(False)
@@ -517,8 +605,18 @@
         if self.device_rows:
             self.dchain.bind(None)
             self.device_rows = False
-        self.pool.close()
-        self._restore_affinity()
+        if keep and self._keep:
+            try:
+                self.pool.end_fit()
+                _park_pool(self._device, self._key, self.pool)
+            except _capi.FoklNativeError:
+                self.pool.close()
+                raise
+            finally:
+                self._restore_affinity()
+        else:
+            self.pool.close()
+            self._restore_affinity()
         return busy
 
     def _restore_affinity(self):
diff --git a/include/fokl_hip_internal.h b/include/fokl_hip_internal.h
--- a/include/fokl_hip_internal.h
+++ b/include/fokl_hip_internal.h
@@ -34,6 +34,8 @@
 int64_t fokl_stream_prestates_published(const fokl_stream *stream);
 double fokl_stream_given_gauss(const fokl_stream *stream);
 void fokl_stream_destroy(fokl_stream *stream);
+int fokl_stream_reset(fokl_stream *stream, const uint32_t *mt_key, int32_t mt_pos, int32_t has_gauss, double gauss_cache,
+                      uint32_t *prestate_ring, int prestate_entries);
 int fokl_stream_walk(fokl_stream *stream, int p1, int draws, double astar, double atau_star, fokl_tape_row *rows,
                      double *gam_sig, double *gam_tau, int32_t *progress);
 int fokl_stream_tell(const fokl_stream *stream, fokl_stream_cursor *out);
@@ -69,6 +71,9 @@
 int fokl_pool_spectral_affinity(fokl_host_pool *pool, const int32_t *cpus, int count);
 fokl_stream *fokl_pool_stream(fokl_host_pool *pool);
 void fokl_pool_destroy(fokl_host_pool *pool);
+int fokl_pool_end_fit(fokl_host_pool *pool);
+int fokl_pool_begin_fit(fokl_host_pool *pool, uint32_t *mt_key, int32_t *mt_pos, int32_t *has_gauss, double *gauss_cache,
+                        uint32_t *prestate_ring, int prestate_entries);
 int fokl_tape_ready(const int32_t *progress, int draws, const int32_t *block_done, int block);
 
 int fokl_pool_submit_noise(fokl_host_pool *pool, int p1, int draws, double astar, double atau_star, fokl_tape_row *rows,
```

Result: slower. 564,800 (-3.2%).
